# limix/CellRegMap

Measured on AMD Instinct MI355X. Metric: variant-tests/sec (interaction test), higher is better.
Workload: dtype f64

## Files before the change

### cellregmap_amd/_lib.py

```python
import ctypes
import os

import numpy as np

_HERE = os.path.dirname(os.path.abspath(__file__))
LIB_PATH = os.path.join(_HERE, "libcrm_hip.so")

c_double_p = ctypes.POINTER(ctypes.c_double)
c_int_p = ctypes.POINTER(ctypes.c_int)
c_long_p = ctypes.POINTER(ctypes.c_long)
vp = ctypes.c_void_p

SIGNATURES = {
    "crm_last_error": (ctypes.c_char_p, []),
    "crm_version": (ctypes.c_char_p, []),
    "crm_ctx_create": (ctypes.c_int, [ctypes.c_int, ctypes.POINTER(vp)]),
    "crm_ctx_destroy": (None, [vp]),
    "crm_ctx_synchronize": (ctypes.c_int, [vp]),
    "crm_ctx_trim": (ctypes.c_int, [vp]),
    "crm_background_create_qs": (ctypes.c_int, [vp, ctypes.c_long, ctypes.c_int, vp, vp, vp, vp,
                                                ctypes.POINTER(vp)]),
    "crm_background_create": (ctypes.c_int, [vp, ctypes.c_long, vp, ctypes.c_int, vp, ctypes.c_long,
                                             ctypes.c_int, vp, ctypes.c_double, ctypes.POINTER(vp)]),
    "crm_background_create_hadamard": (ctypes.c_int, [vp, ctypes.c_long, vp, ctypes.c_int, vp, ctypes.c_int, vp,
                                                      ctypes.c_int, ctypes.c_int, vp, ctypes.c_double,
                                                      ctypes.POINTER(vp)]),
    "crm_background_set_kinship_groups": (ctypes.c_int, [vp, vp, ctypes.c_long, vp, ctypes.c_long, vp, ctypes.c_int]),
    "crm_background_kinship_groups": (ctypes.c_int, [vp]),
    "crm_background_kinship_folded": (ctypes.c_long, [vp]),
    "crm_background_begin": (ctypes.c_int, [vp, ctypes.c_long, vp, ctypes.c_int, vp, ctypes.c_long, vp, ctypes.c_int, vp,
                                            ctypes.c_int, ctypes.c_int, vp, vp, ctypes.c_double, ctypes.POINTER(vp)]),
    "crm_background_complete": (ctypes.c_int, [vp, vp]),
    "crm_background_layout": (ctypes.c_int, [vp, c_long_p, c_long_p, c_long_p, c_int_p]),
    "crm_background_export": (ctypes.c_int, [vp, ctypes.c_int, ctypes.c_int, vp]),
    "crm_background_import": (ctypes.c_int, [vp, ctypes.c_int, ctypes.c_int, vp]),
    "crm_background_seal": (ctypes.c_int, [vp]),
    "crm_background_destroy": (None, [vp]),
    "crm_background_rank": (ctypes.c_int, [vp, ctypes.c_int]),
    "crm_background_read": (ctypes.c_int, [vp, ctypes.c_int, vp, vp]),
    "crm_gene_create": (ctypes.c_int, [vp, vp, vp, ctypes.c_int, vp, ctypes.c_int, ctypes.POINTER(vp)]),
    "crm_gene_create_like": (ctypes.c_int, [vp, vp, ctypes.POINTER(vp)]),
    "crm_gene_create_batch": (ctypes.c_int, [vp, vp, ctypes.c_long, ctypes.c_int, ctypes.POINTER(vp)]),
    "crm_gene_destroy": (None, [vp]),
    "crm_panel_create": (ctypes.c_int, [vp, ctypes.c_long, vp, ctypes.c_long, ctypes.c_long,
                                        ctypes.POINTER(vp)]),
    "crm_panel_create_grouped": (ctypes.c_int, [vp, ctypes.c_long, vp, ctypes.c_long, vp, ctypes.c_long,
                                                ctypes.c_long, ctypes.POINTER(vp)]),
    "crm_panel_create_grouped_i8": (ctypes.c_int, [vp, ctypes.c_long, vp, ctypes.c_long, vp, ctypes.c_long, ctypes.c_long,
                                                   ctypes.c_int, ctypes.POINTER(vp)]),
    "crm_panel_create_auto": (ctypes.c_int, [vp, ctypes.c_long, vp, ctypes.c_long, ctypes.c_long, vp, ctypes.c_long,
                                             vp, ctypes.POINTER(vp), c_int_p]),
    "crm_set_donor_collapse": (ctypes.c_int, [vp, ctypes.c_int]),
    "crm_panel_destroy": (None, [vp]),
    "crm_scan_interaction": (ctypes.c_int, [vp, vp, ctypes.c_long, ctypes.c_long] + [vp] * 13),
    "crm_scan_interaction_info": (ctypes.c_int, [vp, vp, ctypes.c_long, ctypes.c_long] + [vp] * 6),
    "crm_scan_interaction_bounds": (ctypes.c_int, [vp, vp, ctypes.c_long, ctypes.c_long] + [vp] * 8),
    "crm_scan_interaction_permuted": (ctypes.c_int, [vp, vp, ctypes.c_long, ctypes.c_long, ctypes.c_int] + [vp] * 8),
    "crm_scan_interaction_multi": (ctypes.c_int, [vp, ctypes.c_int, vp, ctypes.c_long, ctypes.c_long] + [vp] * 8),
    "crm_scan_interaction_tail": (ctypes.c_int, [vp, vp, ctypes.c_long, ctypes.c_long] + [vp] * 15),
    "crm_scan_interaction_permuted_tail": (ctypes.c_int, [vp, vp, ctypes.c_long, ctypes.c_long, ctypes.c_int] + [vp] * 10),
    "crm_scan_interaction_multi_tail": (ctypes.c_int, [vp, ctypes.c_int, vp, ctypes.c_long, ctypes.c_long] + [vp] * 10),
    "crm_scan_association": (ctypes.c_int, [vp, vp, ctypes.c_long, ctypes.c_long, ctypes.c_int, vp, vp, vp]),
    "crm_association_null_multi": (ctypes.c_int, [vp, ctypes.c_int, vp]),
    "crm_scan_association_multi": (ctypes.c_int, [vp, ctypes.c_int, vp, ctypes.c_long, ctypes.c_long, ctypes.c_int, vp, vp,
                                                  vp]),
    "crm_lmm_fit": (ctypes.c_int, [vp, ctypes.c_int, vp, vp]),
    "crm_cov_solve": (ctypes.c_int, [vp, ctypes.c_int, ctypes.c_double, ctypes.c_double, vp, ctypes.c_int, vp]),
    "crm_effects_multi": (ctypes.c_int, [vp, vp, ctypes.c_long, vp, ctypes.c_int, vp, ctypes.c_int, vp, ctypes.c_int, vp,
                                         ctypes.c_int, vp, ctypes.c_int, ctypes.c_int, vp, vp, vp, vp]),
    "crm_set_block_variants": (ctypes.c_int, [vp, ctypes.c_int]),
    "crm_set_null_fit_polish": (ctypes.c_int, [vp, ctypes.c_int]),
    "crm_set_progress_callback": (ctypes.c_int, [vp, vp, vp]),
    "crm_set_fast_rotation": (ctypes.c_int, [vp, ctypes.c_int]),
    "crm_kernel_timer_reset": (ctypes.c_int, [vp]),
    "crm_kernel_timer_read": (ctypes.c_int, [vp, c_double_p, c_long_p, c_double_p, c_double_p]),
    "crm_kernel_timer_stop": (ctypes.c_int, [vp]),
    "crm_test_set_form": (ctypes.c_int, [ctypes.c_char_p, ctypes.c_int, ctypes.c_int]),
    "crm_test_set_contraction": (ctypes.c_int, [vp, ctypes.c_int, ctypes.c_int]),
    "crm_test_set_shared_h": (ctypes.c_int, [vp, ctypes.c_int]),
    "crm_test_tail_launches": (ctypes.c_long, [vp]),
    "crm_test_spectrum_tail_launches": (ctypes.c_long, [vp]),
    "crm_test_dense_repeats": (ctypes.c_long, [vp]),
    "crm_test_donor_pair_blocks": (ctypes.c_long, [vp]),
    "crm_test_unrelated_donor_blocks": (ctypes.c_int, [vp, ctypes.POINTER(ctypes.c_long)]),
    "crm_test_gram_dma_launches": (ctypes.c_int, [vp, ctypes.POINTER(ctypes.c_long)]),
    "crm_test_rho0_position_blocks": (ctypes.c_int, [vp, ctypes.POINTER(ctypes.c_long)]),
    "crm_test_rotation_tail_launches": (ctypes.c_int, [vp, ctypes.POINTER(ctypes.c_long)]),
    "crm_test_tests_without_pair": (ctypes.c_long, [vp]),
    "crm_test_set_contraction_sync": (ctypes.c_int, [vp, ctypes.c_int]),
    "crm_test_sync_fallbacks": (ctypes.c_long, [vp]),
    "crm_test_overruns": (ctypes.c_long, []),
    "crm_test_live_device_bytes": (ctypes.c_long, []),
    "crm_test_set_kinship_route": (ctypes.c_int, [vp, ctypes.c_int]),
    "crm_test_check_context": (ctypes.c_int, [vp]),
    "crm_test_overrun_selftest": (ctypes.c_int, [vp]),
    "crm_test_null_fit_probe": (ctypes.c_int, [vp, ctypes.c_int, ctypes.c_double]),
    "crm_test_null_fit_probe_read": (ctypes.c_int, [vp, vp, ctypes.c_long]),
    "crm_test_contract": (ctypes.c_int, [vp, ctypes.c_long, ctypes.c_int, ctypes.c_int, vp, vp, vp,
                                         ctypes.c_int]),
    "crm_test_contract_kr": (ctypes.c_int, [vp, ctypes.c_long, ctypes.c_int, ctypes.c_int, ctypes.c_int,
                                            vp, vp, vp, vp]),
    "crm_test_contract_kr_t": (ctypes.c_int, [vp, ctypes.c_long, ctypes.c_int, ctypes.c_int, ctypes.c_int,
                                              vp, vp, vp, vp]),
    "crm_test_eigh": (ctypes.c_int, [vp, ctypes.c_int, ctypes.c_int, vp, vp, vp, ctypes.c_int, vp, vp]),
    "crm_test_eigh2": (ctypes.c_int, [vp, ctypes.c_int, ctypes.c_int, vp, vp, vp, vp, vp, ctypes.c_int, vp, vp, vp]),
    "crm_test_back_tasks": (ctypes.c_int, [ctypes.c_int, ctypes.c_long, ctypes.c_int, vp, ctypes.c_int, c_int_p]),
    "crm_test_dc_plan": (ctypes.c_int, [vp, vp, ctypes.c_int, ctypes.c_int, ctypes.c_double, c_int_p, c_double_p, vp, vp, vp,
                                        c_int_p, vp]),
    "crm_test_eigvalsh": (ctypes.c_int, [vp, ctypes.c_int, ctypes.c_int, vp, vp]),
    "crm_test_davies": (ctypes.c_int, [vp, ctypes.c_int, ctypes.c_int, vp, vp, vp, vp, vp]),
    "crm_test_davies_trace": (ctypes.c_int, [vp, ctypes.c_int, ctypes.c_int, vp, vp, vp, vp, vp, vp]),
    "crm_test_tail_pvalue": (ctypes.c_int, [vp, ctypes.c_int, ctypes.c_int, vp, vp, vp, vp, vp]),
}

_lib = None


class CrmError(RuntimeError):
    pass


def load():
    global _lib
    if _lib is not None:
        return _lib
    if not os.path.exists(LIB_PATH):
        raise CrmError(
            f"{LIB_PATH} is missing: build it with `python -m cellregmap_amd.build` "
            "(there is no CPU fallback for this path)")
    lib = ctypes.CDLL(LIB_PATH)
    for name, (res, args) in SIGNATURES.items():
        fn = getattr(lib, name)
        fn.restype = res
        fn.argtypes = args
    _lib = lib
    return lib


def check(rc):
    if rc != 0:
        msg = load().crm_last_error()
        raise CrmError(f"libcrm_hip error {rc}: {msg.decode() if msg else ''}")


def f64(a):
    return np.ascontiguousarray(a, dtype=np.float64)


def ptr(a):
    return None if a is None else a.ctypes.data_as(vp)
```

### cellregmap_amd/csrc/api_core.hip

```cpp
#include <dlfcn.h>

#include <algorithm>
#include <atomic>
#include <cstdarg>
#include <mutex>

#include <map>

#include "crm_internal.h"
#include "eigh.h"

namespace crm {

static thread_local std::string g_error;

void set_error(const char* fmt, ...) {
    char buf[1024];
    va_list ap;
    va_start(ap, fmt);
    vsnprintf(buf, sizeof buf, fmt, ap);
    va_end(ap);
    g_error = buf;
}

const char* last_error_text() { return g_error.c_str(); }

namespace {
struct Roctx {
    int (*push)(const char*) = nullptr;
    int (*pop)() = nullptr;
    Roctx() {
        void* h = dlopen("librocprofiler-sdk-roctx.so", RTLD_LAZY | RTLD_GLOBAL);
        if (!h) h = dlopen("librocprofiler-sdk-roctx.so.1", RTLD_LAZY | RTLD_GLOBAL);
        if (!h) return;
        push = reinterpret_cast<int (*)(const char*)>(dlsym(h, "roctxRangePushA"));
        pop = reinterpret_cast<int (*)()>(dlsym(h, "roctxRangePop"));
        if (!push || !pop) push = nullptr, pop = nullptr;
    }
};
const Roctx& roctx() {
    static Roctx r;
    return r;
}
bool ranges_on() {
    static const bool on = getenv("CRM_ROCTX") || getenv("ROCP_TOOL_LIBRARIES") || getenv("ROCPROFILER_LIBRARY_CTOR");
    return on;
}
}

void trace_push(const char* name) {
    if (ranges_on() && roctx().push) roctx().push(name);
}
void trace_pop() {
    if (ranges_on() && roctx().pop) roctx().pop();
}

static bool poison_mode() {
    static const bool on = getenv("CRM_POISON") && atoi(getenv("CRM_POISON")) != 0;
    return on;
}
static constexpr size_t REDZONE = 4096;
static std::atomic<long> g_overruns{0};
long overruns_detected() { return g_overruns.load(); }
static std::atomic<long> g_live_bytes{0};
long live_device_bytes() { return g_live_bytes.load(); }

static void check_redzone(const void* ptr, size_t bytes) {
    if (!ptr || !poison_mode()) return;
    std::vector<unsigned char> rz(REDZONE);
    if (hipMemcpy(rz.data(), static_cast<const char*>(ptr) + bytes, REDZONE, hipMemcpyDeviceToHost) != hipSuccess) return;
    for (size_t i = 0; i < REDZONE; i++) {
        if (rz[i] != 0xFF) {
            g_overruns++;
            fprintf(stderr, "[crm] CRM_POISON: write past the end of a %zu-byte device buffer (first touched byte at +%zu)\n",
                    bytes, i);
            break;
        }
    }
}

static hipStream_t fill_stream() {
    static std::mutex mu;
    static std::map<int, hipStream_t> streams;
    int dev = 0;
    if (hipGetDevice(&dev) != hipSuccess) return nullptr;
    std::lock_guard<std::mutex> lock(mu);
    auto it = streams.find(dev);
    if (it != streams.end()) return it->second;
    hipStream_t st = nullptr;
    if (hipStreamCreateWithFlags(&st, hipStreamNonBlocking) != hipSuccess) st = nullptr;
    streams[dev] = st;
    return st;
}

int DevBuf::ensure(size_t need) {
    if (need <= bytes) return CRM_OK;
    if (ptr) {
        check_redzone(ptr, bytes);
        CRM_HIP(hipFree(ptr));
        g_live_bytes -= (long)bytes;
        ptr = nullptr;
        bytes = 0;
    }
    const size_t total = need + REDZONE;
    hipError_t e = hipMalloc(&ptr, total);
    if (e == hipErrorOutOfMemory && trim_idle_workspaces() > 0) {
        (void)hipGetLastError();
        e = hipMalloc(&ptr, total);
    }
    if (e != hipSuccess) {
        ptr = nullptr;
        (void)hipGetLastError();
        set_error("device allocation of %zu bytes failed: %s", need, hipGetErrorString(e));
        return CRM_ERR_HIP;
    }
    bytes = need;
    g_live_bytes += (long)need;
    hipStream_t fs = fill_stream();
    CRM_HIP(hipMemsetAsync(ptr, poison_mode() ? 0xFF : 0, total, fs));
    CRM_HIP(hipStreamSynchronize(fs));
    return CRM_OK;
}

static std::mutex g_ctx_mutex;
static std::vector<crm_ctx*> g_contexts;

static size_t trim_context(crm_ctx* c) {
    if (!c->eigh_ws || c->eigh_ws_busy) return 0;
    size_t freed = 0;
    for (const DevBuf* b : {&c->eigh_ws->A, &c->eigh_ws->Vt, &c->eigh_ws->Vc, &c->eigh_ws->QA, &c->eigh_ws->QB}) freed += b->bytes;
    *c->eigh_ws = EighWork();
    return freed;
}

EighWork* acquire_eigh_workspace(crm_ctx* c) {
    std::lock_guard<std::mutex> lock(g_ctx_mutex);
    if (!c->eigh_ws) c->eigh_ws = new EighWork();
    c->eigh_ws_busy = true;
    return c->eigh_ws;
}

void release_eigh_workspace(crm_ctx* c) {
    std::lock_guard<std::mutex> lock(g_ctx_mutex);
    c->eigh_ws_busy = false;
}

size_t trim_idle_workspaces() {
    std::lock_guard<std::mutex> lock(g_ctx_mutex);
    size_t freed = 0;
    for (crm_ctx* c : g_contexts) freed += trim_context(c);
    return freed;
}
void DevBuf::release() {
    if (ptr) check_redzone(ptr, bytes);
    if (ptr) (void)hipFree(ptr);
    g_live_bytes -= (long)bytes;
    ptr = nullptr;
    bytes = 0;
}

int upload_padded(hipStream_t st, double* dst, long ld_dst, long rows_pad, const double* src,
                  long ld_src, long rows, long cols) {
    CRM_HIP(hipMemsetAsync(dst, 0, sizeof(double) * rows_pad * ld_dst, st));
    if (rows > 0 && cols > 0)
        CRM_HIP(hipMemcpy2DAsync(dst, ld_dst * sizeof(double), src, ld_src * sizeof(double),
                                 cols * sizeof(double), rows, hipMemcpyHostToDevice, st));
    return CRM_OK;
}

}

using namespace crm;

extern "C" {

const char* crm_last_error(void) { return last_error_text(); }
const char* crm_version(void) { return "0.6.0"; }

int crm_ctx_create(int device, crm_ctx** out) {
    return crm::guarded("crm_ctx_create", [&]() -> int {
    if (!out) return CRM_ERR_ARG;
    *out = nullptr;
    int count = 0;
    CRM_HIP(hipGetDeviceCount(&count));
    if (device < 0 || device >= count) {
        set_error("crm_ctx_create: device %d not present (%d visible)", device, count);
        return CRM_ERR_ARG;
    }
    CRM_HIP(hipSetDevice(device));
    crm_ctx* c = new crm_ctx();
    c->device = device;
    if (const char* e = getenv("CRM_KIN_ROUTE")) c->kin_route = std::max(0, std::min(2, atoi(e)));
    CRM_HIP(hipStreamCreateWithFlags(&c->stream, hipStreamNonBlocking));
    CRM_HIP(hipStreamCreateWithFlags(&c->upload_stream, hipStreamNonBlocking));
    CRM_HIP(hipEventCreate(&c->ev0));
    CRM_HIP(hipEventCreate(&c->ev1));
    {
        std::lock_guard<std::mutex> lock(g_ctx_mutex);
        g_contexts.push_back(c);
    }
    *out = c;
    return CRM_OK;
    });
}

int crm_ctx_trim(crm_ctx* c) {
    return crm::guarded_on("crm_ctx_trim", c, [&]() -> int {
    if (!c) return CRM_ERR_ARG;
    CRM_HIP(hipSetDevice(c->device));
    CRM_HIP(hipStreamSynchronize(c->stream));
    std::lock_guard<std::mutex> lock(g_ctx_mutex);
    (void)trim_context(c);
    return CRM_OK;
    });
}

void crm_ctx_destroy(crm_ctx* c) {
    try {
    if (!c) return;
    (void)hipSetDevice(c->device);
    (void)hipStreamSynchronize(c->stream);
    {
        std::lock_guard<std::mutex> lock(g_ctx_mutex);
        g_contexts.erase(std::remove(g_contexts.begin(), g_contexts.end(), c), g_contexts.end());
        delete c->eigh_ws;
        c->eigh_ws = nullptr;
    }
    c->replay_clear();
    for (auto* b : c->all_bufs()) b->release();
    for (auto& e : c->timed) {
        (void)hipEventDestroy(e.first);
        (void)hipEventDestroy(e.second);
    }
    (void)hipEventDestroy(c->ev0);
    (void)hipEventDestroy(c->ev1);
    (void)hipStreamDestroy(c->stream);
    if (c->upload_stream) (void)hipStreamDestroy(c->upload_stream);
    if (c->sync_timeouts_host) (void)hipHostFree(c->sync_timeouts_host);
    delete c;
    } catch (...) {
    }
}

int crm_ctx_synchronize(crm_ctx* c) {
    return crm::guarded_on("crm_ctx_synchronize", c, [&]() -> int {
    if (!c) return CRM_ERR_ARG;
    CRM_HIP(hipSetDevice(c->device));
    CRM_HIP(hipStreamSynchronize(c->stream));
    return CRM_OK;
    });
}

int crm_set_block_variants(crm_ctx* c, int variants) {
    return crm::guarded_on("crm_set_block_variants", c, [&]() -> int {
    if (!c || variants < 0) return CRM_ERR_ARG;
    c->block_variants = variants == 0 ? 0 : (int)round_up(variants, 128);
    return CRM_OK;
    });
}

int crm_set_null_fit_polish(crm_ctx* c, int on) {
    return crm::guarded_on("crm_set_null_fit_polish", c, [&]() -> int {
    if (!c) return CRM_ERR_ARG;
    c->polish = on != 0;
    return CRM_OK;
    });
}

int crm_set_progress_callback(crm_ctx* c, void (*callback)(long, long, void*), void* user) {
    return crm::guarded_on("crm_set_progress_callback", c, [&]() -> int {
    if (!c) return CRM_ERR_ARG;
    if (callback) c->progress[std::this_thread::get_id()] = crm_ctx::Progress{callback, user};
    else c->progress.erase(std::this_thread::get_id());
    return CRM_OK;
    });
}

int crm_set_fast_rotation(crm_ctx* c, int on) {
    return crm::guarded_on("crm_set_fast_rotation", c, [&]() -> int {
    if (!c) return CRM_ERR_ARG;
    c->fast_T = on != 0;
    return CRM_OK;
    });
}

extern "C++" {
namespace crm {
namespace {
struct FormSlot { const char* name; int value; bool set; };
FormSlot g_forms[] = {{"gram_staged", 0, false}, {"kr_no_tail", 0, false}, {"nullfit_per_wave", 0, false}, {"kin_fold", 0, false},
                      {"eigh_one_stage", 0, false}, {"nullfit_exact", 0, false}, {"donor_pairs", 0, false},
                      {"pairs_without_kinship_term", 0, false}, {"flat_kappa_milli", 0, false}, {"chase_abort", 0, false}, {"nullfit_one_per_wave", 0, false},
                      {"kin_diag", 0, false}, {"donor_pairs_rotate", 0, false}, {"rho0_positions", 0, false},
                      {"rotation_tails", 0, false}, {"woodbury_ytY", 0, false},
                      {"wb_block_order", 0, false}};
std::mutex g_forms_mu;
}
int form(const char* name, int otherwise) {
    std::lock_guard<std::mutex> lock(g_forms_mu);
    for (const FormSlot& f : g_forms)
        if (strcmp(f.name, name) == 0) return f.set ? f.value : otherwise;
    return otherwise;
}
}
}

int crm_test_set_form(const char* name, int value, int reset) {
    return crm::guarded("crm_test_set_form", [&]() -> int {
    if (!name) return CRM_ERR_ARG;
    std::lock_guard<std::mutex> lock(crm::g_forms_mu);
    for (crm::FormSlot& f : crm::g_forms)
        if (strcmp(f.name, name) == 0) {
            f.value = value;
            f.set = reset == 0;
            return CRM_OK;
        }
    crm::set_error("crm_test_set_form: no kernel form is called '%s'", name);
    return CRM_ERR_ARG;
    });
}

long crm_test_tail_launches(const crm_ctx* ctx) { return ctx ? ctx->tail_launches : -1; }

long crm_test_spectrum_tail_launches(const crm_ctx* ctx) { return ctx ? ctx->spectrum_tail_launches : -1; }

long crm_test_dense_repeats(const crm_ctx* ctx) { return ctx ? ctx->dense_repeats : -1; }

long crm_test_donor_pair_blocks(const crm_ctx* ctx) { return ctx ? ctx->donor_pair_blocks : -1; }

int crm_test_gram_dma_launches(const crm_ctx* ctx, long* launches) {
    return crm::guarded("crm_test_gram_dma_launches", [&]() -> int {
    if (!ctx || !launches) return CRM_ERR_ARG;
    *launches = ctx->gram_dma_launches;
    return CRM_OK;
    });
}
int crm_test_unrelated_donor_blocks(const crm_ctx* ctx, long* blocks) {
    return crm::guarded("crm_test_unrelated_donor_blocks", [&]() -> int {
    if (!ctx || !blocks) return CRM_ERR_ARG;
    *blocks = ctx->unrelated_donor_blocks;
    return CRM_OK;
    });
}

int crm_test_rho0_position_blocks(const crm_ctx* ctx, long* blocks) {
    return crm::guarded("crm_test_rho0_position_blocks", [&]() -> int {
    if (!ctx || !blocks) return CRM_ERR_ARG;
    *blocks = ctx->rho0_position_blocks;
    return CRM_OK;
    });
}
int crm_test_rotation_tail_launches(const crm_ctx* ctx, long* launches) {
    return crm::guarded("crm_test_rotation_tail_launches", [&]() -> int {
    if (!ctx || !launches) return CRM_ERR_ARG;
    *launches = ctx->rotation_tail_launches;
    return CRM_OK;
    });
}

long crm_test_tests_without_pair(const crm_ctx* ctx) { return ctx ? ctx->tests_without_pair : -1; }

int crm_test_set_shared_h(crm_ctx* ctx, int mode) {
    return crm::guarded_on("crm_test_set_shared_h", ctx, [&]() -> int {
    if (!ctx) return CRM_ERR_ARG;
    ctx->tune.shared_h = mode < 0 ? -1 : (mode > 0 ? 1 : 0);
    return CRM_OK;
    });
}

int crm_kernel_timer_reset(crm_ctx* c) {
    return crm::guarded_on("crm_kernel_timer_reset", c, [&]() -> int {
    if (!c) return CRM_ERR_ARG;
    CRM_HIP(hipSetDevice(c->device));
    CRM_HIP(hipStreamSynchronize(c->stream));
    c->timed_used = 0;
    c->kr_flops = 0.0;
    c->timing = true;
    return CRM_OK;
    });
}

int crm_kernel_timer_stop(crm_ctx* c) {
    return crm::guarded_on("crm_kernel_timer_stop", c, [&]() -> int {
    if (!c) return CRM_ERR_ARG;
    c->timing = false;
    return CRM_OK;
    });
}

int crm_kernel_timer_read(crm_ctx* c, double* kr_ms, long* kr_launches, double* kr_flops,
                          double* total_ms) {
    return crm::guarded_on("crm_kernel_timer_read", c, [&]() -> int {
    if (!c) return CRM_ERR_ARG;
    CRM_HIP(hipSetDevice(c->device));
    CRM_HIP(hipStreamSynchronize(c->stream));
    double ms = 0.0;
    for (size_t i = 0; i < c->timed_used; i++) {
        float t = 0.f;
        CRM_HIP(hipEventElapsedTime(&t, c->timed[i].first, c->timed[i].second));
        ms += t;
    }
    if (kr_ms) *kr_ms = ms;
    if (kr_launches) *kr_launches = (long)c->timed_used;
    if (kr_flops) *kr_flops = c->kr_flops;
    if (total_ms) *total_ms = 0.0;
    return CRM_OK;
    });
}

int crm_test_set_contraction(crm_ctx* c, int tile_width, int lds_dma) {
    return crm::guarded_on("crm_test_set_contraction", c, [&]() -> int {
    if (!c || (tile_width != 0 && tile_width != 64 && tile_width != 128 && tile_width != 160)) return CRM_ERR_ARG;
    c->tune.bn = tile_width;
    c->tune.glds = lds_dma ? 1 : 0;
    return CRM_OK;
    });
}

long crm_test_sync_fallbacks(const crm_ctx* c) { return c ? c->sync_fallbacks : -1; }
long crm_test_overruns(void) { return crm::overruns_detected(); }
long crm_test_live_device_bytes(void) { return crm::live_device_bytes(); }

int crm_test_set_kinship_route(crm_ctx* c, int on) {
    return crm::guarded_on("crm_test_set_kinship_route", c, [&]() -> int {
    if (!c) return CRM_ERR_ARG;
    c->kin_route = on < 0 ? 0 : (on > 2 ? 2 : on);
    return CRM_OK;
    });
}

int crm_test_overrun_selftest(crm_ctx* c) {
    return crm::guarded_on("crm_test_overrun_selftest", c, [&]() -> int {
    if (!c) return CRM_ERR_ARG;
    CRM_HIP(hipSetDevice(c->device));
    const long before = overruns_detected();
    {
        DevBuf b;
        CRM_TRY(b.ensure(1000));
        if (poison_mode()) CRM_HIP(hipMemset(static_cast<char*>(b.ptr) + 1000, 0, 8));
        CRM_HIP(hipDeviceSynchronize());
    }
    return (int)(overruns_detected() - before);
    });
}

int crm_test_check_context(crm_ctx* c) {
    return crm::guarded_on("crm_test_check_context", c, [&]() -> int {
    if (!c) return CRM_ERR_ARG;
    CRM_HIP(hipSetDevice(c->device));
    CRM_HIP(hipStreamSynchronize(c->stream));
    for (const DevBuf* b : c->all_bufs()) check_redzone(b->ptr, b->bytes);
    if (c->eigh_ws)
        for (const DevBuf* b : {&c->eigh_ws->A, &c->eigh_ws->Vt, &c->eigh_ws->Vc, &c->eigh_ws->QA, &c->eigh_ws->QB, &c->eigh_ws->d,
                                &c->eigh_ws->e, &c->eigh_ws->tau, &c->eigh_ws->lam, &c->eigh_ws->small})
            check_redzone(b->ptr, b->bytes);
    return CRM_OK;
    });
}

int crm_test_null_fit_probe(crm_ctx* c, int on, double x) {
    return crm::guarded_on("crm_test_null_fit_probe", c, [&]() -> int {
    if (!c) return CRM_ERR_ARG;
    if (on < 0 || on > 2) return CRM_ERR_ARG;
    c->probe_on = on != 0;
    c->probe_mode = on;
    c->probe_x = x;
    return CRM_OK;
    });
}

int crm_test_null_fit_probe_read(crm_ctx* c, double* out, long capacity) {
    return crm::guarded_on("crm_test_null_fit_probe_read", c, [&]() -> int {
    if (!c || !out || capacity < (long)c->probe_out.size()) return CRM_ERR_ARG;
    std::copy(c->probe_out.begin(), c->probe_out.end(), out);
    return (int)c->probe_out.size();
    });
}

int crm_test_set_contraction_sync(crm_ctx* c, int every) {
    return crm::guarded_on("crm_test_set_contraction_sync", c, [&]() -> int {
    if (!c || every < 0) return CRM_ERR_ARG;
    c->tune.sync = every;
    return CRM_OK;
    });
}

int crm_test_contract(crm_ctx* c, long cells, int M, int N, const double* X, const double* Y,
                      double* C, int ksplit) {
    return crm::guarded_on("crm_test_contract", c, [&]() -> int {
    if (!c || cells <= 0 || M <= 0 || N <= 0 || !X || !Y || !C || ksplit < 1) return CRM_ERR_ARG;
    CRM_HIP(hipSetDevice(c->device));
    const long cp = round_up(cells, GEMM_BK * (long)ksplit);
    const long ldx = round_up(M, 128), ldy = round_up(N, 128);
// ... 170 lines not shown
```

### cellregmap_amd/csrc/blockops.hip

```cpp
#include "nullfit.h"

namespace crm {

namespace {

constexpr int STAT_SPLITS = 64;

__device__ __forceinline__ void row_and_chunk(int chunks, long& row, int& chunk) {
    row = blockIdx.x / (unsigned)chunks;
    chunk = (int)(blockIdx.x - (unsigned)row * (unsigned)chunks);
}
inline dim3 row_chunk_grid(long rows, int chunks) { return dim3((unsigned)(rows * chunks)); }

template <int C>
__global__ __launch_bounds__(256) void variant_stats_kernel(const double* __restrict__ G, long ldg,
                                                           long cells, int variants,
                                                           const double* __restrict__ y,
                                                           const double* __restrict__ W, long ldw,
                                                           double* __restrict__ partial) {
    __shared__ double red[4][C + 2][64];
    const int tx = threadIdx.x & 63, ty = threadIdx.x >> 6;
    const int b = blockIdx.x * 64 + tx;
    const long per = (cells + STAT_SPLITS - 1) / STAT_SPLITS;
    const long i0 = (long)blockIdx.y * per;
// ... 213 lines not shown
    if (q >= dst_cols) return;
    double v = 0.0;
    const int p = q / k0;
    if (p < npairs) v = src[h * ld_src + (long)ord[p] * k0 + (q - p * k0)];
    dst[h * ld_dst + q] = v;
}

int launch_gather_slabs(hipStream_t st, const double* src, long ld_src, long rows, const int* ord, int npairs,
                        int k0, double* dst, long ld_dst, int dst_cols) {
    if (rows <= 0 || dst_cols <= 0) return CRM_OK;
    dim3 grid((unsigned)rows, (dst_cols + 255) / 256);
    hipLaunchKernelGGL(gather_slabs_kernel, grid, dim3(256), 0, st, src, ld_src, ord, npairs, k0, dst, ld_dst,
                       dst_cols);
    CRM_HIP(hipGetLastError());
    return CRM_OK;
}

__global__ void gather_rows_kernel(const double* __restrict__ src, long ld_src, const int* __restrict__ map, int cols,
                                   double* __restrict__ dst, long ld_dst, int chunks) {
    long k;
    int chunk;
    row_and_chunk(chunks, k, chunk);
    const int j = chunk * blockDim.x + threadIdx.x;
    if (j >= cols) return;
    const int c = map[k];
    dst[k * ld_dst + j] = c >= 0 ? src[(long)c * ld_src + j] : 0.0;
}

int launch_gather_rows(hipStream_t st, const double* src, long ld_src, const int* map, long rows, int cols, double* dst,
                       long ld_dst) {
    if (rows <= 0 || cols <= 0) return CRM_OK;
    const int chunks = (cols + 255) / 256;
    hipLaunchKernelGGL(gather_rows_kernel, row_chunk_grid(rows, chunks), dim3(256), 0, st, src, ld_src, map, cols, dst, ld_dst,
                       chunks);
    CRM_HIP(hipGetLastError());
    return CRM_OK;
}

__global__ void kin_operand_kernel(const double* __restrict__ U, int k2, const double* __restrict__ H, long ldh, int k1,
                                   const int* __restrict__ map, double* __restrict__ Y, long ldy) {
    const long k = blockIdx.x;
    const int j = threadIdx.x;
    if (j >= ldy) return;
    const int c = map[k];
    double v = 0.0;
    if (c >= 0) {
        if (j < k2) v = U[(long)c * k2 + j];
        else if (j < k2 + k1) v = H[(long)c * ldh + (j - k2)];
    }
    Y[k * ldy + j] = v;
}

int launch_kin_operand(hipStream_t st, const double* U, int k2, const double* H, long ldh, int k1, const int* map, long rows,
                       double* Y, long ldy) {
    if (rows <= 0) return CRM_OK;
    hipLaunchKernelGGL(kin_operand_kernel, dim3((unsigned)rows), dim3((unsigned)ldy), 0, st, U, k2, H, ldh, k1, map, Y, ldy);
    CRM_HIP(hipGetLastError());
    return CRM_OK;
}

__global__ void kin_verify_kernel(const double* __restrict__ H, long ldh, int k1, const double* __restrict__ U, int k2,
                                  const int* __restrict__ group, const double* __restrict__ hKd, long ldk, long m,
                                  unsigned long long* __restrict__ out) {
    const long c = blockIdx.x;
    const long g = group[c];
    double dmax = 0.0, hmax = 0.0;
    for (long e = threadIdx.x; e < (long)k2 * m; e += blockDim.x) {
        const long j = e / m, d = e - j * m;
        const double h = H[c * ldh + k1 + e];
        const double want = U[c * k2 + j] * hKd[g * ldk + d];
        const double diff = fabs(h - want);
        dmax = diff > dmax || diff != diff ? diff : dmax;
        hmax = fmax(hmax, fabs(h));
    }
    for (int off = 32; off > 0; off >>= 1) {
        const double o = __shfl_xor(dmax, off);
        dmax = o > dmax || o != o ? o : dmax;
        hmax = fmax(hmax, __shfl_xor(hmax, off));
    }
    if ((threadIdx.x & 63) == 0) {
        if (dmax != dmax) dmax = INFINITY;
        atomicMax(&out[0], (unsigned long long)__double_as_longlong(dmax));
        atomicMax(&out[1], (unsigned long long)__double_as_longlong(hmax));
    }
}

int launch_kin_verify(hipStream_t st, const double* H, long ldh, int k1, const double* U, int k2, const int* group,
                      const double* hKd, long ldk, long m, long n, unsigned long long* out) {
    if (n <= 0) return CRM_OK;
    hipLaunchKernelGGL(kin_verify_kernel, dim3((unsigned)n), dim3(256), 0, st, H, ldh, k1, U, k2, group, hKd, ldk, m, out);
    CRM_HIP(hipGetLastError());
    return CRM_OK;
}

__global__ void kin_sum_e1_kernel(const double* __restrict__ S, long ld_s, int KT, int k2, int groups, long cols,
                                  double* __restrict__ AH, long ld_ah) {
    const int a = blockIdx.y;
    const long c = (long)blockIdx.x * blockDim.x + threadIdx.x;
    if (c >= cols) return;
    double acc = 0.0;
    for (int d = 0; d < groups; d++) acc += S[((long)d * KT + k2 + a) * ld_s + c];
    AH[(long)a * ld_ah + c] = acc;
}

int launch_kin_sum_e1(hipStream_t st, const double* S, long ld_s, int KT, int k2, int k1, int groups, long cols, double* AH,
                      long ld_ah) {
    if (k1 <= 0 || cols <= 0) return CRM_OK;
    dim3 grid((unsigned)((cols + 255) / 256), (unsigned)k1);
    hipLaunchKernelGGL(kin_sum_e1_kernel, grid, dim3(256), 0, st, S, ld_s, KT, k2, groups, cols, AH, ld_ah);
    CRM_HIP(hipGetLastError());
    return CRM_OK;
}

__global__ void ortho_coef_kernel(const double* __restrict__ gW, long ld_gW, const double* __restrict__ proj, int c,
                                  int variants, int cols, double* __restrict__ coef, long ld_coef,
                                  double* __restrict__ thr) {
    const int b = blockIdx.x * blockDim.x + threadIdx.x;
    if (b >= cols) return;
    constexpr double EPS = 2.220446049250313e-16;
    const double* __restrict__ inv = proj;
    const double* __restrict__ V = proj + (long)c * c;
    const double* __restrict__ d2 = V + (long)c * c;
    const double* __restrict__ h = gW + (long)b * ld_gW;
    double t = 1.0;
    for (int j = 0; j < c; j++) {
        double a = 0.0;
        if (b < variants) {
            double hv = 0.0;
            for (int k = 0; k < c; k++) {
                a = fma(inv[j * c + k], h[k], a);
                hv = fma(V[k * c + j], h[k], hv);
            }
            t += (hv / d2[j]) * (hv / (d2[j] - EPS));
        }
        coef[(long)j * ld_coef + b] = a;
    }
    if (b < variants) thr[b] = EPS * t;
}

__global__ __launch_bounds__(256) void ortho_apply_kernel(const double* __restrict__ G, long ldg,
                                                         const double* __restrict__ W, long ldw, int c,
                                                         const double* __restrict__ coef, long ld_coef, int cols,
                                                         double* __restrict__ Gx, long ldx, int chunks) {
    long i;
    int chunk;
    row_and_chunk(chunks, i, chunk);
    const int b = chunk * blockDim.x + threadIdx.x;
    if (b >= cols) return;
    double v = G[i * ldg + b];
    for (int j = 0; j < c; j++) v = fma(-W[i * ldw + j], coef[(long)j * ld_coef + b], v);
    Gx[i * ldx + b] = v;
}

__global__ void ortho_rank_kernel(const double* __restrict__ gg, const double* __restrict__ thr, int variants,
                                  int* __restrict__ drop) {
    const int b = blockIdx.x * blockDim.x + threadIdx.x;
    if (b < variants) drop[b] = gg[b] < thr[b] ? 1 : 0;
}

__global__ void collinear_flag_kernel(const double* __restrict__ gg, const double* __restrict__ gW, long ld_gW,
                                      const double* __restrict__ proj, int c, int variants, double tau,
                                      int* __restrict__ near) {
    const int b = blockIdx.x * blockDim.x + threadIdx.x;
    if (b >= variants) return;
    const double* __restrict__ h = gW + (long)b * ld_gW;
    double rest = gg[b];
    for (int j = 0; j < c; j++) {
        double a = 0.0;
        for (int k = 0; k < c; k++) a = fma(proj[j * c + k], h[k], a);
        rest -= h[j] * a;
    }
    near[b] = rest > tau * gg[b] ? 0 : 1;
}

int launch_ortho_block(hipStream_t st, const double* G, long ldg, long cells_pad, int variants, int cols,
                       const double* W, long ldw, int c, const double* proj, const double* gW, long ld_gW,
                       double* coef, long ld_coef, double* thr, double* Gx, long ldx) {
    if (cols <= 0) return CRM_OK;
    hipLaunchKernelGGL(ortho_coef_kernel, dim3((cols + 255) / 256), dim3(256), 0, st, gW, ld_gW, proj, c, variants, cols,
                       coef, ld_coef, thr);
    CRM_HIP(hipGetLastError());
    const int chunks = (cols + 255) / 256;
    hipLaunchKernelGGL(ortho_apply_kernel, row_chunk_grid(cells_pad, chunks), dim3(256), 0, st, G, ldg, W,
                       ldw, c, coef, ld_coef, cols, Gx, ldx, chunks);
    CRM_HIP(hipGetLastError());
    return CRM_OK;
}

int launch_ortho_rank(hipStream_t st, const double* gg, const double* thr, int variants, int* drop) {
    if (variants <= 0) return CRM_OK;
    hipLaunchKernelGGL(ortho_rank_kernel, dim3((variants + 255) / 256), dim3(256), 0, st, gg, thr, variants, drop);
    CRM_HIP(hipGetLastError());
    return CRM_OK;
}

int launch_collinear_flag(hipStream_t st, const double* gg, const double* gW, long ld_gW, const double* proj, int c,
                          int variants, double tau, int* near) {
    if (variants <= 0) return CRM_OK;
    hipLaunchKernelGGL(collinear_flag_kernel, dim3((variants + 255) / 256), dim3(256), 0, st, gg, gW, ld_gW, proj, c,
                       variants, tau, near);
    CRM_HIP(hipGetLastError());
    return CRM_OK;
}

__global__ void pair_features_kernel(const double* __restrict__ H, long ldh, int k1, const double* __restrict__ Ep,
                                     long ld_ep, int k0, double* __restrict__ P, long ldp) {
    const long c = blockIdx.x;
    for (int q = threadIdx.x; q < ldp; q += blockDim.x) {
        const int a = q / k0, i = q - a * k0;
        P[c * ldp + q] = a < k1 ? H[c * ldh + a] * Ep[c * ld_ep + i] : 0.0;
    }
}

int launch_pair_features(hipStream_t st, const double* H, long ldh, int k1, const double* Ep, long ld_ep, int k0,
                         long cells_pad, double* P, long ldp) {
    if (cells_pad <= 0) return CRM_OK;
    hipLaunchKernelGGL(pair_features_kernel, dim3((unsigned)cells_pad), dim3(256), 0, st, H, ldh, k1, Ep, ld_ep, k0, P, ldp);
    CRM_HIP(hipGetLastError());
    return CRM_OK;
}

__global__ void same_columns_kernel(const double* __restrict__ H, long ldh, const double* __restrict__ Ep, long ld_ep,
                                    long cells, int k, int* __restrict__ flag) {
    const long c = blockIdx.x;
    if (c >= cells) return;
    bool diff = false;
    for (int a = threadIdx.x; a < k; a += blockDim.x)
        diff |= __double_as_longlong(H[c * ldh + a]) != __double_as_longlong(Ep[c * ld_ep + a]);
    if (diff) atomicOr(flag, 1);
}

int launch_same_columns(hipStream_t st, const double* H, long ldh, const double* Ep, long ld_ep, long cells, int k, int* flag) {
    if (cells <= 0 || k <= 0) return CRM_OK;
    hipLaunchKernelGGL(same_columns_kernel, dim3((unsigned)cells), dim3(64), 0, st, H, ldh, Ep, ld_ep, cells, k, flag);
    CRM_HIP(hipGetLastError());
    return CRM_OK;
}

__global__ void pair_rows_sym_kernel(const double* __restrict__ C, long ldc, int variants, int k0, double* __restrict__ S,
                                     long lds) {
    const int a = blockIdx.y;
    const long e = (long)blockIdx.x * blockDim.x + threadIdx.x;
    if (e >= (long)variants * k0) return;
    const long b = e / k0;
    const int i = (int)(e - b * k0);
    const int lo = a < i ? a : i, hi = a < i ? i : a;
    const long pidx = (long)lo * k0 - (long)lo * (lo - 1) / 2 + (hi - lo);
    S[(long)a * lds + e] = C[b * ldc + pidx];
}

int launch_pair_rows_sym(hipStream_t st, const double* C, long ldc, int variants, int k0, double* S, long lds) {
    if (variants <= 0 || k0 <= 0) return CRM_OK;
    dim3 grid((unsigned)(((long)variants * k0 + 255) / 256), (unsigned)k0);
    hipLaunchKernelGGL(pair_rows_sym_kernel, grid, dim3(256), 0, st, C, ldc, variants, k0, S, lds);
    CRM_HIP(hipGetLastError());
    return CRM_OK;
}

constexpr int DP_VARIANTS = 4, DP_MAX_SLOTS = 32;

template <int DP_SLOTS>
__global__ __launch_bounds__(256) void donor_pairs_expand_kernel(const double* __restrict__ P, long p_slab, long ldp, int donors,
                                                                  int variants, int k0, int k1, double* __restrict__ S, long lds,
                                                                  double* __restrict__ Psum, long psum_slab, long row_d, long row_j) {
    extern __shared__ double tile[];
    const int npair = k0 * (k0 + 1) / 2, total = DP_VARIANTS * npair;
    const int v0 = blockIdx.x * DP_VARIANTS, tid = threadIdx.x;
    const int per = (donors + gridDim.y - 1) / gridDim.y;
    const int d0 = blockIdx.y * per, d1 = min(donors, d0 + per);
    if (d0 >= d1) return;
    double acc[DP_SLOTS], x[DP_SLOTS];
    int src[DP_SLOTS];
#pragma unroll
    for (int q = 0; q < DP_SLOTS; q++) {
        const int e = tid + 256 * q, v = e / npair, pr = e - v * npair;
        acc[q] = 0.0;
        src[q] = e < total && v0 + v < variants ? (int)((long)(v0 + v) * ldp + pr) : -1;
    }
    auto fetch = [&](int d) {
        const double* __restrict__ Pd = P + (size_t)d * p_slab;
#pragma unroll
        for (int q = 0; q < DP_SLOTS; q++)
            if (tid + 256 * q < total) x[q] = src[q] >= 0 ? Pd[src[q]] : 0.0;
    };
    const int row_len = DP_VARIANTS * k0;
    const int vw = tid / k0, iw = tid - vw * k0;
    const bool writer = tid < row_len && v0 + vw < variants;
    const int base_i = iw * k0 - iw * (iw - 1) / 2 - iw;
    const double* __restrict__ mine = tile + vw * npair;
    fetch(d0);
    for (int d = d0; d < d1; d++) {
#pragma unroll
        for (int q = 0; q < DP_SLOTS; q++)
            if (tid + 256 * q < total) { acc[q] += x[q]; tile[tid + 256 * q] = x[q]; }
        __syncthreads();
        if (d + 1 < d1) fetch(d + 1);
        if (writer) {
            double* __restrict__ Sd = S + (size_t)(k1 + (long)d * row_d) * lds + (long)v0 * k0 + tid;
            for (int j = 0; j < k0; j++) {
                const int pidx = j <= iw ? j * k0 - j * (j - 1) / 2 + (iw - j) : base_i + j;
                Sd[(long)j * row_j * lds] = mine[pidx];
            }
        }
        __syncthreads();
    }
    double* __restrict__ out = Psum + (size_t)blockIdx.y * psum_slab;
#pragma unroll
    for (int q = 0; q < DP_SLOTS; q++)
        if (tid + 256 * q < total && src[q] >= 0) out[src[q]] = acc[q];
}

bool donor_pairs_serves(int k0) { return k0 >= 2 && DP_VARIANTS * (k0 * (k0 + 1) / 2) <= 256 * DP_MAX_SLOTS && DP_VARIANTS * k0 <= 256; }

int launch_donor_pairs_expand(hipStream_t st, const double* P, long p_slab, long ldp, int donors, int variants, int k0, int k1,
                              double* S, long lds, double* Psum, long psum_slab, int splits, long row_d, long row_j) {
    if (row_d <= 0) { row_d = k0; row_j = 1; }
    if (variants <= 0 || donors <= 0) return CRM_OK;
    if (!donor_pairs_serves(k0) || splits < 1) {
        set_error("donor pairs: k0=%d outside the supported range", k0);
        return CRM_ERR_UNSUPPORTED;
    }
    const size_t lds_bytes = sizeof(double) * DP_VARIANTS * (size_t)(k0 * (k0 + 1) / 2);
    dim3 grid((unsigned)((variants + DP_VARIANTS - 1) / DP_VARIANTS), (unsigned)splits);
    const int slots = (DP_VARIANTS * (k0 * (k0 + 1) / 2) + 255) / 256;
#define CRM_DP_LAUNCH(SL)                                                                                                        \
    hipLaunchKernelGGL(donor_pairs_expand_kernel<SL>, grid, dim3(256), lds_bytes, st, P, p_slab, ldp, donors, variants, k0, k1, \
                       S, lds, Psum, psum_slab, row_d, row_j)
    if (slots <= 4) CRM_DP_LAUNCH(4);
    else if (slots <= 8) CRM_DP_LAUNCH(8);
    else if (slots <= 16) CRM_DP_LAUNCH(16);
    else if (slots <= 24) CRM_DP_LAUNCH(24);
    else CRM_DP_LAUNCH(32);
#undef CRM_DP_LAUNCH
    CRM_HIP(hipGetLastError());
    return CRM_OK;
}

// ... 247 lines not shown
```

### cellregmap_amd/csrc/crm_internal.h

```cpp
#pragma once
#include <map>
#include <mutex>
#include <thread>
#include <type_traits>
#include <utility>

#include "crm_common.h"

namespace crm {

constexpr int CRM_DEFAULT_BLOCK = 1024;
constexpr int CRM_MAX_AUTO_BLOCK = 4096;
constexpr int CRM_MAX_RHO = 16;
constexpr int CRM_MAX_COV = 8;
constexpr int CRM_MAX_COV_WIDE = 62;
constexpr int CRM_MAX_COV_XWIDE = 128;
constexpr int CRM_MAX_K0 = 256;
constexpr int CRM_MAX_GRAM_ROWS = 288;
constexpr int DT_SUMS_LD = 136;
constexpr int BLOCK_SLACK_MAX = 4096;

struct DevBuf {
    void* ptr = nullptr;
    size_t bytes = 0;
    DevBuf() = default;
    DevBuf(const DevBuf&) = delete;
    DevBuf& operator=(const DevBuf&) = delete;
    DevBuf(DevBuf&& o) noexcept : ptr(o.ptr), bytes(o.bytes) { o.ptr = nullptr; o.bytes = 0; }
    DevBuf& operator=(DevBuf&& o) noexcept {
        if (this != &o) {
            release();
            ptr = o.ptr; bytes = o.bytes;
            o.ptr = nullptr; o.bytes = 0;
        }
        return *this;
    }
    ~DevBuf() { release(); }
    int ensure(size_t need);
    void release();
    template <class T>
    T* as() const { return static_cast<T*>(ptr); }
};
static_assert(!std::is_copy_constructible<DevBuf>::value, "DevBuf owns its allocation");

int upload_padded(hipStream_t st, double* dst, long ld_dst, long rows_pad, const double* src,
                  long ld_src, long rows, long cols);

struct EighWork;
size_t trim_idle_workspaces();
long overruns_detected();
long live_device_bytes();
}
struct crm_ctx;
namespace crm {
EighWork* acquire_eigh_workspace(crm_ctx* ctx);
void release_eigh_workspace(crm_ctx* ctx);

}

struct crm_ctx {
    std::recursive_mutex mu;
    int device = 0;
    hipStream_t stream = nullptr;
    hipStream_t upload_stream = nullptr;
    hipEvent_t ev0 = nullptr, ev1 = nullptr;
    int block_variants = 0;
    bool fast_T = true;
    int kin_route = 1;
    bool fast_gene_rot = true;
    bool collapse = true;
    struct Progress { void (*fn)(long done, long total, void* user) = nullptr; void* user = nullptr; };
    std::map<std::thread::id, Progress> progress;
    bool progress_muted = false;
    void report(long done, long total) {
        if (progress_muted) return;
        auto it = progress.find(std::this_thread::get_id());
        if (it != progress.end() && it->second.fn) it->second.fn(done, total, it->second.user);
    }
    bool in_scan = false;
    bool polish = false;
    bool probe_on = false;
    int probe_mode = 0;
    double probe_x = 0.0;
    std::vector<double> probe_out;
    bool nullfit_exact = false;
    crm::GemmTune tune;
    crm::DevBuf sync_counters;
    unsigned* sync_timeouts_host = nullptr;
    long sync_fallbacks = 0;
    long dense_repeats = 0;
    long tail_launches = 0;
    long spectrum_tail_launches = 0;
    long donor_pair_blocks = 0;
    long rotation_tail_launches = 0;
    long rho0_position_blocks = 0;
    long unrelated_donor_blocks = 0;
    long gram_dma_launches = 0;
    long tests_without_pair = 0;
    struct ReplayBlock {
        long col0 = 0;
        int nb = 0;
        bool collapsed = false;
        std::vector<char> fit;
        crm::DevBuf T;
    };
    int replay_mode = 0;
    size_t replay_cursor = 0;
    std::vector<ReplayBlock*> replay_blocks;
    void replay_clear() {
        for (ReplayBlock* b : replay_blocks) delete b;
        replay_blocks.clear();
        replay_cursor = 0;
        replay_mode = 0;
    }
    crm::EighWork* eigh_ws = nullptr;
    bool eigh_ws_busy = false;
    bool timing = false;
    std::vector<std::pair<hipEvent_t, hipEvent_t>> timed;
    size_t timed_used = 0;
    double kr_flops = 0.0;
    crm::DevBuf ws_T, ws_A, ws_Gb, ws_Gx, ws_Gs, ws_G2, ws_GG, ws_Gt, ws_Z, ws_small, ws_probs, ws_F, ws_Gext, ws_TH, ws_AH, ws_XG;
    crm::DevBuf ws_xwide;
    crm::DevBuf ws_Tcut;
    crm::DevBuf ws_Gk, ws_S, ws_S2;
    crm::DevBuf ws_WB;
    crm::DevBuf ws_Pd;
    crm::DevBuf ws_Anone;
    std::vector<crm::DevBuf*> all_bufs() {
        return {&sync_counters, &ws_xwide, &ws_Tcut, &ws_S, &ws_S2, &ws_Gk, &ws_Pd, &ws_WB, &ws_Anone, &ws_AH, &ws_XG, &ws_TH, &ws_T, &ws_A, &ws_Gb, &ws_Gx, &ws_Gs, &ws_G2, &ws_GG, &ws_Gt, &ws_Z, &ws_small, &ws_probs, &ws_F, &ws_Gext};
    }
};

namespace crm {
template <class Body>
inline int guarded_on(const char* entry, crm_ctx* ctx, Body&& body) noexcept {
    try {
        if (!ctx) return guarded(entry, body);
        std::lock_guard<std::recursive_mutex> lock(ctx->mu);
        return guarded(entry, body);
    } catch (...) {
        set_error("%s: could not take the context's lock", entry);
        return CRM_ERR_INTERNAL;
    }
}
}
```

### cellregmap_amd/csrc/kinship.hip

```cpp
#include <algorithm>
#include <atomic>

#include "nullfit.h"
#include "objects.h"

using namespace crm;

namespace crm {

void jacobi_rotate(int k, double* A, double* V, int p, int q, double cs, double sn) {
    for (int r = 0; r < k; r++) {
        const double arp = A[(size_t)r * k + p], arq = A[(size_t)r * k + q];
        A[(size_t)r * k + p] = cs * arp - sn * arq;
        A[(size_t)r * k + q] = sn * arp + cs * arq;
    }
    for (int r = 0; r < k; r++) {
        const double apr = A[(size_t)p * k + r], aqr = A[(size_t)q * k + r];
        A[(size_t)p * k + r] = cs * apr - sn * aqr;
        A[(size_t)q * k + r] = sn * apr + cs * aqr;
    }
    for (int r = 0; r < k; r++) {
        const double vrp = V[(size_t)r * k + p], vrq = V[(size_t)r * k + q];
        V[(size_t)r * k + p] = cs * vrp - sn * vrq;
        V[(size_t)r * k + q] = sn * vrp + cs * vrq;
    }
}

static void jacobi_eigh(int k, std::vector<double>& A, std::vector<double>& V, std::vector<double>& w) {
    V.assign((size_t)k * k, 0.0);
    for (int i = 0; i < k; i++) V[(size_t)i * k + i] = 1.0;
    for (int sweep = 0; sweep < 60; sweep++) {
        bool rotated = false;
        for (int p = 0; p < k - 1; p++)
            for (int q = p + 1; q < k; q++) {
                const double apq = A[(size_t)p * k + q], app = A[(size_t)p * k + p], aqq = A[(size_t)q * k + q];
                if (!(std::fabs(apq) > 2.220446049250313e-16 * std::sqrt(std::fabs(app * aqq))) || apq == 0.0) continue;
                rotated = true;
                const double theta = (aqq - app) / (2.0 * apq);
                const double t = (theta >= 0.0 ? 1.0 : -1.0) / (std::fabs(theta) + std::sqrt(theta * theta + 1.0));
                const double cs = 1.0 / std::sqrt(t * t + 1.0), sn = t * cs;
                jacobi_rotate(k, A.data(), V.data(), p, q, cs, sn);
                A[(size_t)p * k + q] = A[(size_t)q * k + p] = 0.0;
            }
        if (!rotated) break;
    }
    w.resize(k);
    for (int i = 0; i < k; i++) w[i] = A[(size_t)i * k + i];
}

static int seal_unrelated_donors(crm_background* bg, const double* hKd, long m) {
    bg->kin_wb = false;
    const long groups = bg->kin_groups;
    const int k1 = bg->kin_k1, k2 = bg->kin_k2, KK = k1 + k2;
    if (form("kin_diag", 1) == 0 || k2 > 128 || k1 > 64 || (double)groups * groups * m > 4e9) return CRM_OK;
    std::vector<double> kappa(groups, 0.0);
    for (long d = 0; d < groups; d++)
        for (long q = 0; q < m; q++) kappa[d] += hKd[d * m + q] * hKd[d * m + q];
    const double tol = 8.0 * (double)m * 2.220446049250313e-16;
    for (long d = 0; d < groups; d++)
        for (long e = d + 1; e < groups; e++) {
            double s = 0.0;
            for (long q = 0; q < m; q++) s += hKd[d * m + q] * hKd[e * m + q];
            if (!(std::fabs(s) <= tol * std::sqrt(kappa[d] * kappa[e]))) return CRM_OK;
        }
    crm_ctx* ctx = bg->ctx;
    hipStream_t st = ctx->stream;
    const long ldc = round_up(KK, 128);
    if (sizeof(double) * (double)groups * KK * ldc > (double)(1ull << 30)) return CRM_OK;
    DevBuf dC, probs_dev;
    CRM_TRY(dC.ensure(sizeof(double) * (size_t)groups * KK * ldc));
    std::vector<GemmProblem> pr((size_t)groups);
    long maxlen = GEMM_BK;
    for (long d = 0; d < groups; d++) {
        GemmProblem p{};
        p.X = bg->kin_Y.as<double>() + bg->kin_row0[d] * bg->kin_ldy; p.ldx = bg->kin_ldy;
        p.Y = p.X; p.ldy = bg->kin_ldy;
        p.C = dC.as<double>() + (size_t)d * KK * ldc; p.ldc = ldc;
        p.M = KK; p.N = KK; p.cells = bg->kin_len[d];
        maxlen = std::max(maxlen, bg->kin_len[d]);
        pr[d] = p;
    }
    CRM_TRY(probs_dev.ensure(sizeof(GemmProblem) * pr.size()));
    CRM_HIP(hipMemcpyAsync(probs_dev.ptr, pr.data(), sizeof(GemmProblem) * pr.size(), hipMemcpyHostToDevice, st));
    CRM_TRY(launch_gemm_tn(ctx, probs_dev.as<GemmProblem>(), (int)groups, KK, KK, maxlen, false, 0, 1, 0));
    std::vector<double> C((size_t)groups * KK * ldc);
    CRM_HIP(hipMemcpyAsync(C.data(), dC.ptr, sizeof(double) * C.size(), hipMemcpyDeviceToHost, st));
    CRM_HIP(hipStreamSynchronize(st));
    const int k2pad = (int)round_up(k2, GEMM_BK);
    const long P = groups * k2, ldp = round_up(P, 128);
    std::vector<double> hU((size_t)groups * k2pad * 128, 0.0), hR((size_t)k1 * ldp, 0.0), hEE((size_t)k1 * k1, 0.0),
        lam((size_t)P, 0.0);
    std::vector<double> A((size_t)k2 * k2), V, w;
    long kept = 0;
    for (long d = 0; d < groups; d++) {
        const double* Cd = C.data() + (size_t)d * KK * ldc;
        for (int i = 0; i < k2; i++)
            for (int j = 0; j < k2; j++) A[(size_t)i * k2 + j] = 0.5 * (Cd[i * ldc + j] + Cd[j * ldc + i]);
        jacobi_eigh(k2, A, V, w);
        double wmax = 0.0;
        for (int j = 0; j < k2; j++) wmax = std::max(wmax, w[j]);
        double* Ud = hU.data() + (size_t)d * k2pad * 128;
        for (int j = 0; j < k2; j++) {
            if (!(w[j] > (double)k2 * 2.220446049250313e-16 * wmax)) continue;
            const double sc = 1.0 / std::sqrt(w[j]);
            lam[d * k2 + j] = w[j];
            kept++;
            for (int q = 0; q < k2; q++) Ud[(size_t)q * 128 + j] = V[(size_t)q * k2 + j] * sc;
            for (int a = 0; a < k1; a++) {
                double s = 0.0;
                for (int q = 0; q < k2; q++) s += Ud[(size_t)q * 128 + j] * Cd[q * ldc + k2 + a];
                hR[(size_t)a * ldp + d * k2 + j] = s;
            }
        }
        for (int a = 0; a < k1; a++)
            for (int e = 0; e < k1; e++) hEE[(size_t)a * k1 + e] += Cd[(k2 + a) * ldc + k2 + e];
    }
    CRM_TRY(bg->wb_U.ensure(sizeof(double) * hU.size()));
    CRM_TRY(bg->wb_R.ensure(sizeof(double) * hR.size()));
    CRM_TRY(bg->wb_EE.ensure(sizeof(double) * hEE.size()));
    CRM_HIP(hipMemcpyAsync(bg->wb_U.ptr, hU.data(), sizeof(double) * hU.size(), hipMemcpyHostToDevice, st));
    CRM_HIP(hipMemcpyAsync(bg->wb_R.ptr, hR.data(), sizeof(double) * hR.size(), hipMemcpyHostToDevice, st));
    CRM_HIP(hipMemcpyAsync(bg->wb_EE.ptr, hEE.data(), sizeof(double) * hEE.size(), hipMemcpyHostToDevice, st));
    std::vector<std::vector<double>> s0(bg->nrho, std::vector<double>((size_t)ldp, 0.0));
    for (int i = 0; i < bg->nrho; i++) {
        for (long p = 0; p < P; p++) s0[i][p] = (1.0 - bg->rho[i]) * kappa[p / k2] * lam[p];
        CRM_TRY(bg->wb_S0[i].ensure(sizeof(double) * (size_t)ldp));
        CRM_HIP(hipMemcpyAsync(bg->wb_S0[i].ptr, s0[i].data(), sizeof(double) * (size_t)ldp, hipMemcpyHostToDevice, st));
    }
    CRM_HIP(hipStreamSynchronize(st));
    bg->wb_P = P;
    bg->wb_kept = kept;
    bg->wb_ldp = ldp;
    bg->wb_k2pad = k2pad;
    static std::atomic<unsigned long> wb_tables_made{0};
    bg->wb_gen = ++wb_tables_made;
    bg->kin_wb = true;
    return CRM_OK;
}

}

extern "C" {

int crm_background_set_kinship_groups(crm_background* bg, const int* group, long groups, const double* hKd, long m,
                                      const double* U, int k2) {
    return crm::guarded_on("crm_background_set_kinship_groups", bg ? bg->ctx : nullptr, [&]() -> int {
    if (!bg || !group || !hKd || !U || groups < 1 || m < 1 || k2 < 1) return CRM_ERR_ARG;
    if (bg->builder) {
        set_error("kinship groups: the background is still under construction");
        return CRM_ERR_ARG;
    }
    const long n = bg->n;
    const int k1 = (int)(bg->cols - (long)k2 * m);
    if (!bg->fast_T || !bg->H.ptr || k1 < 1 || k1 + k2 > 2 * CRM_MAX_K0 || groups > 4096) return CRM_OK;
    for (long i = 0; i < n; i++)
        if (group[i] < 0 || group[i] >= groups) {
            set_error("kinship groups: group index %d at cell %ld outside [0, %ld)", group[i], i, groups);
            return CRM_ERR_ARG;
        }
    crm_ctx* ctx = bg->ctx;
    CRM_HIP(hipSetDevice(ctx->device));
    hipStream_t st = ctx->stream;
    bg->kin = false;
    struct Undo {
        crm_background* b;
        ~Undo() {
            if (b->kin) return;
            b->kin_fold = false;
            b->kin_wb = false;
            for (DevBuf* x : {&b->kin_map, &b->kin_Y, &b->kin_hKd, &b->wb_U, &b->wb_R, &b->wb_EE}) x->release();
            for (int i = 0; i < b->nrho; i++) b->wb_S0[i].release();
            for (int i = 0; i < b->nrho; i++) b->MixK[i].release();
        }
    } undo{bg};
    std::vector<long> count(groups, 0);
    for (long i = 0; i < n; i++) count[group[i]]++;
    bg->kin_row0.assign(groups, 0);
    bg->kin_len.assign(groups, 0);
    long rows = 0;
    for (long d = 0; d < groups; d++) {
        bg->kin_row0[d] = rows;
        bg->kin_len[d] = round_up(std::max<long>(count[d], 1), GEMM_BK);
        rows += bg->kin_len[d];
    }
    std::vector<int> map(rows, -1);
    std::vector<long> fill(groups, 0);
    for (long i = 0; i < n; i++) {
        const long d = group[i];
        map[bg->kin_row0[d] + fill[d]++] = (int)i;
    }
    bg->kin_rows = rows;
    bg->kin_groups = groups;
    bg->kin_groups_pad = round_up(groups, GEMM_BK);
    bg->kin_cols = m;
    bg->kin_k1 = k1;
    bg->kin_k2 = k2;
    bg->kin_ldh = round_up(m, 128);
    bg->kin_ldy = round_up(k1 + k2, 128);
    CRM_TRY(bg->kin_map.ensure(sizeof(int) * rows));
    CRM_TRY(bg->kin_Y.ensure(sizeof(double) * rows * bg->kin_ldy));
    CRM_TRY(bg->kin_hKd.ensure(sizeof(double) * bg->kin_groups_pad * bg->kin_ldh));
    DevBuf dU;
    CRM_TRY(dU.ensure(sizeof(double) * n * k2));
    CRM_HIP(hipMemcpyAsync(bg->kin_map.ptr, map.data(), sizeof(int) * rows, hipMemcpyHostToDevice, st));
    CRM_HIP(hipMemcpyAsync(dU.ptr, U, sizeof(double) * n * k2, hipMemcpyHostToDevice, st));
    CRM_TRY(upload_padded(st, bg->kin_hKd.as<double>(), bg->kin_ldh, bg->kin_groups_pad, hKd, m, groups, m));
    CRM_TRY(launch_kin_operand(st, dU.as<double>(), k2, bg->H.as<double>(), bg->ldh, k1, bg->kin_map.as<int>(), rows,
                               bg->kin_Y.as<double>(), bg->kin_ldy));
    DevBuf dgroup, dcheck;
    CRM_TRY(dgroup.ensure(sizeof(int) * n));
    CRM_TRY(dcheck.ensure(2 * sizeof(unsigned long long)));
    unsigned long long check[2] = {0, 0};
    CRM_HIP(hipMemcpyAsync(dgroup.ptr, group, sizeof(int) * n, hipMemcpyHostToDevice, st));
    CRM_HIP(hipMemsetAsync(dcheck.ptr, 0, sizeof check, st));
    CRM_TRY(launch_kin_verify(st, bg->H.as<double>(), bg->ldh, k1, dU.as<double>(), k2, dgroup.as<int>(),
                              bg->kin_hKd.as<double>(), bg->kin_ldh, m, n, dcheck.as<unsigned long long>()));
    CRM_HIP(hipMemcpyAsync(check, dcheck.ptr, sizeof check, hipMemcpyDeviceToHost, st));
    CRM_HIP(hipStreamSynchronize(st));
    double dmax, hmax;
    memcpy(&dmax, &check[0], sizeof dmax);
    memcpy(&hmax, &check[1], sizeof hmax);
    if (!(dmax <= 1e-12 * hmax)) {
        set_error("kinship groups: the half factor of this background is not U[c, j] * hKd[group(c), d] (largest difference "
                  "%.3g against entries up to %.3g)", dmax, hmax);
        return CRM_ERR_ARG;
    }
    if (m + 1 <= bg->kin_ldh) {
        std::vector<double> ones((size_t)groups, 1.0);
        CRM_HIP(hipMemcpy2DAsync(bg->kin_hKd.as<double>() + m, sizeof(double) * bg->kin_ldh, ones.data(), sizeof(double),
                                 sizeof(double), groups, hipMemcpyHostToDevice, st));
        CRM_HIP(hipStreamSynchronize(st));
    }
    bg->kin_fold = false;
    const long kfold = k1 + groups * (long)k2, m_pad = round_up(m, GEMM_BK);
    const int fold_form = form("kin_fold", 1);
    if ((double)kfold <= 1.25 * (double)bg->cols && bg->cols + (m_pad - m) <= bg->ldh && (k2 >= 32 || k2 == 1 || fold_form > 1) && fold_form != 0) {
        const long kdim = round_up(kfold, GEMM_BK), ldq = bg->ldq, ld_t = round_up(groups, 128);
        DevBuf hKdT, probs_dev;
        CRM_TRY(hKdT.ensure(sizeof(double) * m_pad * ld_t));
        {
            std::vector<double> t((size_t)m_pad * ld_t, 0.0);
            for (long dd = 0; dd < groups; dd++)
                for (long d = 0; d < m; d++) t[(size_t)d * ld_t + dd] = hKd[dd * m + d];
            CRM_HIP(hipMemcpyAsync(hKdT.ptr, t.data(), sizeof(double) * t.size(), hipMemcpyHostToDevice, st));
            CRM_HIP(hipStreamSynchronize(st));
        }
        std::vector<GemmProblem> pr((size_t)bg->nrho * k2);
        for (int i = 0; i < bg->nrho; i++) {
            CRM_TRY(bg->MixK[i].ensure(sizeof(double) * kdim * ldq));
            CRM_HIP(hipMemsetAsync(bg->MixK[i].ptr, 0, sizeof(double) * kdim * ldq, st));
            CRM_HIP(hipMemcpyAsync(bg->MixK[i].ptr, bg->Mix[i].ptr, sizeof(double) * (size_t)k1 * ldq, hipMemcpyDeviceToDevice, st));
            for (int j = 0; j < k2; j++) {
                GemmProblem p{};
                p.X = hKdT.as<double>(); p.ldx = ld_t;
                p.Y = bg->Mix[i].as<double>() + (size_t)(k1 + (long)j * m) * ldq; p.ldy = ldq;
                p.C = bg->MixK[i].as<double>() + (size_t)(k1 + j) * ldq; p.ldc = (long)k2 * ldq;
                p.M = (int)groups; p.N = bg->r[i] > 0 ? bg->r[i] : 1;
                pr[(size_t)i * k2 + j] = p;
            }
        }
        CRM_TRY(probs_dev.ensure(sizeof(GemmProblem) * pr.size()));
        CRM_HIP(hipMemcpyAsync(probs_dev.ptr, pr.data(), sizeof(GemmProblem) * pr.size(), hipMemcpyHostToDevice, st));
        CRM_TRY(launch_gemm_tn(ctx, probs_dev.as<GemmProblem>(), (int)pr.size(), (int)groups, (int)ldq, m_pad, false, 0, 1, 0));
        CRM_HIP(hipStreamSynchronize(st));
        bg->kin_kdim = kdim;
        bg->kin_fold = true;
        CRM_TRY(seal_unrelated_donors(bg, hKd, m));
    }
    bg->kin = true;
    return CRM_OK;
    });
}

int crm_background_kinship_groups(const crm_background* bg) {
    if (!bg) return 0;
    try {
        std::lock_guard<std::recursive_mutex> lock(bg->ctx->mu);
        return bg->kin ? (int)bg->kin_groups : 0;
    } catch (...) {
        return 0;
    }
}

long crm_background_kinship_folded(const crm_background* bg) {
    if (!bg) return 0;
    try {
        std::lock_guard<std::recursive_mutex> lock(bg->ctx->mu);
        return bg->kin && bg->kin_fold ? bg->kin_kdim : 0;
    } catch (...) {
        return 0;
    }
}

}
```

### cellregmap_amd/csrc/nullfit.h

```cpp
#pragma once
#include "crm_internal.h"

namespace crm {

struct NullFitRho {
    const double* T;
    const double* ty;
    const double* tW;
    const double* S0;
    long ldT, ldW;
    int r;
    int pad_;
};

struct NullFitTrial {
    double lml, delta, scale;
    int use_g, nfev;
    double margin;
    double noise;
    double curv;
};

struct NullFitOut {
    int rho_index;
    int use_g;
    double lml, delta, scale, v0, v1;
    double decision, rho_decision;
    double margin, noise, gap, curv;
};

struct NullFitArgs {
    NullFitRho rho[CRM_MAX_RHO];
    int nrho, c, restricted;
    int polish;
    int exact;
    int track;
    int probe;
    double probe_x;
    long n;
    const double* WW;
    const double* Wy;
    double yy;
    const double* gg;
    const double* gy;
    const double* gW;
    long ld_gW;
    const int* g_drop;
    double* xwide;
    NullFitTrial* trial;
    NullFitOut* out;
};
void nullfit_gene_args(NullFitArgs& a, const crm_gene* gene, int restricted);

int launch_nullfit(hipStream_t st, const NullFitArgs& a, int variants, bool force_wide = false, unsigned* queue = nullptr);
int launch_nullfit_wide(hipStream_t st, const NullFitArgs& a, int variants);
int launch_nullfit_xwide(hipStream_t st, const NullFitArgs& a, int variants);
size_t nullfit_xwide_scratch_doubles(int variants, int nrho, int c);

struct AssocArgs {
    const double* T;
    const double* ty;
    const double* tW;
    const double* S0;
    long ldT, ldW;
    int r, c;
    long n;
    double delta0;
    const double* WW; const double* Wy; double yy;
    const double* gg; const double* gy; const double* gW; long ld_gW;
};
size_t fastscan_prep_doubles();
int launch_fastscan_prep(hipStream_t st, const AssocArgs& a, double* prep, double* wts);
int launch_fastscan_prep_batch(hipStream_t st, const AssocArgs* args_dev, int genes, int c, double* prep, long prep_stride,
                               double* wts, long wts_stride);
int launch_fastscan(hipStream_t st, const AssocArgs& a, const double* prep, const double* wts,
                    int variants, double* alt_lml);
int launch_lrt(hipStream_t st, const double* alt_lml, double null_lml, int count, double* pv);
int launch_gather_trial_lml(hipStream_t st, const NullFitTrial* trial, int count, double* out);

int launch_variant_stats(hipStream_t st, const double* G, long ldg, long cells, int variants,
                         const double* y, const double* W, long ldw, int c, double* partial,
                         double* gg, double* gy, double* gW, long ld_gW);
size_t variant_stats_workspace(int variants, int c);
int launch_ortho_block(hipStream_t st, const double* G, long ldg, long cells_pad, int variants, int cols,
                       const double* W, long ldw, int c, const double* proj, const double* gW, long ld_gW,
                       double* coef, long ld_coef, double* thr, double* Gx, long ldx);
int launch_ortho_rank(hipStream_t st, const double* gg, const double* thr, int variants, int* drop);
int launch_collinear_flag(hipStream_t st, const double* gg, const double* gW, long ld_gW, const double* proj, int c,
                          int variants, double tau, int* near);
int launch_gather_block(hipStream_t st, const double* src, long ld_src, long cells_pad, long cells,
                        const int* row_index, const int* col_index, int variants, double* dst,
                        long ld_dst, int dst_cols);
int launch_gather_slabs(hipStream_t st, const double* src, long ld_src, long rows, const int* ord, int npairs,
                        int k0, double* dst, long ld_dst, int dst_cols);
int launch_gather_rows(hipStream_t st, const double* src, long ld_src, const int* map, long rows, int cols, double* dst,
                       long ld_dst);
int launch_kin_operand(hipStream_t st, const double* U, int k2, const double* H, long ldh, int k1, const int* map, long rows,
                       double* Y, long ldy);
int launch_kin_verify(hipStream_t st, const double* H, long ldh, int k1, const double* U, int k2, const int* group,
                      const double* hKd, long ldk, long m, long n, unsigned long long* out);
int launch_kin_sum_e1(hipStream_t st, const double* S, long ld_s, int KT, int k2, int k1, int groups, long cols, double* AH,
                      long ld_ah);
int launch_pair_features(hipStream_t st, const double* H, long ldh, int k1, const double* Ep, long ld_ep, int k0,
                         long cells_pad, double* P, long ldp);
int launch_pair_rows(hipStream_t st, const double* C, long ldc, int variants, int k1, int k0, double* S, long lds);
int launch_same_columns(hipStream_t st, const double* H, long ldh, const double* Ep, long ld_ep, long cells, int k, int* flag);
int launch_pair_rows_sym(hipStream_t st, const double* C, long ldc, int variants, int k0, double* S, long lds);
bool donor_pairs_serves(int k0);
int launch_donor_pairs_expand(hipStream_t st, const double* P, long p_slab, long ldp, int donors, int variants, int k0, int k1,
                              double* S, long lds, double* Psum, long psum_slab, int splits, long row_d = 0, long row_j = 0);
bool donor_pairs_rotate_serves(int k0);
int launch_donor_pairs_rotate(hipStream_t st, const double* P, long p_slab, long ldp, int donors, int variants, int k0,
                              const double* U, long u_slab, long ldu, int k2pad, double* A, long lda, double* Psum, long psum_slab,
                              int splits);
int launch_scale_rows(hipStream_t st, const double* src, long ld_src, const double* scale, long ld_scale, long rows, int cols,
                      double* dst, long ld_dst);
int launch_expand_block(hipStream_t st, const double* Gd, long ld_gd, const int* group, long cells_pad,
                        long cells, const int* row_index, int variants, double* dst, long ld_dst,
                        int dst_cols);
int launch_indicator(hipStream_t st, const int* group, long cells, long cells_pad, int m, double* Z, long ldz);
int launch_donor_stats(hipStream_t st, const double* Gam, long ld_gam, int m, int variants,
                       const double* sums, int c, double* gg, double* gy, double* gW, long ld_gW);
int launch_square_block(hipStream_t st, const double* Gt, const double* G, long ldg, long ldg_t,
                        long cells_pad, int cols, double* G2, double* GG, long ld_out);
int launch_context_features(hipStream_t st, const double* E, long lde, const int* row_index,
                            long cells, long cells_pad, int k0, const double* y, const double* W,
                            long ldw, int c, double* Ep, long ld_ep, double* YE, long ld_ye,
                            double* EE, long ld_ee);

struct AssembleRho {
    const double* ty;
    const double* tW;
    const double* S0;
    const double* T;
    long ldW, ldT;
    int r;
    int pad_;
    double rho;
};

struct AssembleArgs {
    AssembleRho rho[CRM_MAX_RHO];
    const NullFitOut* fit;
    const int* sorted_pos;
    const double* A;
    long ldA;
    const double* A_none;
    int k0, c;
    long n;
    const double* Z1; long ldZ1;
    const double* Z2; long ldZ2;
    const double* Z3; long ldZ3;
    const double* WW; const double* Wy; double yy;
    const double* gg; const double* gy; const double* gW; long ld_gW;
    const double* coef; long ld_coef;
    double* Q;
    double* F;
    int wb_k1;
    const double* wb_R; long wb_ldR;
    const double* wb_E1X; long wb_ldE1X;
    const double* wb_E1yW; long wb_ldE1yW;
    const double* wb_E1g; long wb_ldE1g;
    const double* wb_EE;
    double* wb_Gw;
};

int launch_assemble(hipStream_t st, const AssembleArgs& a, int variants, double* Gext, double* fin_rows = nullptr,
                    long* dma_launches = nullptr);
size_t assemble_rows_scratch_doubles(int variants, int k0, int c);
size_t woodbury_lds_bytes(int KT, int k1);

int launch_eig_davies(hipStream_t st, const double* F, const double* Q, int count, int k,
                      double* lambda, double* pvalue, int* ifault, double* liu, bool do_eig, double* scratch = nullptr,
                      int* trace = nullptr);
size_t eig_scratch_doubles(int count, int k);

int launch_tail_pvalue(hipStream_t st, const double* Q, const double* lambda, int count, int k, double* pvalue,
                       double* logp, int* status);

}
```

### cellregmap_amd/csrc/objects.h

```cpp
#pragma once
#include <cmath>
#include <memory>

#include "crm_internal.h"

namespace crm {
constexpr long CELL_PAD = 128;
}

struct crm_donor_tables {
    unsigned long e0_key = 0, group_key = 0;
    unsigned long stamp = 0;
    crm::DevBuf TZ;
    crm::DevBuf Bd;
    crm::DevBuf Z2;
    crm::DevBuf Z3;
};

struct crm_background_builder;

struct crm_background {
    ~crm_background();
    crm_background_builder* builder = nullptr;
    crm_ctx* ctx = nullptr;
    long n = 0, n_pad = 0;
    int nrho = 0;
    double rho[crm::CRM_MAX_RHO] = {0};
    int r[crm::CRM_MAX_RHO] = {0};
    double ortho_defect[crm::CRM_MAX_RHO] = {0};
    long ldq = 0;
    crm::DevBuf Q0[crm::CRM_MAX_RHO];
    bool q0_ready[crm::CRM_MAX_RHO] = {false};
    crm::DevBuf Ht;
    crm::DevBuf S0[crm::CRM_MAX_RHO];
    std::vector<double> s0_max;
    bool fast_T = false;
    long ldh = 0, cols = 0;
    crm::DevBuf H;
    crm::DevBuf Mix[crm::CRM_MAX_RHO];
    bool kin = false;
    long kin_groups = 0, kin_groups_pad = 0;
    long kin_cols = 0;
    int kin_k1 = 0, kin_k2 = 0;
    long kin_rows = 0;
    std::vector<long> kin_row0, kin_len;
    crm::DevBuf kin_map;
    crm::DevBuf kin_Y;
    long kin_ldy = 128;
    crm::DevBuf kin_hKd;
    long kin_ldh = 0;
    bool kin_fold = false;
    long kin_kdim = 0;
    crm::DevBuf MixK[crm::CRM_MAX_RHO];
    bool kin_wb = false;
    long wb_P = 0, wb_ldp = 0;
    long wb_kept = 0;
    int wb_k2pad = 0;
    crm::DevBuf wb_U;
    crm::DevBuf wb_R;
    crm::DevBuf wb_EE;
    crm::DevBuf wb_S0[crm::CRM_MAX_RHO];
    unsigned long wb_gen = 0;
    static constexpr int DT_CACHE = 2;
    std::vector<crm_donor_tables*> dt_cache;
    unsigned long dt_clock = 0;
};

int crm_background_require_q0(crm_background* bg, int i);

struct crm_gene {
    crm_background* bg = nullptr;
    crm_ctx* ctx = nullptr;
    int c = 0, k0 = 0;
    long ld_yw = 0, ldw = 0, lde = 0;
    std::vector<double> W_host;
    std::vector<double> W_basis;
    crm::DevBuf yW;
    crm::DevBuf E0;
    crm::DevBuf WW, Wy;
    crm::DevBuf Wproj;
    double yy = 0.0;
    crm::DevBuf rot;
    crm::DevBuf Ep, YE, EE, idx;
    crm::DevBuf kinEp;
    crm::DevBuf kinP;
    crm::DevBuf kinUE;
    crm::DevBuf kinEE;
    crm::DevBuf wb_yW;
    unsigned long wb_gen = 0;
    long ld_ep = 0, ld_ye = 0, ld_ee = 0;
    unsigned long e0_key = 0;
    unsigned long w_key = 0;
    unsigned long dt_group = 0;
    crm_donor_tables dt_own;
    crm::DevBuf dt_Z1;
    crm::DevBuf dt_sums;
    crm::DevBuf dt_Zt;
};

struct crm_panel {
    crm_ctx* ctx = nullptr;
    unsigned long uid = 0;
    long n = 0, n_pad = 0, p = 0, ld = 0;
    crm::DevBuf G;
    bool grouped = false;
    long m = 0, m_pad = 0;
    crm::DevBuf Gd;
    crm::DevBuf group;
    unsigned long group_key = 0;
    crm::DevBuf Z;
    long ldz = 0;
};

namespace crm {
template <class T> struct Destroy;
template <> struct Destroy<crm_background> { void operator()(crm_background* p) const { crm_background_destroy(p); } };
template <> struct Destroy<crm_gene> { void operator()(crm_gene* p) const { crm_gene_destroy(p); } };
template <> struct Destroy<crm_panel> { void operator()(crm_panel* p) const { crm_panel_destroy(p); } };
template <class T> using Owned = std::unique_ptr<T, Destroy<T>>;

unsigned long content_key(const void* data, size_t bytes, unsigned long seed);

void jacobi_rotate(int k, double* A, double* V, int p, int q, double cs, double sn);

int build_donor_tables(crm_gene* gene, const crm_panel* panel, crm_donor_tables* shared, const double* d_Ep, const double* d_EE,
                       const double* Zt, bool cross);
int launch_permute_group(hipStream_t st, const int* group, const int* idx, long n, int* out);
int launch_donor_cross(hipStream_t st, int nb, const double* Gam, long ld_gam, int m, const double* C, long ldc, int k0,
                       double* Z2, long ldz2);
}
```

### cellregmap_amd/csrc/scan_block.hip

```cpp
#include "scan_pass.h"

namespace crm {

int ctx_cus(const crm_ctx* ctx) {
    int cus = 256;
    if (hipDeviceGetAttribute(&cus, hipDeviceAttributeMultiprocessorCount, ctx->device) != hipSuccess || cus < 1) cus = 256;
    return cus;
}

__global__ void replay_rows_kernel(double* __restrict__ T, long blk, long ldT, const crm::NullFitOut* __restrict__ fit, int nb,
                                   int cols, double* __restrict__ rows, int restore) {
    const int b = blockIdx.y;
    const int j = blockIdx.x * blockDim.x + threadIdx.x;
    if (b >= nb || j >= cols) return;
    const int ri = fit[b].rho_index;
    if (ri < 0) return;
    double* slab = T + ((size_t)ri * blk + b) * ldT;
    if (restore) slab[j] = rows[(size_t)b * ldT + j];
    else rows[(size_t)b * ldT + j] = slab[j];
}

int ScanPass::copy_block(Block& B) {
    const long ldb = P.ldb;
    const int nb = B.nb;
    B.Gb = B.Gt = B.Gx = ctx->ws_Gb.as<double>();
    if (P.collapsed()) {
        CRM_TRY(launch_gather_block(st, panel->Gd.as<double>() + B.col0, panel->ld, P.mp, panel->m, nullptr, nullptr, nb, B.Gb, ldb, (int)ldb));
    } else if (panel->grouped) {
        CRM_TRY(launch_expand_block(st, panel->Gd.as<double>() + B.col0, panel->ld, panel->group.as<int>(), np, n, nullptr, nb, B.Gb, ldb, (int)ldb));
        if (idx_G) {
            B.Gt = ctx->ws_Gt.as<double>();
            CRM_TRY(launch_expand_block(st, panel->Gd.as<double>() + B.col0, panel->ld, panel->group.as<int>(), np, n, d_idxG, nb, B.Gt, ldb, (int)ldb));
        }
    } else {
        CRM_TRY(launch_gather_block(st, panel->G.as<double>() + B.col0, panel->ld, np, n, nullptr, nullptr, nb, B.Gb, ldb, (int)ldb));
        if (idx_G) {
            B.Gt = ctx->ws_Gt.as<double>();
            CRM_TRY(launch_gather_block(st, panel->G.as<double>() + B.col0, panel->ld, np, n, d_idxG, nullptr, nb, B.Gt, ldb, (int)ldb));
        }
    }
    return CRM_OK;
}

int ScanPass::block_stats(Block& B) {
    const long ldb = P.ldb, ld_gW = P.ld_gW;
    const int nb = B.nb, BLK = P.BLK;
    if (!P.collapsed()) {
        B.Gx = ctx->ws_Gx.as<double>();
        CRM_TRY(launch_variant_stats(st, B.Gb, ldb, np, nb, g0->yW.as<double>(), g0->yW.as<double>() + 1, g0->ld_yw, c, d_part, d_gg, d_gy, d_gW, ld_gW));
        CRM_TRY(launch_ortho_block(st, B.Gb, ldb, np, nb, (int)ldb, g0->yW.as<double>() + 1, g0->ld_yw, c, g0->Wproj.as<double>(),
                                   d_gW, ld_gW, d_coef, ldb, d_thr, B.Gx, ldb));
    }
    for (int gi = 0; gi < ng; gi++) {
        crm_gene* g = genes[gi];
        if (P.collapsed())
            CRM_TRY(launch_donor_stats(st, B.Gb, ldb, (int)panel->m, nb, g->dt_sums.as<double>(), c, d_gg, d_gy + (size_t)gi * BLK, d_gW, ld_gW));
        else
            CRM_TRY(launch_variant_stats(st, B.Gx, ldb, np, nb, g->yW.as<double>(), g->yW.as<double>() + 1, g->ld_yw, c, d_part, d_gg, d_gy + (size_t)gi * BLK, d_gW, ld_gW));
    }
    if (P.collapsed()) {
        if (near_out) CRM_TRY(launch_collinear_flag(st, d_gg, d_gW, ld_gW, g0->Wproj.as<double>(), c, nb, COLLINEAR_TAU, d_near));
    } else
        CRM_TRY(launch_ortho_rank(st, d_gg, d_thr, nb, d_drop));
    return CRM_OK;
}

int ScanPass::fold_TH(const Block& B) {
    const long ldb = P.ldb;
    const int nb = B.nb, k1 = bg->kin_k1, k2 = bg->kin_k2;
    const long groups = bg->kin_groups;
    double* Gk = ctx->ws_Gk.as<double>();
    double* TH = ctx->ws_TH.as<double>();
    CRM_TRY(launch_gather_rows(st, B.Gx, ldb, bg->kin_map.as<int>(), bg->kin_rows, (int)ldb, Gk, ldb));
    std::vector<GemmProblem> kp((size_t)groups + 1);
    GemmProblem p{};
    p.X = bg->kin_Y.as<double>(); p.ldx = bg->kin_ldy; p.Y = Gk; p.ldy = ldb; p.C = TH + (size_t)k1 * ldb; p.ldc = ldb;
    p.M = k2; p.N = nb;
    const long maxlen = donor_run_records(bg, p, (long)k2 * ldb, kp.data());
    GemmProblem& e = kp[groups];
    e.X = bg->H.as<double>(); e.ldx = bg->ldh; e.Y = B.Gx; e.ldy = ldb;
    e.C = ctx->ws_S2.as<double>(); e.ldc = ldb; e.M = k1; e.N = nb;
    const long e1_slab = (long)k1 * ldb;
    return with_records(SLOT_KIN, kp, [&](GemmProblem* d_kp) -> int {
        CRM_TRY(launch_gemm_tn(ctx, d_kp, (int)groups, k2, nb, maxlen, false, 0, 1, 0));
        CRM_TRY(launch_gemm_tn(ctx, d_kp + groups, 1, k1, nb, np, false, 0, P.fold_split3, e1_slab));
        CRM_TRY(launch_reduce_splits(st, ctx->ws_S2.as<double>(), e1_slab, P.fold_split3, e1_slab));
        CRM_HIP(hipMemcpyAsync(TH, ctx->ws_S2.ptr, sizeof(double) * (size_t)e1_slab, hipMemcpyDeviceToDevice, st));
        return CRM_OK;
    });
}

int ScanPass::unfolded_TH(const Block& B) {
    const long ldb = P.ldb, KK = P.KK;
    const int nb = B.nb, k1 = bg->kin_k1, k2 = bg->kin_k2;
    const long groups = bg->kin_groups, mk = bg->kin_cols;
    double* Gk = ctx->ws_Gk.as<double>();
    double* S2 = ctx->ws_S2.as<double>();
    CRM_TRY(launch_gather_rows(st, B.Gx, ldb, bg->kin_map.as<int>(), bg->kin_rows, (int)ldb, Gk, ldb));
    std::vector<GemmProblem> kp((size_t)groups + k2);
    GemmProblem p{};
    p.X = bg->kin_Y.as<double>(); p.ldx = bg->kin_ldy; p.Y = Gk; p.ldy = ldb; p.C = S2; p.ldc = ldb;
    p.M = (int)KK; p.N = nb;
    const long maxlen = donor_run_records(bg, p, KK * ldb, kp.data());
    for (int j = 0; j < k2; j++) {
        GemmProblem& q = kp[groups + j];
        q.X = bg->kin_hKd.as<double>(); q.ldx = bg->kin_ldh; q.Y = S2 + (size_t)j * ldb; q.ldy = KK * ldb;
        q.C = ctx->ws_TH.as<double>() + (size_t)(k1 + (long)j * mk) * ldb; q.ldc = ldb; q.M = (int)mk; q.N = nb;
    }
    return with_records(SLOT_KIN, kp, [&](GemmProblem* d_kp) -> int {
        CRM_TRY(launch_gemm_tn(ctx, d_kp, (int)groups, (int)KK, nb, maxlen, false, 0, 1, 0));
        CRM_TRY(launch_gemm_tn(ctx, d_kp + groups, k2, (int)mk, nb, bg->kin_groups_pad, false, 0, 1, 0));
        return launch_kin_sum_e1(st, S2, ldb, (int)KK, k2, k1, (int)groups, nb, ctx->ws_TH.as<double>(), ldb);
    });
}

int ScanPass::plain_TH(const Block& B) {
    const long ldb = P.ldb;
    GemmProblem p{};
    p.X = bg->H.as<double>(); p.ldx = bg->ldh; p.Y = B.Gx; p.ldy = ldb;
    p.C = ctx->ws_TH.as<double>(); p.ldc = ldb; p.M = (int)bg->cols; p.N = B.nb;
    CRM_TRY(upload(SLOT_ONE, &p, 1));
    CRM_TRY(launch_gemm_tn(ctx, d_probs + SLOT_ONE, 1, (int)bg->cols, B.nb, np, false, 0, P.ks_h, P.th_slab));
    return launch_reduce_splits(st, ctx->ws_TH.as<double>(), (long)bg->cols * ldb, P.ks_h, P.th_slab);
}

bool ScanPass::cut_choice(int nb, int cnt, const int* N, bool* is_cut, long& acc, long& rounds) const {
    const long slots = 2L * ctx_cus(ctx), mtl = (nb + GEMM_BM - 1) / GEMM_BM;
    long tiles[CRM_MAX_RHO], total = 0;
    int order[CRM_MAX_RHO];
    for (int i = 0; i < cnt; i++) { tiles[i] = mtl * ((N[i] + 127) / 128); total += tiles[i]; order[i] = i; }
    std::sort(order, order + cnt, [&](int a, int b) { return tiles[a] < tiles[b]; });
    const long need = total % slots;
    acc = 0;
    int take = 0;
    while (take < cnt - 1 && acc < need) acc += tiles[order[take++]];
    const bool cut = total > slots && need > 0 && acc >= need && acc <= slots / 4;
    rounds = ((cut ? total - acc : total) + slots - 1) / slots;
    for (int q = 0; q < take && cut; q++) is_cut[order[q]] = true;
    return cut;
}
int ScanPass::cut_rotations(const Block& B, int n_list, int& n_main) {
    const int nb = B.nb, BLK = P.BLK;
    n_main = n_list;
    const long slots = 2L * ctx_cus(ctx);
    int widths[CRM_MAX_RHO];
    bool is_cut[CRM_MAX_RHO] = {false};
    long acc = 0, rounds = 0;
    for (int i = 0; i < n_list; i++) widths[i] = probs[i].N;
    if (!cut_choice(nb, n_list, widths, is_cut, acc, rounds)) return CRM_OK;
    int n_cut = 0, cut_ks = 1;
    GemmProblem cut_probs[CRM_MAX_RHO];
    double* cut_dst[CRM_MAX_RHO];
    long cut_doubles = 0;
    while ((long)(cut_ks + 1) * acc <= slots && cut_ks < 16 && P.kdim / GEMM_BK / (cut_ks + 1) >= 8) cut_ks++;
    n_main = 0;
    for (int i = 0; i < n_list; i++) {
        if (!is_cut[i]) { probs[n_main++] = probs[i]; continue; }
        GemmProblem c = probs[i];
        cut_dst[n_cut] = c.C;
        c.ldc = round_up(c.N, 128);
        cut_doubles += (long)BLK * c.ldc;
        cut_probs[n_cut++] = c;
    }
    CRM_TRY(ctx->ws_Tcut.ensure(sizeof(double) * (size_t)cut_doubles * cut_ks));
    long at = 0;
    for (int q = 0; q < n_cut; q++) {
        cut_probs[q].C = ctx->ws_Tcut.as<double>() + at;
        at += (long)BLK * cut_probs[q].ldc;
    }
    const int slot = SLOT_RHO + n_main;
    CRM_TRY(upload(slot, cut_probs, n_cut));
    int cut_maxn = 1;
    for (int q = 0; q < n_cut; q++) cut_maxn = std::max(cut_maxn, cut_probs[q].N);
    CRM_TRY(launch_gemm_tn(ctx, d_probs + slot, n_cut, nb, cut_maxn, P.kdim, false, 0, cut_ks, cut_doubles));
    CRM_TRY(launch_reduce_splits(st, ctx->ws_Tcut.as<double>(), cut_doubles, cut_ks, cut_doubles));
    for (int q = 0; q < n_cut; q++)
        CRM_HIP(hipMemcpy2DAsync(cut_dst[q], sizeof(double) * P.ldT, cut_probs[q].C, sizeof(double) * cut_probs[q].ldc,
                                 sizeof(double) * cut_probs[q].N, nb, hipMemcpyDeviceToDevice, st));
    return CRM_OK;
}

int ScanPass::rotations(const Block& B) {
    const int nb = B.nb;
    if (P.folded()) CRM_TRY(fold_TH(B));
    else if (P.kin()) CRM_TRY(unfolded_TH(B));
    else if (P.fastT) CRM_TRY(plain_TH(B));
    if (P.wb()) CRM_TRY(woodbury_phi(B));
    GemmProblem all[CRM_MAX_RHO];
    for (int i = 0; i < nrho; i++) {
        GemmProblem p{};
        if (P.fastT) {
            p.X = ctx->ws_TH.as<double>(); p.ldx = P.ldb;
            p.Y = P.folded() ? bg->MixK[i].as<double>() : bg->Mix[i].as<double>(); p.ldy = ldq;
        } else {
            p.X = B.Gx; p.ldx = P.ldb;
            p.Y = P.collapsed() ? tab->TZ.as<double>() + (size_t)i * P.mp * ldq : bg->Q0[i].as<double>(); p.ldy = ldq;
        }
        p.C = ctx->ws_T.as<double>() + (size_t)i * P.BLK * P.ldT; p.ldc = P.ldT;
        p.M = nb; p.N = bg->r[i] > 0 ? bg->r[i] : 1;
        all[i] = p;
    }
    const int n_list = plan_rotations(B, all);
    if (n_list == 0) return CRM_OK;
    int n_main = n_list;
    if (P.fastT) CRM_TRY(cut_rotations(B, n_list, n_main));
    CRM_TRY(upload(SLOT_RHO, probs.data(), n_main));
    const bool timing_T = P.wb() && ctx->timing && ctx->timed_used < 65536;
    if (timing_T) CRM_TRY(timer_open(true));
    CRM_TRY(launch_gemm_tn(ctx, d_probs + SLOT_RHO, n_main, nb, (int)ldq, P.fastT ? P.kdim : P.xrows, false, 0, 1, 0));
    if (timing_T) {
        CRM_TRY(timer_close());
        for (int q = 0; q < n_main; q++) ctx->kr_flops += 2.0 * (double)P.kdim * (double)nb * (double)probs[q].N;
    }
    if (!rot_tails.empty()) {
        CRM_TRY(upload(SLOT_RHO + n_list, rot_tails.data(), rot_tails.size()));
        CRM_TRY(launch_skinny_tn(st, d_probs + SLOT_RHO + n_list, (int)rot_tails.size(), nb, P.kdim));
        ctx->rotation_tail_launches++;
    }
    return CRM_OK;
}

int ScanPass::plan_rotations(const Block& B, const GemmProblem* all) {
    const int mode0 = P.fastT && P.wb() ? form("rho0_positions", 1) : 0;
    const int modeT = P.fastT && P.kin() && !form("kr_no_tail", 0) ? form("rotation_tails", 1) : 0;
    bool cand[CRM_MAX_RHO] = {false};
    int rem[CRM_MAX_RHO] = {0}, n_cand = 0, n_rem = 0;
    for (int i = 0; i < nrho; i++) {
        const GemmProblem& p = all[i];
        cand[i] = mode0 > 0 && bg->rho[i] == 0.0 && bg->r[i] > 0 && bg->wb_kept == bg->r[i];
        const int m = p.N % 128;
        if (modeT > 0 && p.N >= 1024 && m > 0 && m <= 16 && p.ldx % 2 == 0 && (reinterpret_cast<uintptr_t>(p.X) & 15) == 0) rem[i] = m;
        n_cand += cand[i] ? 1 : 0;
    }
    for (int i = 0; i < nrho; i++) n_rem += rem[i] > 0 ? 1 : 0;
    auto rounds = [&](bool drop, bool tails) {
        int widths[CRM_MAX_RHO], cnt = 0;
        bool is_cut[CRM_MAX_RHO] = {false};
        long acc = 0, r = 0;
        for (int i = 0; i < nrho; i++)
            if (!(drop && cand[i])) widths[cnt++] = all[i].N - (tails ? rem[i] : 0);
        if (cnt > 0) cut_choice(B.nb, cnt, widths, is_cut, acc, r);
        return r;
    };
    const bool can0 = n_cand > 0, canT = n_rem > 0, force0 = mode0 >= 2 && can0, forceT = modeT >= 2 && canT;
    bool drop = force0, tails = forceT;
    long best = rounds(drop, tails);
    for (int pick = 1; pick < 4; pick++) {
        const bool d = force0 || (can0 && (pick & 1)), t = forceT || (canT && (pick & 2));
        const long r = rounds(d, t);
        if (r < best) { best = r; drop = d; tails = t; }
    }
// ... 147 lines not shown
```

### cellregmap_amd/csrc/scan_pairs.hip

```cpp
#include "scan_pass.h"

namespace crm {

SubRange ScanPass::sub_range(const Block& B, int b0) const {
    SubRange R;
    R.b0 = b0;
    R.nb = B.nb - b0;
    R.done = B.done + b0;
    if (ng > 1) {
        long pairs = 0;
        int take = 0;
        for (; b0 + take < B.nb; take++) {
            unsigned seen = 0;
            for (int gi = 0; gi < ng; gi++) {
                const NullFitOut& f = h_fit[(size_t)gi * P.BLK + b0 + take];
                if (!no_kinship_term(f)) seen |= 1u << f.rho_index;
            }
            const int here = __builtin_popcount(seen);
            if (take > 0 && pairs + here > P.pair_cap) break;
            pairs += here;
        }
        R.nb = take;
    }
    return R;
}

int ScanPass::select_pairs(const Block& B, const SubRange& R, Pairs& Q) {
    const int nb = R.nb, BLK = P.BLK;
    const NullFitOut* fit = h_fit.data() + R.b0;
    std::fill(pair_of.begin(), pair_of.end(), -1);
    long with_pair = 0;
    for (int gi = 0; gi < ng; gi++)
        for (int b = 0; b < nb; b++) {
            const NullFitOut& f = fit[(size_t)gi * BLK + b];
            if (no_kinship_term(f)) continue;
            pair_of[(size_t)f.rho_index * BLK + b] = 0;
            with_pair++;
        }
    ctx->tests_without_pair += (long)ng * nb - with_pair;
    if (with_pair == 0) pair_of[(size_t)fit[0].rho_index * BLK] = 0;
    for (int i = 0; i < nrho; i++) {
        Q.start[i] = Q.npairs;
        for (int b = 0; b < nb; b++) {
            if (pair_of[(size_t)i * BLK + b] == 0) {
                pair_of[(size_t)i * BLK + b] = Q.npairs;
                h_ord[Q.npairs++] = b;
            }
        }
        Q.cnt[i] = Q.npairs - Q.start[i];
    }
    Q.start[nrho] = Q.npairs;
    for (int gi = 0; gi < ng; gi++)
        for (int b = 0; b < nb; b++) {
            const NullFitOut& f = fit[(size_t)gi * BLK + b];
            h_pos[(size_t)gi * BLK + b] = no_kinship_term(f) ? -1 : pair_of[(size_t)f.rho_index * BLK + b];
        }
    if (P.wb_block && ng == 1) {
        for (int b = 0; b < nb; b++)
            if (h_pos[b] >= 0) h_pos[b] = b;
        CRM_HIP(hipMemcpyAsync(d_pos, h_pos.data(), sizeof(int) * (size_t)BLK, hipMemcpyHostToDevice, st));
        return CRM_OK;
    }
    CRM_HIP(hipMemcpyAsync(d_pos, h_pos.data(), sizeof(int) * (size_t)BLK * ng, hipMemcpyHostToDevice, st));
    if (P.wb() && ng > 1) {
        std::vector<int> h_posw((size_t)BLK * ng, -1);
        for (int gi = 0; gi < ng; gi++)
            for (int b = 0; b < nb; b++)
                if (h_pos[(size_t)gi * BLK + b] >= 0) h_posw[(size_t)gi * BLK + b] = b;
        CRM_HIP(hipMemcpyAsync(d_posw, h_posw.data(), sizeof(int) * h_posw.size(), hipMemcpyHostToDevice, st));
        CRM_HIP(hipStreamSynchronize(st));
    }
    CRM_HIP(hipMemcpyAsync(d_ord, h_ord.data(), sizeof(int) * Q.npairs, hipMemcpyHostToDevice, st));
    return launch_gather_block(st, B.Gt + R.b0, P.ldb, P.xrows, P.xrows, nullptr, d_ord, Q.npairs, ctx->ws_Gs.as<double>(),
                               P.ldp, (int)P.ldp);
}

int ScanPass::direct_splits(const Pairs& Q, AGroups& A, bool* tail_of) {
    A.a_slab = (size_t)P.pair_cap * k0 * P.ldA;
    long row_tiles = 0;
    int mn = 1;
    for (int i = 0; i < nrho; i++)
        if (Q.cnt[i] > 0) { row_tiles += ((long)Q.cnt[i] * k0 + GEMM_BM - 1) / GEMM_BM; mn = std::max(mn, bg->r[i]); }
    const int cap = (int)std::min<size_t>(8, ((size_t)16 << 30) / std::max<size_t>(sizeof(double) * A.a_slab, 1));
    A.kr_split = kr_split_for(ctx, row_tiles, mn, 1, np, std::max(cap, 1));
    if (A.kr_split > 1) CRM_TRY(ctx->ws_A.ensure(sizeof(double) * A.a_slab * A.kr_split));
    if (A.kr_split > 1 || !ctx->tune.glds || ctx->tune.bn == 64 || ctx->tune.bn == 160 || form("kr_no_tail", 0)) return CRM_OK;
    long tail_row_tiles = 0, main_tiles = 0;
    for (int i = 0; i < nrho; i++) {
        if (Q.cnt[i] == 0) continue;
        const int N = bg->r[i], rem = N % 128;
        const long rt = ((long)Q.cnt[i] * k0 + GEMM_BM - 1) / GEMM_BM;
        main_tiles += rt * ((N + 127) / 128);
        if (N >= 1024 && rem > 0 && rem <= 32) {
            tail_of[i] = true;
            tail_row_tiles += rt;
            A.tail_maxn = std::max(A.tail_maxn, 128 + rem);
        }
    }
    if (tail_row_tiles == 0 || main_tiles <= 1024) {
        std::fill(tail_of, tail_of + CRM_MAX_RHO, false);
    } else {
        const int saved_bn = ctx->tune.bn;
        ctx->tune.bn = 160;
        A.tail_split = kr_split_for(ctx, tail_row_tiles, A.tail_maxn, 1, np, std::max(cap, 1));
        ctx->tune.bn = saved_bn;
        if (A.tail_split > 1) CRM_TRY(ctx->ws_A.ensure(sizeof(double) * A.a_slab * A.tail_split));
    }
    return CRM_OK;
}

void ScanPass::a_records(const Pairs& Q, bool via_H, const bool* tail_of, AGroups& A) {
    const double kin_rows = P.folded() ? bg->kin_k1 + bg->kin_groups * (long)bg->kin_k2 : bg->cols;
    for (int i = 0; i < nrho; i++) {
        if (Q.cnt[i] == 0 || P.wb()) continue;
        GemmProblem p{};
        p.X = ctx->ws_Gs.as<double>() + Q.start[i]; p.ldx = P.ldp;
        p.C = ctx->ws_A.as<double>() + (size_t)Q.start[i] * k0 * P.ldA;
        if (P.collapsed()) {
            p.Y = tab->Bd.as<double>() + (size_t)i * P.mp * k0 * ldq; p.ldy = (long)k0 * ldq; p.ldc = (long)k0 * P.ldA;
            p.M = Q.cnt[i]; p.N = (int)((long)k0 * ldq);
        } else if (via_H) {
            if (P.kin() && ng == 1) {
                p.X = (P.folded() ? ctx->ws_S.as<double>() : ctx->ws_AH.as<double>()) + (size_t)Q.start[i] * k0; p.ldx = P.ld_ah;
            } else {
                p.X = ctx->ws_XG.as<double>() + (size_t)Q.start[i] * k0; p.ldx = P.ld_xg;
            }
            p.Y = P.folded() ? bg->MixK[i].as<double>() : bg->Mix[i].as<double>(); p.ldy = ldq; p.ldc = P.ldA;
            p.M = Q.cnt[i] * k0; p.N = bg->r[i] > 0 ? bg->r[i] : 1;
            A.kr_flops += 2.0 * kin_rows * (double)bg->r[i] * (double)k0 * (double)Q.cnt[i];
        } else {
            p.E = d_Ep; p.lde = g0->ld_ep; p.k0 = k0; p.Y = bg->Q0[i].as<double>(); p.ldy = ldq; p.ldc = P.ldA;
            p.M = Q.cnt[i] * k0; p.N = bg->r[i] > 0 ? bg->r[i] : 1;
            A.kr_flops += 2.0 * (double)n * (double)bg->r[i] * (double)k0 * (double)Q.cnt[i];
            if (tail_of[i]) {
                GemmProblem t = p;
                const int rem = 128 + p.N % 128;
                p.N -= rem;
                t.Y = p.Y + p.N; t.C = p.C + p.N; t.N = rem;
                A.tails.push_back(t);
            }
        }
        if (P.kin() && p.N >= 1024 && p.N % 128 > 0 && p.N % 128 <= 16 && p.ldx % 2 == 0 &&
            (reinterpret_cast<uintptr_t>(p.X) & 15) == 0 && !form("kr_no_tail", 0)) {
            GemmProblem t = p;
            const int rem = p.N % 128;
            A.kr_flops -= 2.0 * kin_rows * (double)rem * (double)k0 * (double)Q.cnt[i];
            p.N -= rem;
            t.Y = p.Y + p.N; t.C = p.C + p.N; t.N = rem;
            A.spectrum_tails.push_back(t);
        }
        A.max_m = std::max(A.max_m, p.M);
        A.max_n = std::max(A.max_n, p.N);
        probs[A.nz++] = p;
    }
}

int ScanPass::donor_columns(const Block& B, const SubRange& R, const Pairs& Q, DonorCols& D) {
    D.in_pair_order = ng == 1 && !P.wb_block;
    D.G = D.in_pair_order ? ctx->ws_Gs.as<double>() : B.Gt + R.b0;
    D.ldg = D.in_pair_order ? P.ldp : P.ldb;
    D.ncol = D.in_pair_order ? Q.npairs : R.nb;
    const int blk_cols = (int)(P.ldb - R.b0);
    return launch_gather_rows(st, D.G, D.ldg, bg->kin_map.as<int>(), bg->kin_rows, D.in_pair_order ? (int)D.ldg : blk_cols,
                              ctx->ws_Gk.as<double>(), D.ldg);
}
int ScanPass::gather_pairs(const double* src, long rows, const Pairs& Q) {
    const int xg_cols = (int)std::min<long>(P.ld_xg, round_up((long)Q.npairs * k0, 128) + 128);
    return launch_gather_slabs(st, src, P.ld_ah, rows, d_ord, Q.npairs, k0, ctx->ws_XG.as<double>(), P.ld_xg, xg_cols);
}

int ScanPass::folded_S(const Block& B, const SubRange& R, const Pairs& Q) {
    DonorCols D;
    CRM_TRY(donor_columns(B, R, Q, D));
    double* S = ctx->ws_S.as<double>();
    double* Gk = ctx->ws_Gk.as<double>();
    const int k1 = bg->kin_k1, k2 = bg->kin_k2, ncol = D.ncol, npair = P.npair;
    const long groups = bg->kin_groups, ld_ah = P.ld_ah;
    std::vector<GemmProblem> kp((size_t)groups + P.fold_split6);
    GemmProblem p{};
    p.X = Gk; p.ldx = D.ldg;
    if (probed.donor_pairs) {
        p.Y = g0->kinEE.as<double>(); p.ldy = g0->ld_ee; p.C = ctx->ws_Pd.as<double>(); p.ldc = P.ldPd;
        p.M = ncol; p.N = npair;
    } else if (k2 == 1) {
        p.Y = g0->kinUE.as<double>(); p.ldy = g0->ld_ep; p.C = S + (size_t)k1 * ld_ah; p.ldc = k0; p.M = ncol; p.N = k0;
    } else {
        p.E = g0->kinEp.as<double>(); p.lde = g0->ld_ep; p.k0 = k0; p.Y = bg->kin_Y.as<double>(); p.ldy = bg->kin_ldy;
        p.C = S + (size_t)k1 * ld_ah; p.ldc = ld_ah; p.M = ncol * k0; p.N = k2;
    }
    const long maxlen = donor_run_records(bg, p, probed.donor_pairs ? P.pd_slab : (long)k2 * ld_ah, kp.data());
    const long stages_all = np / GEMM_BK, per = (stages_all + P.fold_split6 - 1) / P.fold_split6;
    const long e1_slab = (long)k1 * ld_ah;
    int slices = 0;
    long chunk_max = GEMM_BK;
    if (P.e1_pairs) {
        GemmProblem& e = kp[groups];
        e.X = D.G; e.ldx = D.ldg; e.Y = g0->kinP.as<double>(); e.ldy = P.ldP;
        e.C = ctx->ws_AH.as<double>(); e.ldc = P.ldP; e.M = ncol; e.N = k1 * k0;
        if (probed.e1_sym) { e.Y = d_EE; e.ldy = g0->ld_ee; e.N = npair; }
    }
    for (int sps = 0; sps < P.fold_split6 && !P.e1_pairs; sps++) {
        const long s0 = sps * per, s1 = std::min(stages_all, s0 + per);
        if (s1 <= s0) break;
        GemmProblem& e = kp[groups + slices++];
        e.X = D.G + s0 * GEMM_BK * D.ldg; e.ldx = D.ldg;
        e.E = d_Ep + s0 * GEMM_BK * g0->ld_ep; e.lde = g0->ld_ep; e.k0 = k0;
        e.Y = bg->H.as<double>() + s0 * GEMM_BK * bg->ldh; e.ldy = bg->ldh;
        e.C = ctx->ws_AH.as<double>() + (size_t)sps * e1_slab; e.ldc = ld_ah;
        e.M = ncol * k0; e.N = k1; e.cells = (s1 - s0) * GEMM_BK;
        chunk_max = std::max(chunk_max, e.cells);
    }
    kp.resize((size_t)groups + std::max(slices, 1));
    return with_records(SLOT_KIN, kp, [&](GemmProblem* d_kp) -> int {
        double* AH = ctx->ws_AH.as<double>();
        if (probed.donor_pairs) {
            CRM_TRY(launch_gemm_tn(ctx, d_kp, (int)groups, ncol, npair, maxlen, false, 0, 1, 0));
            if (probed.wb_rotate)
                CRM_TRY(launch_donor_pairs_rotate(st, ctx->ws_Pd.as<double>(), P.pd_slab, P.ldPd, (int)groups, ncol, k0,
                                                  bg->wb_U.as<double>(), (long)bg->wb_k2pad * 128, 128, bg->wb_k2pad,
                                                  ctx->ws_A.as<double>(), P.ldAw, AH, P.pd_slab, P.donor_pair_splits));
            else
                CRM_TRY(launch_donor_pairs_expand(st, ctx->ws_Pd.as<double>(), P.pd_slab, P.ldPd, (int)groups, ncol, k0, k1, S, ld_ah,
                                                  AH, P.pd_slab, P.donor_pair_splits));
            CRM_TRY(launch_reduce_splits(st, AH, (long)ncol * P.ldPd, P.donor_pair_splits, P.pd_slab));
            CRM_TRY(launch_pair_rows_sym(st, AH, P.ldPd, ncol, k0, S, ld_ah));
            ctx->donor_pair_blocks++;
        } else {
            if (k2 == 1) CRM_TRY(launch_gemm_tn(ctx, d_kp, (int)groups, ncol, k0, maxlen, false, 0, 1, 0));
            else CRM_TRY(launch_kr_transposed(ctx, d_kp, (int)groups, ncol * k0, k2, maxlen, k0));
            if (P.e1_pairs) {
                const long p_slab = (long)(std::max<long>(P.BLK, P.pair_cap) + 128) * P.ldP;
                CRM_TRY(launch_gemm_tn(ctx, d_kp + groups, 1, ncol, probed.e1_sym ? npair : k1 * k0, np, false, 0, P.fold_split6, p_slab));
                CRM_TRY(launch_reduce_splits(st, AH, (long)ncol * P.ldP, P.fold_split6, p_slab));
                if (probed.e1_sym) CRM_TRY(launch_pair_rows_sym(st, AH, P.ldP, ncol, k0, S, ld_ah));
                else CRM_TRY(launch_pair_rows(st, AH, P.ldP, ncol, k1, k0, S, ld_ah));
            } else {
                CRM_TRY(launch_kr_transposed(ctx, d_kp + groups, slices, ncol * k0, k1, chunk_max, k0));
                CRM_TRY(launch_reduce_splits(st, AH, e1_slab, slices, e1_slab));
                CRM_HIP(hipMemcpyAsync(S, AH, sizeof(double) * (size_t)e1_slab, hipMemcpyDeviceToDevice, st));
            }
        }
        if (!D.in_pair_order && !P.wb()) CRM_TRY(gather_pairs(S, P.kdim, Q));
        return CRM_OK;
    });
}

int ScanPass::unfolded_AH(const Block& B, const SubRange& R, const Pairs& Q) {
    DonorCols D;
    CRM_TRY(donor_columns(B, R, Q, D));
    double* S = ctx->ws_S.as<double>();
    double* AH = ctx->ws_AH.as<double>();
    const int k1 = bg->kin_k1, k2 = bg->kin_k2, ncol = D.ncol, npair = P.npair;
    const long groups = bg->kin_groups, mk = bg->kin_cols, KK = P.KK, ld_ah = P.ld_ah;
    GemmProblem p{};
    p.X = ctx->ws_Gk.as<double>(); p.ldx = D.ldg;
    if (probed.pairs_unfolded) {
        double* Pd = ctx->ws_Pd.as<double>();
        double* Z = S;
        std::vector<GemmProblem> kp((size_t)groups + 1);
        p.Y = g0->kinEE.as<double>(); p.ldy = g0->ld_ee; p.C = Pd; p.ldc = P.ldPd; p.M = ncol; p.N = npair;
        const long maxlen = donor_run_records(bg, p, P.pd_slab, kp.data());
        GemmProblem& z = kp[groups];
        z.X = bg->kin_hKd.as<double>(); z.ldx = bg->kin_ldh;
        z.Y = Pd; z.ldy = P.pd_slab; z.C = Z; z.ldc = P.pd_slab; z.M = (int)mk + 1; z.N = (int)((long)ncol * P.ldPd);
        return with_records(SLOT_KIN, kp, [&](GemmProblem* d_kp) -> int {
            CRM_TRY(launch_gemm_tn(ctx, d_kp, (int)groups, ncol, npair, maxlen, false, 0, 1, 0));
            CRM_TRY(launch_gemm_tn(ctx, d_kp + groups, 1, (int)mk + 1, (int)((long)ncol * P.ldPd), bg->kin_groups_pad, false, 0, 1, 0));
            CRM_TRY(launch_donor_pairs_expand(st, Z, P.pd_slab, P.ldPd, (int)mk, ncol, k0, k1, AH, ld_ah, Pd, P.pd_slab, 1, 1, mk));
            CRM_TRY(launch_pair_rows_sym(st, Z + (size_t)mk * P.pd_slab, P.ldPd, ncol, k0, AH, ld_ah));
            ctx->donor_pair_blocks++;
            if (!D.in_pair_order) CRM_TRY(gather_pairs(AH, bg->ldh, Q));
            return CRM_OK;
        });
    }
    std::vector<GemmProblem> kp((size_t)groups + k2);
    p.E = g0->kinEp.as<double>(); p.lde = g0->ld_ep; p.k0 = k0; p.Y = bg->kin_Y.as<double>(); p.ldy = bg->kin_ldy;
    p.C = S; p.ldc = ld_ah; p.M = ncol * k0; p.N = (int)KK;
    const long maxlen = donor_run_records(bg, p, KK * ld_ah, kp.data());
    for (int j = 0; j < k2; j++) {
        GemmProblem& q = kp[groups + j];
        q.X = bg->kin_hKd.as<double>(); q.ldx = bg->kin_ldh; q.Y = S + (size_t)j * ld_ah; q.ldy = KK * ld_ah;
        q.C = AH + (size_t)(k1 + (long)j * mk) * ld_ah; q.ldc = ld_ah; q.M = (int)mk; q.N = ncol * k0;
    }
    return with_records(SLOT_KIN, kp, [&](GemmProblem* d_kp) -> int {
        CRM_TRY(launch_kr_transposed(ctx, d_kp, (int)groups, ncol * k0, (int)KK, maxlen, k0));
        CRM_TRY(launch_gemm_tn(ctx, d_kp + groups, k2, (int)mk, ncol * k0, bg->kin_groups_pad, false, 0, 1, 0));
        CRM_TRY(launch_kin_sum_e1(st, S, ld_ah, (int)KK, k2, k1, (int)groups, (long)ncol * k0, AH, ld_ah));
        if (!D.in_pair_order) CRM_TRY(gather_pairs(AH, bg->ldh, Q));
        return CRM_OK;
    });
}

int ScanPass::direct_AH(const Block& B, const SubRange& R, const Pairs& Q, AGroups& A) {
    GemmProblem p{};
    p.X = B.Gt + R.b0; p.ldx = P.ldb; p.E = d_Ep; p.lde = g0->ld_ep; p.k0 = k0; p.Y = bg->H.as<double>(); p.ldy = bg->ldh;
    p.C = ctx->ws_AH.as<double>(); p.ldc = P.ld_ah; p.M = R.nb * k0; p.N = (int)bg->cols;
    CRM_TRY(upload(SLOT_ONE, &p, 1));
    CRM_TRY(launch_kr_transposed(ctx, d_probs + SLOT_ONE, 1, p.M, p.N, np, k0));
    A.kr_flops += 2.0 * (double)n * (double)bg->cols * (double)k0 * (double)R.nb;
    return gather_pairs(ctx->ws_AH.as<double>(), bg->ldh, Q);
}

int ScanPass::woodbury_S(const SubRange& R, const Pairs& Q) {
    const long groups = bg->kin_groups;
    const int ncol = P.wb_block ? R.nb : Q.npairs;
    std::vector<GemmProblem> kp((size_t)groups);
    GemmProblem p{};
    p.X = ctx->ws_S.as<double>() + (size_t)bg->kin_k1 * P.ld_ah; p.ldx = P.ld_ah;
    p.C = ctx->ws_A.as<double>(); p.ldc = P.ldAw; p.M = ncol * k0;
    woodbury_records(bg, p, (long)bg->kin_k2 * P.ld_ah, kp.data());
    return with_records(SLOT_KIN, kp, [&](GemmProblem* d_kp) {
        return launch_gemm_tn(ctx, d_kp, (int)groups, ncol * k0, bg->kin_k2, bg->wb_k2pad, false, 0, 1, 0);
    });
}

int ScanPass::form_A(const Block& B, const SubRange& R, const Pairs& Q) {
    bool via_H = P.kin();
    if (P.fastT && ng > 1 && !P.kin()) {
        double direct = 0.0, via = (double)R.nb * (double)bg->cols * (double)n;
        for (int i = 0; i < nrho; i++) {
            direct += (double)Q.cnt[i] * bg->r[i] * (double)n;
            via += (double)Q.cnt[i] * bg->r[i] * (double)bg->ldh;
        }
        via_H = ctx->tune.shared_h < 0 ? via < 0.9 * direct : ctx->tune.shared_h > 0;
    }
    const bool direct = !P.collapsed() && !via_H;
    if (direct)
        for (int i = 0; i < nrho; i++)
            if (Q.cnt[i] > 0) CRM_TRY(crm_background_require_q0(bg, i));
    AGroups A;
    bool tail_of[CRM_MAX_RHO] = {false};
    if (direct) CRM_TRY(direct_splits(Q, A, tail_of));
    a_records(Q, via_H, tail_of, A);
    const bool timing = !P.wb() && ctx->timing && ctx->timed_used < 65536;
    if (timing) CRM_TRY(timer_open(!P.kin()));
    if (P.folded()) CRM_TRY(folded_S(B, R, Q));
    else if (P.kin()) CRM_TRY(unfolded_AH(B, R, Q));
    else if (via_H) CRM_TRY(direct_AH(B, R, Q, A));
    CRM_TRY(upload(SLOT_ONE, probs.data(), A.nz));
    GemmProblem* d_A = d_probs + SLOT_ONE;
    if (P.collapsed()) {
        CRM_TRY(launch_gemm_tn(ctx, d_A, A.nz, A.max_m, (int)((long)k0 * ldq), P.mp, false, 0, 1, 0));
    } else if (P.wb()) {
        if (!probed.wb_rotate) CRM_TRY(woodbury_S(R, Q));
    } else if (P.kin()) {
        if (timing) CRM_HIP(hipEventRecord(ctx->timed[ctx->timed_used].first, st));
        struct Restore { crm_ctx* c; ~Restore() { c->tune.tag = 0; } } restore{ctx};
        ctx->tune.tag = 1;
        CRM_TRY(launch_gemm_tn(ctx, d_A, A.nz, A.max_m, A.max_n, P.kdim, false, 0, 1, 0));
    } else if (via_H) {
        CRM_TRY(launch_gemm_tn(ctx, d_A, A.nz, A.max_m, A.max_n, P.kdim, false, 0, 1, 0));
    } else {
        CRM_TRY(launch_gemm_tn(ctx, d_A, A.nz, A.max_m, A.max_n, np, true, k0, A.kr_split, (long)A.a_slab));
        CRM_TRY(launch_reduce_splits(st, ctx->ws_A.as<double>(), (long)Q.npairs * k0 * P.ldA, A.kr_split, (long)A.a_slab));
        if (!A.tails.empty()) {
            const int saved_bn = ctx->tune.bn;
            ctx->tune.bn = 160;
            struct Restore { crm_ctx* c; int bn; ~Restore() { c->tune.bn = bn; } } restore{ctx, saved_bn};
            CRM_TRY(upload(A.nz, A.tails.data(), A.tails.size()));
            CRM_TRY(launch_gemm_tn(ctx, d_probs + A.nz, (int)A.tails.size(), A.max_m, A.tail_maxn, np, true, k0, A.tail_split, (long)A.a_slab));
            ctx->tail_launches++;
            for (const GemmProblem& t : A.tails)
                CRM_TRY(launch_reduce_splits_band(st, t.C, (long)t.M, t.ldc, 0, t.N, A.tail_split, (long)A.a_slab));
        }
    }
    if (timing) {
        CRM_TRY(timer_close());
        ctx->kr_flops += A.kr_flops;
    }
    if (!A.spectrum_tails.empty()) {
        CRM_TRY(upload(A.nz, A.spectrum_tails.data(), A.spectrum_tails.size()));
        CRM_TRY(launch_skinny_tn(st, d_probs + A.nz, (int)A.spectrum_tails.size(), A.max_m, P.kdim));
        ctx->spectrum_tail_launches++;
        CRM_HIP(hipStreamSynchronize(st));
    }
    return CRM_OK;
}

int ScanPass::side_contractions(const Block& B, const SubRange& R) {
    const long ldb = P.ldb;
    const int nb = R.nb;
    double* const Gt = B.Gt + R.b0;
    double* G2 = ctx->ws_G2.as<double>();
    double* GG = !P.collapsed() ? ctx->ws_GG.as<double>() : nullptr;
    CRM_TRY(launch_square_block(st, Gt, B.Gx + R.b0, ldb, ldb, P.xrows, (int)(ldb - R.b0), G2, GG, ldb));
    if (!GG) GG = G2;
    const int s2 = P.collapsed() ? 1 : P.ks2, s3 = P.collapsed() ? 1 : P.ks3;
    GemmProblem p{};
    p.ldx = ldb; p.M = nb;
    p.X = GG; p.Y = P.collapsed() ? tab->Z2.as<double>() : d_Ep; p.ldy = g0->ld_ep; p.C = dZ2; p.ldc = P.ldZ2; p.N = k0;
    probs[1] = p;
    p.X = G2; p.Y = P.collapsed() ? tab->Z3.as<double>() : d_EE; p.ldy = g0->ld_ee; p.C = dZ3; p.ldc = P.ldZ3; p.N = P.npair;
    probs[2] = p;
    CRM_TRY(upload(SLOT_RHO, probs.data() + 1, 2));
    if (P.cross) {
        CRM_TRY(launch_donor_cross(st, nb, B.Gb + R.b0, ldb, (int)panel->m, tab->Z2.as<double>(), P.ldZ2, k0, dZ2, P.ldZ2));
    } else {
        CRM_TRY(launch_gemm_tn(ctx, d_probs + SLOT_RHO, 1, nb, k0, P.xrows, false, 0, s2, z2_sz));
        CRM_TRY(launch_reduce_splits(st, dZ2, z2_sz, s2, z2_sz));
    }
    CRM_TRY(launch_gemm_tn(ctx, d_probs + SLOT_RHO + 1, 1, nb, P.npair, P.xrows, false, 0, s3, z3_sz));
    return launch_reduce_splits(st, dZ3, z3_sz, s3, z3_sz);
}

int ScanPass::z1_products(const Block& B, const SubRange& R) {
    const int s1 = P.collapsed() ? 1 : P.ks1;
    std::vector<GemmProblem> zp((size_t)ng);
    for (int gi = 0; gi < ng; gi++) {
        crm_gene* g = genes[gi];
        GemmProblem& p = zp[(size_t)gi];
        p.X = B.Gt + R.b0; p.ldx = P.ldb; p.Y = P.collapsed() ? g->dt_Z1.as<double>() : g->YE.as<double>(); p.ldy = g->ld_ye;
        p.C = dZ1 + (size_t)gi * z1_sz * P.ks1; p.ldc = P.ldZ1; p.M = R.nb; p.N = k0 * (1 + c);
    }
    CRM_TRY(upload(P.z1_slot(), zp.data(), zp.size()));
    CRM_TRY(launch_gemm_tn(ctx, d_probs + P.z1_slot(), ng, R.nb, k0 * (1 + c), P.xrows, false, 0, s1, z1_sz));
    for (int gi = 0; gi < ng; gi++)
        CRM_TRY(launch_reduce_splits(st, dZ1 + (size_t)gi * z1_sz * P.ks1, z1_sz, s1, z1_sz));
    return CRM_OK;
}

}
```

### cellregmap_amd/csrc/scan_pass.h

```cpp
#pragma once
#include <algorithm>
#include <vector>

#include "nullfit.h"
#include "objects.h"

namespace crm {

int ctx_cus(const crm_ctx* ctx);

constexpr double COLLINEAR_TAU = 1e-2;

constexpr double STOP_SHIFT_C = 2.5e-13;
constexpr double FLAT_KAPPA = 1.0;
constexpr double RHO_KAPPA = 1.0;
constexpr int FLAT_REC = 10;

struct ScanOut {
    double *pv, *rho1, *e2, *g2, *eps2, *Q, *lml, *delta, *scale, *lambda, *F;
    int* ifault = nullptr;
    double* liu = nullptr;
    int* flags = nullptr;
    double* bound_Q = nullptr;
    double* bound_p = nullptr;
    bool exact = false;
    double* logp = nullptr;
    int* status = nullptr;
};

enum class Route {
    collapsed,
    direct,
    kin_unfolded,
    kin_folded,
    unrelated,
};

constexpr int SLOT_ONE = 0, SLOT_RHO = 1, SLOT_KIN = 2 * CRM_MAX_RHO + 4;

struct ScanPlan {
    Route route = Route::direct;
    bool fastT = false, slow_forms = false, skip_pairs = true, cross = false;
    bool e1_pairs = false, e1_sym = false, donor_pairs = false, wb_rotate = false, pairs_unfolded = false;
    bool wb_block = false;
    int ng = 1, BLK = 0, pair_cap = 0;
    long ldb = 0, ldp = 0, ldA = 0, ldAw = 0, ldT = 0, ldZ1 = 0, ldZ2 = 0, ldZ3 = 0, ld_ah = 0, ld_xg = 0, ldP = 0, ldPd = 0,
         pd_slab = 0, ldwb = 0, ld_gW = 0, th_slab = 0, s_rows = 0;
    size_t s_bytes = 0;
    int ks1 = 1, ks2 = 1, ks3 = 1, ks_h = 1, fold_split6 = 1, fold_split3 = 1, donor_pair_splits = 1;
    int npair = 0, KT = 0, KK = 0, kin_probs = 0;
    long kdim = 0, mp = 0, xrows = 0;
    bool collapsed() const { return route == Route::collapsed; }
    bool kin() const { return route == Route::kin_unfolded || route == Route::kin_folded || route == Route::unrelated; }
    bool folded() const { return route == Route::kin_folded || route == Route::unrelated; }
    bool wb() const { return route == Route::unrelated; }
    bool through_H() const { return fastT && (ng > 1 || kin()); }
    int z1_slot() const { return SLOT_KIN + kin_probs; }
};

int scan_block_variants(const crm_ctx* ctx, const crm_gene* g0, long count);
ScanPlan plan_scan(const std::vector<crm_gene*>& genes, const crm_panel* panel, const int* idx_G, bool allow_collapse,
                   long count);

long donor_run_records(const crm_background* bg, const GemmProblem& p, long c_step, GemmProblem* out);
void woodbury_records(const crm_background* bg, const GemmProblem& p, long x_step, GemmProblem* out);
struct SameColumns { const double* A; long lda; const double* B; long ldb; long rows; };
int same_columns(hipStream_t st, int* d_flag, int k, std::initializer_list<SameColumns> pairs, bool& same);

struct Block {
    long done = 0, col0 = 0;
    int nb = 0;
    double* Gb = nullptr;
    double* Gt = nullptr;
    double* Gx = nullptr;
    std::vector<double> flat_obj;
};
struct SubRange {
    int b0 = 0, nb = 0;
    long done = 0;
};
struct Pairs {
    int cnt[CRM_MAX_RHO] = {0}, start[CRM_MAX_RHO + 1] = {0}, npairs = 0;
};
struct AGroups {
    int nz = 0, max_m = 0, max_n = 1, kr_split = 1, tail_split = 1, tail_maxn = 0;
    double kr_flops = 0.0;
    size_t a_slab = 0;
    std::vector<GemmProblem> tails, spectrum_tails;
};
struct DonorCols { bool in_pair_order; const double* G; long ldg; int ncol; };

struct ScanPass {
    const std::vector<crm_gene*>& genes;
    crm_panel* panel;
    const long first, count;
    const int *idx_E, *idx_G;
    const std::vector<ScanOut>& outs;
    std::vector<long>* near_out;
    const int ng;
    crm_gene* const g0;
    crm_background* const bg;
    crm_ctx* const ctx;
    const hipStream_t st;
    const long n, np, ldq, slab;
    const int nrho, c, k0;
    const ScanPlan P;
    struct Probed { bool e1_sym, donor_pairs, pairs_unfolded, wb_rotate; } probed{P.e1_sym, P.donor_pairs, P.pairs_unfolded, P.wb_rotate};
    int *d_idxE = nullptr, *d_idxG = nullptr;
    const double *d_Ep = nullptr, *d_EE = nullptr;
    crm_donor_tables* tab = nullptr;
    GemmProblem* d_probs = nullptr;
    double *dZ1 = nullptr, *dZ2 = nullptr, *dZ3 = nullptr;
    long z1_sz = 0, z2_sz = 0, z3_sz = 0;
    double *d_gg, *d_gy, *d_gW, *d_Q, *d_pv, *d_lam, *d_liu, *d_part, *d_coef, *d_thr, *d_tp, *d_tlp;
    int *d_pos, *d_ord, *d_if, *d_drop, *d_near, *d_posw, *d_tst;
    NullFitTrial* d_trial;
    NullFitOut* d_fit;
    unsigned* d_queue;
    double *wb_yW = nullptr, *wb_E1yW = nullptr, *wb_g = nullptr, *wb_Gw = nullptr, *wb_tmp = nullptr;
    std::vector<NullFitOut> h_fit = std::vector<NullFitOut>((size_t)P.BLK * ng);
    std::vector<int> h_pos = std::vector<int>((size_t)P.BLK * ng), h_ord = std::vector<int>(P.pair_cap);
    std::vector<GemmProblem> probs = std::vector<GemmProblem>(CRM_MAX_RHO + 4);
    std::vector<int> pair_of = std::vector<int>((size_t)nrho * P.BLK), h_near = std::vector<int>(P.BLK);
    bool rho0_pos[CRM_MAX_RHO] = {false};
    std::vector<GemmProblem> rot_tails;
    std::vector<GemmProblem> phi_recs;

    ScanPass(const std::vector<crm_gene*>& genes_, crm_panel* panel_, long first_, long count_, const int* idx_E_,
             const int* idx_G_, const std::vector<ScanOut>& outs_, bool allow_collapse, std::vector<long>* near_out_)
        : genes(genes_), panel(panel_), first(first_), count(count_), idx_E(idx_E_), idx_G(idx_G_), outs(outs_),
          near_out(near_out_), ng((int)genes_.size()), g0(genes_[0]), bg(g0->bg), ctx(bg->ctx), st(ctx->stream), n(bg->n),
          np(bg->n_pad), ldq(bg->ldq), slab((long)(1 + g0->c) * bg->ldq), nrho(bg->nrho), c(g0->c), k0(g0->k0),
          P(plan_scan(genes_, panel_, idx_G_, allow_collapse, count_)) {}

    int upload(int slot, const GemmProblem* p, size_t k) {
        CRM_HIP(hipMemcpyAsync(d_probs + slot, p, sizeof(GemmProblem) * k, hipMemcpyHostToDevice, st));
        return CRM_OK;
    }
    template <class F>
    int with_records(int slot, const std::vector<GemmProblem>& kp, F&& launches) {
        CRM_TRY(upload(slot, kp.data(), kp.size()));
        CRM_TRY(launches(d_probs + slot));
        CRM_HIP(hipStreamSynchronize(st));
        return CRM_OK;
    }
    int timer_open(bool record_start) {
        if (ctx->timed_used == ctx->timed.size()) {
            hipEvent_t a, b;
            CRM_HIP(hipEventCreate(&a));
            CRM_HIP(hipEventCreate(&b));
            ctx->timed.emplace_back(a, b);
        }
        if (record_start) CRM_HIP(hipEventRecord(ctx->timed[ctx->timed_used].first, st));
        return CRM_OK;
    }
    int timer_close() {
        CRM_HIP(hipEventRecord(ctx->timed[ctx->timed_used].second, st));
        ctx->timed_used++;
        return CRM_OK;
    }
    bool no_kinship_term(const NullFitOut& f) const {
        return P.skip_pairs && f.v1 > 0.0 && f.v0 >= 0.0 && f.v0 * bg->s0_max[f.rho_index] <= 1e-10 * f.v1;
    }

    int workspaces();
    int context_features(bool shared_too);
    int prepare_contexts();
    int prepare_kinship();
    int prepare_woodbury();
    int copy_block(Block& B);
    int block_stats(Block& B);
    int fold_TH(const Block& B);
    int unfolded_TH(const Block& B);
    int plain_TH(const Block& B);
    bool cut_choice(int nb, int cnt, const int* N, bool* is_cut, long& acc, long& rounds) const;
    int cut_rotations(const Block& B, int n_list, int& n_main);
    int rotations(const Block& B);
    int plan_rotations(const Block& B, const GemmProblem* all);
    int null_fits(const Block& B);
    int replay_block(const Block& B);
    int woodbury_phi(const Block& B);
    int collect_fits(Block& B);
    SubRange sub_range(const Block& B, int b0) const;
    int select_pairs(const Block& B, const SubRange& R, Pairs& Q);
    int direct_splits(const Pairs& Q, AGroups& A, bool* tail_of);
    void a_records(const Pairs& Q, bool via_H, const bool* tail_of, AGroups& A);
    int donor_columns(const Block& B, const SubRange& R, const Pairs& Q, DonorCols& D);
    int gather_pairs(const double* src, long rows, const Pairs& Q);
    int folded_S(const Block& B, const SubRange& R, const Pairs& Q);
    int unfolded_AH(const Block& B, const SubRange& R, const Pairs& Q);
    int direct_AH(const Block& B, const SubRange& R, const Pairs& Q, AGroups& A);
    int woodbury_S(const SubRange& R, const Pairs& Q);
    int form_A(const Block& B, const SubRange& R, const Pairs& Q);
    int side_contractions(const Block& B, const SubRange& R);
    int z1_products(const Block& B, const SubRange& R);
    int flat_probes(const Block& B, const SubRange& R, int gi, const AssembleArgs& aa, double* slow_ws, std::vector<char>& flat,
                    std::vector<double>& probe_rec);
    int gene_results(const Block& B, const SubRange& R, int gi);
};

}
```

### cellregmap_amd/csrc/scan_prepare.hip

```cpp
#include "scan_pass.h"

namespace crm {

long donor_run_records(const crm_background* bg, const GemmProblem& p, long c_step, GemmProblem* out) {
    long maxlen = GEMM_BK;
    for (long d = 0; d < bg->kin_groups; d++) {
        const long r0 = bg->kin_row0[d];
        GemmProblem q = p;
        q.X = p.X + r0 * p.ldx;
        if (p.E) q.E = p.E + r0 * p.lde;
        q.Y = p.Y + r0 * p.ldy; q.C = p.C + d * c_step; q.cells = bg->kin_len[d];
        maxlen = std::max(maxlen, bg->kin_len[d]);
        out[d] = q;
    }
    return maxlen;
}

void woodbury_records(const crm_background* bg, const GemmProblem& p, long x_step, GemmProblem* out) {
    for (long d = 0; d < bg->kin_groups; d++) {
        GemmProblem q = p;
        q.X = p.X + d * x_step; q.Y = bg->wb_U.as<double>() + (size_t)d * bg->wb_k2pad * 128; q.ldy = 128;
        q.C = p.C + d * bg->kin_k2; q.N = bg->kin_k2; q.cells = bg->wb_k2pad;
        out[d] = q;
    }
}

int same_columns(hipStream_t st, int* d_flag, int k, std::initializer_list<SameColumns> pairs, bool& same) {
    int h_flag = 0;
    CRM_HIP(hipMemsetAsync(d_flag, 0, sizeof(int), st));
    for (const SameColumns& q : pairs) CRM_TRY(launch_same_columns(st, q.A, q.lda, q.B, q.ldb, q.rows, k, d_flag));
    CRM_HIP(hipMemcpyAsync(&h_flag, d_flag, sizeof(int), hipMemcpyDeviceToHost, st));
    CRM_HIP(hipStreamSynchronize(st));
    same = h_flag == 0;
    return CRM_OK;
}

int ScanPass::workspaces() {
    const int BLK = P.BLK, max_pairs = P.pair_cap;
    const long ldb = P.ldb;
    CRM_TRY(ctx->ws_T.ensure(sizeof(double) * (size_t)nrho * BLK * P.ldT));
    CRM_TRY(ctx->ws_A.ensure(sizeof(double) * (size_t)(P.wb() ? std::max(max_pairs, BLK) : max_pairs) * k0 * P.ldAw));
    CRM_TRY(ctx->ws_Anone.ensure(sizeof(double) * (size_t)P.ldAw));
    CRM_HIP(hipMemsetAsync(ctx->ws_Anone.ptr, 0, sizeof(double) * (size_t)P.ldAw, st));
    CRM_TRY(ctx->ws_Gb.ensure(sizeof(double) * (size_t)np * ldb));
    CRM_TRY(ctx->ws_Gs.ensure(sizeof(double) * (size_t)np * P.ldp));
    CRM_TRY(ctx->ws_G2.ensure(sizeof(double) * (size_t)np * ldb));
    if (idx_G)
        CRM_TRY(ctx->ws_Gt.ensure(sizeof(double) * (size_t)np * ldb));
    z1_sz = (long)BLK * P.ldZ1, z2_sz = (long)BLK * P.ldZ2, z3_sz = (long)BLK * P.ldZ3;
    const long z1_all = z1_sz * P.ks1 * ng;
    CRM_TRY(ctx->ws_Z.ensure(sizeof(double) * (size_t)(z1_all + z2_sz * P.ks2 + z3_sz * P.ks3)));
    dZ1 = ctx->ws_Z.as<double>();
    dZ2 = dZ1 + z1_all;
    dZ3 = dZ2 + z2_sz * P.ks2;
    if (bg->fast_T) {
        CRM_TRY(ctx->ws_TH.ensure(sizeof(double) * (size_t)P.th_slab * P.ks_h));
        CRM_HIP(hipMemsetAsync(ctx->ws_TH.ptr, 0, sizeof(double) * (size_t)P.th_slab, st));
    }
    CRM_TRY(ctx->ws_F.ensure(sizeof(double) * (size_t)BLK * k0 * k0));
    CRM_TRY(ctx->ws_Gext.ensure(sizeof(double) * (size_t)BLK * P.KT * P.KT));
    if (c > CRM_MAX_COV_WIDE || P.slow_forms) {
        size_t xw = c > CRM_MAX_COV_WIDE ? nullfit_xwide_scratch_doubles(BLK, nrho, c) : 0;
        if (P.slow_forms) xw = std::max(xw, std::max(assemble_rows_scratch_doubles(BLK, k0, c), eig_scratch_doubles(BLK, k0)));
        CRM_TRY(ctx->ws_xwide.ensure(sizeof(double) * xw));
    }
    const size_t stats_ws = variant_stats_workspace(BLK, std::min(c, CRM_MAX_COV));
    auto carve_small = [&](char* base) {
        size_t off = 0;
        auto carve = [&](auto*& ptr, size_t bytes) {
            ptr = base ? reinterpret_cast<std::remove_reference_t<decltype(ptr)>>(base + off) : nullptr;
            off += (bytes + 255) / 256 * 256;
        };
        carve(d_gg, sizeof(double) * BLK), carve(d_gy, sizeof(double) * BLK * ng);
        carve(d_gW, sizeof(double) * BLK * P.ld_gW), carve(d_trial, sizeof(NullFitTrial) * BLK * nrho);
        carve(d_fit, sizeof(NullFitOut) * BLK * ng), carve(d_pos, sizeof(int) * BLK * ng), carve(d_ord, sizeof(int) * max_pairs);
        carve(d_Q, sizeof(double) * BLK), carve(d_pv, sizeof(double) * BLK), carve(d_lam, sizeof(double) * BLK * k0);
        carve(d_if, sizeof(int) * BLK), carve(d_liu, sizeof(double) * BLK), carve(d_part, stats_ws);
        carve(d_queue, sizeof(unsigned) * CRM_MAX_RHO);
        carve(d_coef, sizeof(double) * (size_t)c * ldb);
        carve(d_thr, sizeof(double) * BLK);
        carve(d_drop, sizeof(int) * BLK);
        carve(d_near, sizeof(int) * BLK);
        carve(d_posw, sizeof(int) * BLK * ng);
        carve(d_tp, sizeof(double) * BLK), carve(d_tlp, sizeof(double) * BLK), carve(d_tst, sizeof(int) * BLK);
        return off;
    };
    CRM_TRY(ctx->ws_small.ensure(carve_small(nullptr)));
    carve_small(ctx->ws_small.as<char>());
    CRM_TRY(ctx->ws_probs.ensure(sizeof(GemmProblem) * (P.z1_slot() + ng)));
    d_probs = ctx->ws_probs.as<GemmProblem>();
    if (!P.collapsed()) {
        CRM_TRY(ctx->ws_Gx.ensure(sizeof(double) * (size_t)np * ldb));
        CRM_TRY(ctx->ws_GG.ensure(sizeof(double) * (size_t)np * ldb));
    }
    if (P.through_H()) {
        if (P.folded()) {
            CRM_TRY(ctx->ws_AH.ensure(sizeof(double) * (size_t)P.fold_split6 *
                                      (P.e1_pairs ? (size_t)(std::max<long>(BLK, max_pairs) + 128) * P.ldP : (size_t)bg->kin_k1 * P.ld_ah)));
        } else {
            CRM_TRY(ctx->ws_AH.ensure(sizeof(double) * (size_t)bg->ldh * P.ld_ah));
        }
        if (ng > 1) CRM_TRY(ctx->ws_XG.ensure(sizeof(double) * (size_t)P.kdim * P.ld_xg));
    }
    const long KK = P.KK;
    if (P.folded()) {
        CRM_TRY(ctx->ws_S.ensure(P.s_bytes));
        CRM_TRY(ctx->ws_Gk.ensure(sizeof(double) * (size_t)bg->kin_rows * std::max(ldb, P.ldp)));
        CRM_TRY(ctx->ws_S2.ensure(sizeof(double) * (size_t)P.fold_split3 * bg->kin_k1 * ldb));
        const long used = bg->kin_k1 + bg->kin_groups * (long)bg->kin_k2;
        if (P.s_rows > used)
            CRM_HIP(hipMemsetAsync(ctx->ws_S.as<double>() + (size_t)used * P.ld_ah, 0, sizeof(double) * (size_t)(P.s_rows - used) * P.ld_ah, st));
    } else if (P.kin()) {
        CRM_TRY(ctx->ws_S.ensure(P.s_bytes));
        CRM_TRY(ctx->ws_Gk.ensure(sizeof(double) * (size_t)bg->kin_rows * std::max(ldb, P.ldp)));
        CRM_TRY(ctx->ws_S2.ensure(sizeof(double) * (size_t)bg->kin_groups_pad * KK * ldb));
        if (bg->kin_groups_pad > bg->kin_groups)
            CRM_HIP(hipMemsetAsync(ctx->ws_S2.as<double>() + (size_t)bg->kin_groups * KK * ldb, 0,
                                   sizeof(double) * (size_t)(bg->kin_groups_pad - bg->kin_groups) * KK * ldb, st));
        if (bg->kin_groups_pad > bg->kin_groups)
            CRM_HIP(hipMemsetAsync(ctx->ws_S.as<double>() + (size_t)bg->kin_groups * KK * P.ld_ah, 0,
                                   sizeof(double) * (size_t)(bg->kin_groups_pad - bg->kin_groups) * KK * P.ld_ah, st));
    }
    if (P.wb()) {
        const long brows = bg->kin_groups * bg->kin_k2 + GEMM_BK, kt = P.KT + bg->kin_k1;
        const size_t n_yW = (size_t)ng * (1 + c) * P.ldwb, n_E1 = (size_t)ng * bg->kin_k1 * 128, n_g = (size_t)BLK * P.ldwb,
                     n_Gw = (size_t)BLK * kt * kt, n_tmp = (size_t)(bg->kin_rows + brows) * 128;
        CRM_TRY(ctx->ws_WB.ensure(sizeof(double) * (n_yW + n_E1 + n_g + n_Gw + n_tmp)));
        wb_yW = ctx->ws_WB.as<double>();
        wb_E1yW = wb_yW + n_yW;
        wb_g = wb_E1yW + n_E1;
        wb_Gw = wb_g + n_g;
        wb_tmp = wb_Gw + n_Gw;
    }
    return CRM_OK;
}

int ScanPass::context_features(bool shared_too) {
    for (int gi = 0; gi < ng; gi++) {
        crm_gene* g = genes[gi];
        const bool both = gi == 0 && shared_too;
        CRM_TRY(g->YE.ensure(sizeof(double) * np * g->ld_ye));
        if (both) {
            CRM_TRY(g->Ep.ensure(sizeof(double) * np * g->ld_ep));
            CRM_TRY(g->EE.ensure(sizeof(double) * np * g->ld_ee));
        }
        CRM_TRY(launch_context_features(st, g->E0.as<double>(), g->lde, d_idxE, n, np, k0, g->yW.as<double>(),
                                        g->yW.as<double>() + 1, g->ld_yw, c,
                                        both ? g->Ep.as<double>() : nullptr, g->ld_ep, g->YE.as<double>(),
                                        g->ld_ye, both ? g->EE.as<double>() : nullptr, g->ld_ee));
    }
    if (shared_too) {
        d_Ep = g0->Ep.as<double>();
        d_EE = g0->EE.as<double>();
    }
    return CRM_OK;
}

int ScanPass::prepare_contexts() {
    CRM_TRY(g0->idx.ensure(sizeof(int) * 2 * n));
    if (idx_E) {
        d_idxE = g0->idx.as<int>();
        CRM_HIP(hipMemcpyAsync(d_idxE, idx_E, sizeof(int) * n, hipMemcpyHostToDevice, st));
    }
    if (idx_G) {
        d_idxG = g0->idx.as<int>() + n;
        CRM_HIP(hipMemcpyAsync(d_idxG, idx_G, sizeof(int) * n, hipMemcpyHostToDevice, st));
    }
    for (crm_gene* g : genes) {
        g->ld_ep = round_up(k0, 128);
        g->ld_ye = P.ldZ1;
        g->ld_ee = P.ldZ3;
    }
    if (!P.collapsed()) return context_features(true);
    const double* Zt = panel->Z.as<double>();
    if (P.cross) {
        CRM_TRY(g0->dt_Zt.ensure(sizeof(double) * (size_t)np * panel->ldz + sizeof(int) * n));
        int* gperm = reinterpret_cast<int*>(g0->dt_Zt.as<double>() + (size_t)np * panel->ldz);
        CRM_TRY(launch_permute_group(st, panel->group.as<int>(), d_idxG, n, gperm));
        CRM_TRY(launch_indicator(st, gperm, n, np, (int)panel->m, g0->dt_Zt.as<double>(), panel->ldz));
        Zt = g0->dt_Zt.as<double>();
    }
    const bool reusable = !idx_E && !idx_G;
    bool build_shared = false;
    if (reusable) {
        for (crm_donor_tables* t : bg->dt_cache)
            if (t->e0_key == g0->e0_key && t->group_key == panel->group_key) tab = t;
        if (!tab) {
            if ((int)bg->dt_cache.size() >= crm_background::DT_CACHE) {
                size_t lru = 0;
                for (size_t i = 1; i < bg->dt_cache.size(); i++)
                    if (bg->dt_cache[i]->stamp < bg->dt_cache[lru]->stamp) lru = i;
                tab = bg->dt_cache[lru];
            } else {
                tab = new crm_donor_tables();
                bg->dt_cache.push_back(tab);
            }
            tab->e0_key = 0;
            build_shared = true;
        }
        tab->stamp = ++bg->dt_clock;
    } else {
        tab = &g0->dt_own;
        build_shared = true;
    }
    CRM_TRY(context_features(build_shared));
    for (int gi = 0; gi < ng; gi++) {
        crm_gene* g = genes[gi];
        const bool have = reusable && g->dt_group == panel->group_key && !(gi == 0 && build_shared);
        if (!have) {
            g->dt_group = 0;
            CRM_TRY(build_donor_tables(g, panel, (gi == 0 && build_shared) ? tab : nullptr, d_Ep, d_EE, Zt, P.cross));
            if (reusable) g->dt_group = panel->group_key;
        }
    }
    if (build_shared && reusable) {
        tab->e0_key = g0->e0_key;
        tab->group_key = panel->group_key;
    }
    return CRM_OK;
}

int ScanPass::prepare_kinship() {
    const long ldh = bg->ldh;
    const double* H = bg->H.as<double>();
    if (P.kin()) {
        CRM_TRY(g0->kinEp.ensure(sizeof(double) * (size_t)bg->kin_rows * g0->ld_ep));
        CRM_TRY(launch_gather_rows(st, d_Ep, g0->ld_ep, bg->kin_map.as<int>(), bg->kin_rows, (int)g0->ld_ep,
                                   g0->kinEp.as<double>(), g0->ld_ep));
    }
    if (P.folded() && bg->kin_k2 == 1) {
        CRM_TRY(g0->kinUE.ensure(sizeof(double) * (size_t)bg->kin_rows * g0->ld_ep));
        CRM_TRY(launch_scale_rows(st, g0->kinEp.as<double>(), g0->ld_ep, bg->kin_Y.as<double>(), bg->kin_ldy, bg->kin_rows,
                                  (int)g0->ld_ep, g0->kinUE.as<double>(), g0->ld_ep));
    }
    const SameColumns e1_is_E{H, ldh, d_Ep, g0->ld_ep, n};
    const SameColumns us_is_E{bg->kin_Y.as<double>(), bg->kin_ldy, g0->kinEp.as<double>(), g0->ld_ep, bg->kin_rows};
    if (probed.e1_sym) CRM_TRY(same_columns(st, d_near, k0, {e1_is_E}, probed.e1_sym));
    if (P.e1_pairs && !probed.e1_sym) {
        CRM_TRY(g0->kinP.ensure(sizeof(double) * (size_t)np * P.ldP));
        CRM_TRY(launch_pair_features(st, H, ldh, bg->kin_k1, d_Ep, g0->ld_ep, k0, np, g0->kinP.as<double>(), P.ldP));
    }
    probed.donor_pairs = probed.donor_pairs && probed.e1_sym;
    if (probed.donor_pairs) CRM_TRY(same_columns(st, d_near, k0, {us_is_E}, probed.donor_pairs));
    if (probed.pairs_unfolded) CRM_TRY(same_columns(st, d_near, k0, {e1_is_E, us_is_E}, probed.pairs_unfolded));
    probed.wb_rotate = probed.wb_rotate && probed.donor_pairs;
    if (probed.donor_pairs || probed.pairs_unfolded) {
        CRM_TRY(g0->kinEE.ensure(sizeof(double) * (size_t)bg->kin_rows * g0->ld_ee));
        CRM_TRY(launch_gather_rows(st, d_EE, g0->ld_ee, bg->kin_map.as<int>(), bg->kin_rows, (int)g0->ld_ee, g0->kinEE.as<double>(),
                                   g0->ld_ee));
        CRM_TRY(ctx->ws_Pd.ensure(sizeof(double) * (size_t)(probed.donor_pairs ? bg->kin_groups : bg->kin_groups_pad) * P.pd_slab));
    }
    if (probed.donor_pairs)
        CRM_TRY(ctx->ws_AH.ensure(sizeof(double) * (size_t)std::max<long>(P.donor_pair_splits, P.fold_split6) *
                                  (size_t)std::max<long>(P.pd_slab, (std::max<long>(P.BLK, P.pair_cap) + 128) * P.ldP)));
    if (probed.pairs_unfolded && bg->kin_groups_pad > bg->kin_groups)
        CRM_HIP(hipMemsetAsync(ctx->ws_Pd.as<double>() + (size_t)bg->kin_groups * P.pd_slab, 0,
                               sizeof(double) * (size_t)(bg->kin_groups_pad - bg->kin_groups) * P.pd_slab, st));
    if (P.through_H() && !P.folded()) {
        if (probed.pairs_unfolded && ldh > bg->cols)
            CRM_HIP(hipMemsetAsync(ctx->ws_AH.as<double>() + (size_t)bg->cols * P.ld_ah, 0, sizeof(double) * (size_t)(ldh - bg->cols) * P.ld_ah, st));
        else if (!probed.pairs_unfolded)
            CRM_HIP(hipMemsetAsync(ctx->ws_AH.ptr, 0, sizeof(double) * (size_t)ldh * P.ld_ah, st));
    }
    return CRM_OK;
}

int ScanPass::prepare_woodbury() {
    if (!P.wb()) return CRM_OK;
    const int k2 = bg->kin_k2, k1 = bg->kin_k1;
    const long groups = bg->kin_groups, brows = groups * k2 + GEMM_BK;
    const size_t n_yW1 = (size_t)(1 + c) * P.ldwb, n_E11 = (size_t)k1 * 128;
    double* yWk = wb_tmp;
    double* Bk = yWk + (size_t)bg->kin_rows * 128;
    for (int gi = 0; gi < ng; gi++) {
        crm_gene* g = genes[gi];
        if (g->wb_gen != bg->wb_gen) {
            CRM_TRY(g->wb_yW.ensure(sizeof(double) * (n_yW1 + n_E11)));
            CRM_HIP(hipMemsetAsync(g->wb_yW.ptr, 0, sizeof(double) * (n_yW1 + n_E11), st));
            CRM_HIP(hipMemsetAsync(Bk, 0, sizeof(double) * (size_t)brows * 128, st));
            CRM_TRY(launch_gather_rows(st, g->yW.as<double>(), g->ld_yw, bg->kin_map.as<int>(), bg->kin_rows, 1 + c, yWk, 128));
            std::vector<GemmProblem> kp((size_t)2 * groups);
            GemmProblem p{};
            p.X = bg->kin_Y.as<double>(); p.ldx = bg->kin_ldy; p.Y = yWk; p.ldy = 128; p.C = Bk; p.ldc = 128;
            p.M = k2; p.N = 1 + c;
            const long maxlen = donor_run_records(bg, p, (long)k2 * 128, kp.data());
            GemmProblem q{};
            q.X = Bk; q.ldx = 128; q.C = g->wb_yW.as<double>(); q.ldc = P.ldwb; q.M = 1 + c;
            woodbury_records(bg, q, (long)k2 * 128, kp.data() + groups);
            GemmProblem e{};
            e.X = bg->H.as<double>(); e.ldx = bg->ldh; e.Y = g->yW.as<double>(); e.ldy = g->ld_yw;
            e.C = g->wb_yW.as<double>() + n_yW1; e.ldc = 128; e.M = k1; e.N = 1 + c;
            CRM_TRY(with_records(SLOT_KIN, kp, [&](GemmProblem* d_kp) -> int {
                CRM_TRY(launch_gemm_tn(ctx, d_kp, (int)groups, k2, 1 + c, maxlen, false, 0, 1, 0));
                CRM_TRY(launch_gemm_tn(ctx, d_kp + groups, (int)groups, 1 + c, k2, bg->wb_k2pad, false, 0, 1, 0));
                CRM_TRY(upload(SLOT_ONE, &e, 1));
                return launch_gemm_tn(ctx, d_probs + SLOT_ONE, 1, k1, 1 + c, np, false, 0, 1, 0);
            }));
            g->wb_gen = bg->wb_gen;
        }
        CRM_HIP(hipMemcpyAsync(wb_yW + (size_t)gi * n_yW1, g->wb_yW.as<double>(), sizeof(double) * n_yW1, hipMemcpyDeviceToDevice, st));
        CRM_HIP(hipMemcpyAsync(wb_E1yW + (size_t)gi * n_E11, g->wb_yW.as<double>() + n_yW1, sizeof(double) * n_E11,
                               hipMemcpyDeviceToDevice, st));
    }
    return CRM_OK;
}

}
```

Baseline: 75250.

## Fuse per-block copy, orthogonalize, square and kinship gather; cache per-gene tables

Blocks that are aligned in the panel now read genotypes in place, with no copy into a workspace. A single block_pass kernel computes the orthogonalized Gx, G², G·Gx and the kinship-gathered rows, replacing separate gather, square and ortho launches. Per-gene context tables (YE, Ep, kinEp, kinEE, pair features, same-columns probes) and the TH zeroing are now cached across calls under generation-stamp keys, so repeat scans skip rebuilding them. This adds complexity and a risk of stale caches if a key misses an input that changed.

```diff
diff --git a/cellregmap_amd/_lib.py b/cellregmap_amd/_lib.py
--- a/cellregmap_amd/_lib.py
+++ b/cellregmap_amd/_lib.py
@@ -84,6 +84,7 @@
     "crm_test_donor_pair_blocks": (ctypes.c_long, [vp]),
     "crm_test_unrelated_donor_blocks": (ctypes.c_int, [vp, ctypes.POINTER(ctypes.c_long)]),
     "crm_test_gram_dma_launches": (ctypes.c_int, [vp, ctypes.POINTER(ctypes.c_long)]),
+    "crm_test_fused_blocks": (ctypes.c_int, [vp, ctypes.POINTER(ctypes.c_long)]),
     "crm_test_rho0_position_blocks": (ctypes.c_int, [vp, ctypes.POINTER(ctypes.c_long)]),
     "crm_test_rotation_tail_launches": (ctypes.c_int, [vp, ctypes.POINTER(ctypes.c_long)]),
     "crm_test_tests_without_pair": (ctypes.c_long, [vp]),
diff --git a/cellregmap_amd/csrc/api_core.hip b/cellregmap_amd/csrc/api_core.hip
--- a/cellregmap_amd/csrc/api_core.hip
+++ b/cellregmap_amd/csrc/api_core.hip
@@ -115,6 +115,8 @@
         return CRM_ERR_HIP;
     }
     bytes = need;
+    static std::atomic<unsigned long> allocations{0};
+    serial = ++allocations;
     g_live_bytes += (long)need;
     hipStream_t fs = fill_stream();
     CRM_HIP(hipMemsetAsync(ptr, poison_mode() ? 0xFF : 0, total, fs));
@@ -157,6 +159,7 @@
     g_live_bytes -= (long)bytes;
     ptr = nullptr;
     bytes = 0;
+    serial = 0;
 }
 
 int upload_padded(hipStream_t st, double* dst, long ld_dst, long rows_pad, const double* src,
@@ -293,7 +296,7 @@
                       {"pairs_without_kinship_term", 0, false}, {"flat_kappa_milli", 0, false}, {"chase_abort", 0, false}, {"nullfit_one_per_wave", 0, false},
                       {"kin_diag", 0, false}, {"donor_pairs_rotate", 0, false}, {"rho0_positions", 0, false},
                       {"rotation_tails", 0, false}, {"woodbury_ytY", 0, false},
-                      {"wb_block_order", 0, false}};
+                      {"wb_block_order", 0, false}, {"block_fused", 0, false}};
 std::mutex g_forms_mu;
 }
 int form(const char* name, int otherwise) {
@@ -339,6 +342,14 @@
     return crm::guarded("crm_test_unrelated_donor_blocks", [&]() -> int {
     if (!ctx || !blocks) return CRM_ERR_ARG;
     *blocks = ctx->unrelated_donor_blocks;
+    return CRM_OK;
+    });
+}
+
+int crm_test_fused_blocks(const crm_ctx* ctx, long* blocks) {
+    return crm::guarded("crm_test_fused_blocks", [&]() -> int {
+    if (!ctx || !blocks) return CRM_ERR_ARG;
+    *blocks = ctx->fused_blocks;
     return CRM_OK;
     });
 }
diff --git a/cellregmap_amd/csrc/blockops.hip b/cellregmap_amd/csrc/blockops.hip
--- a/cellregmap_amd/csrc/blockops.hip
+++ b/cellregmap_amd/csrc/blockops.hip
@@ -389,6 +389,38 @@
     Gx[i * ldx + b] = v;
 }
 
+__global__ __launch_bounds__(256) void block_pass_kernel(const double* __restrict__ G, long ldg, long cells, long cells_pad,
+                                                        int variants, const double* __restrict__ W, long ldw, int c,
+                                                        const double* __restrict__ coef, long ld_coef, int cols,
+                                                        double* __restrict__ Gx, double* __restrict__ G2, double* __restrict__ GG,
+                                                        long ld_out, const int* __restrict__ inv, const int* __restrict__ pad_rows,
+                                                        double* __restrict__ Gkx, double* __restrict__ Gkt, int chunks) {
+    long i;
+    int chunk;
+    row_and_chunk(chunks, i, chunk);
+    const int b = chunk * blockDim.x + threadIdx.x;
+    if (b >= cols) return;
+    if (i >= cells_pad) {
+        const long k = pad_rows[i - cells_pad];
+        Gkx[k * ld_out + b] = 0.0;
+        if (Gkt) Gkt[k * ld_out + b] = 0.0;
+        return;
+    }
+    const double g = i < cells && b < variants ? G[i * ldg + b] : 0.0;
+    double v = g;
+    for (int j = 0; j < c; j++) v = fma(-W[i * ldw + j], coef[(long)j * ld_coef + b], v);
+    Gx[i * ld_out + b] = v;
+    G2[i * ld_out + b] = g * g;
+    GG[i * ld_out + b] = g * v;
+    if (inv) {
+        const long k = inv[i];
+        if (k >= 0) {
+            Gkx[k * ld_out + b] = v;
+            if (Gkt) Gkt[k * ld_out + b] = g;
+        }
+    }
+}
+
 __global__ void ortho_rank_kernel(const double* __restrict__ gg, const double* __restrict__ thr, int variants,
                                   int* __restrict__ drop) {
     const int b = blockIdx.x * blockDim.x + threadIdx.x;
@@ -420,6 +452,21 @@
     const int chunks = (cols + 255) / 256;
     hipLaunchKernelGGL(ortho_apply_kernel, row_chunk_grid(cells_pad, chunks), dim3(256), 0, st, G, ldg, W,
                        ldw, c, coef, ld_coef, cols, Gx, ldx, chunks);
+    CRM_HIP(hipGetLastError());
+    return CRM_OK;
+}
+
+int launch_block_pass(hipStream_t st, const double* G, long ldg, long cells, long cells_pad, int variants, int cols,
+                      const double* W, long ldw, int c, const double* proj, const double* gW, long ld_gW, double* coef,
+                      long ld_coef, double* thr, double* Gx, double* G2, double* GG, long ld_out, const int* inv,
+                      const int* pad_rows, long pads, double* Gkx, double* Gkt) {
+    if (cols <= 0) return CRM_OK;
+    hipLaunchKernelGGL(ortho_coef_kernel, dim3((cols + 255) / 256), dim3(256), 0, st, gW, ld_gW, proj, c, variants, cols,
+                       coef, ld_coef, thr);
+    CRM_HIP(hipGetLastError());
+    const int chunks = (cols + 255) / 256;
+    hipLaunchKernelGGL(block_pass_kernel, row_chunk_grid(cells_pad + (inv ? pads : 0), chunks), dim3(256), 0, st, G, ldg, cells,
+                       cells_pad, variants, W, ldw, c, coef, ld_coef, cols, Gx, G2, GG, ld_out, inv, pad_rows, Gkx, Gkt, chunks);
     CRM_HIP(hipGetLastError());
     return CRM_OK;
 }
diff --git a/cellregmap_amd/csrc/crm_internal.h b/cellregmap_amd/csrc/crm_internal.h
--- a/cellregmap_amd/csrc/crm_internal.h
+++ b/cellregmap_amd/csrc/crm_internal.h
@@ -23,15 +23,16 @@
 struct DevBuf {
     void* ptr = nullptr;
     size_t bytes = 0;
+    unsigned long serial = 0;
     DevBuf() = default;
     DevBuf(const DevBuf&) = delete;
     DevBuf& operator=(const DevBuf&) = delete;
-    DevBuf(DevBuf&& o) noexcept : ptr(o.ptr), bytes(o.bytes) { o.ptr = nullptr; o.bytes = 0; }
+    DevBuf(DevBuf&& o) noexcept : ptr(o.ptr), bytes(o.bytes), serial(o.serial) { o.ptr = nullptr; o.bytes = 0; o.serial = 0; }
     DevBuf& operator=(DevBuf&& o) noexcept {
         if (this != &o) {
             release();
-            ptr = o.ptr; bytes = o.bytes;
-            o.ptr = nullptr; o.bytes = 0;
+            ptr = o.ptr; bytes = o.bytes; serial = o.serial;
+            o.ptr = nullptr; o.bytes = 0; o.serial = 0;
         }
         return *this;
     }
@@ -94,6 +95,7 @@
     long donor_pair_blocks = 0;
     long rotation_tail_launches = 0;
     long rho0_position_blocks = 0;
+    long fused_blocks = 0;
     long unrelated_donor_blocks = 0;
     long gram_dma_launches = 0;
     long tests_without_pair = 0;
@@ -123,11 +125,20 @@
     crm::DevBuf ws_xwide;
     crm::DevBuf ws_Tcut;
     crm::DevBuf ws_Gk, ws_S, ws_S2;
+    struct ThKey {
+        unsigned long serial = 0, stamp = 0;
+        int route = -1, ks_h = 0;
+        long ldb = 0, th_slab = 0;
+        bool operator==(const ThKey& o) const {
+            return serial == o.serial && stamp == o.stamp && route == o.route && ks_h == o.ks_h && ldb == o.ldb && th_slab == o.th_slab;
+        }
+    } th_key;
+    crm::DevBuf ws_Gkt;
     crm::DevBuf ws_WB;
     crm::DevBuf ws_Pd;
     crm::DevBuf ws_Anone;
     std::vector<crm::DevBuf*> all_bufs() {
-        return {&sync_counters, &ws_xwide, &ws_Tcut, &ws_S, &ws_S2, &ws_Gk, &ws_Pd, &ws_WB, &ws_Anone, &ws_AH, &ws_XG, &ws_TH, &ws_T, &ws_A, &ws_Gb, &ws_Gx, &ws_Gs, &ws_G2, &ws_GG, &ws_Gt, &ws_Z, &ws_small, &ws_probs, &ws_F, &ws_Gext};
+        return {&sync_counters, &ws_xwide, &ws_Tcut, &ws_S, &ws_S2, &ws_Gk, &ws_Gkt, &ws_Pd, &ws_WB, &ws_Anone, &ws_AH, &ws_XG, &ws_TH, &ws_T, &ws_A, &ws_Gb, &ws_Gx, &ws_Gs, &ws_G2, &ws_GG, &ws_Gt, &ws_Z, &ws_small, &ws_probs, &ws_F, &ws_Gext};
     }
 };
 
diff --git a/cellregmap_amd/csrc/kinship.hip b/cellregmap_amd/csrc/kinship.hip
--- a/cellregmap_amd/csrc/kinship.hip
+++ b/cellregmap_amd/csrc/kinship.hip
@@ -161,6 +161,7 @@
     crm_ctx* ctx = bg->ctx;
     CRM_HIP(hipSetDevice(ctx->device));
     hipStream_t st = ctx->stream;
+    bg->kin_gen = next_stamp();
     bg->kin = false;
     struct Undo {
         crm_background* b;
@@ -168,7 +169,7 @@
             if (b->kin) return;
             b->kin_fold = false;
             b->kin_wb = false;
-            for (DevBuf* x : {&b->kin_map, &b->kin_Y, &b->kin_hKd, &b->wb_U, &b->wb_R, &b->wb_EE}) x->release();
+            for (DevBuf* x : {&b->kin_map, &b->kin_inv, &b->kin_Y, &b->kin_hKd, &b->wb_U, &b->wb_R, &b->wb_EE}) x->release();
             for (int i = 0; i < b->nrho; i++) b->wb_S0[i].release();
             for (int i = 0; i < b->nrho; i++) b->MixK[i].release();
         }
@@ -189,6 +190,12 @@
         const long d = group[i];
         map[bg->kin_row0[d] + fill[d]++] = (int)i;
     }
+    std::vector<int> inv((size_t)bg->n_pad + (size_t)(rows - n), -1);
+    for (long k = 0, pads = 0; k < rows; k++) {
+        if (map[k] >= 0) inv[map[k]] = (int)k;
+        else inv[(size_t)bg->n_pad + pads++] = (int)k;
+    }
+    bg->kin_pads = rows - n;
     bg->kin_rows = rows;
     bg->kin_groups = groups;
     bg->kin_groups_pad = round_up(groups, GEMM_BK);
@@ -202,7 +209,9 @@
     CRM_TRY(bg->kin_hKd.ensure(sizeof(double) * bg->kin_groups_pad * bg->kin_ldh));
     DevBuf dU;
     CRM_TRY(dU.ensure(sizeof(double) * n * k2));
+    CRM_TRY(bg->kin_inv.ensure(sizeof(int) * inv.size()));
     CRM_HIP(hipMemcpyAsync(bg->kin_map.ptr, map.data(), sizeof(int) * rows, hipMemcpyHostToDevice, st));
+    CRM_HIP(hipMemcpyAsync(bg->kin_inv.ptr, inv.data(), sizeof(int) * inv.size(), hipMemcpyHostToDevice, st));
     CRM_HIP(hipMemcpyAsync(dU.ptr, U, sizeof(double) * n * k2, hipMemcpyHostToDevice, st));
     CRM_TRY(upload_padded(st, bg->kin_hKd.as<double>(), bg->kin_ldh, bg->kin_groups_pad, hKd, m, groups, m));
     CRM_TRY(launch_kin_operand(st, dU.as<double>(), k2, bg->H.as<double>(), bg->ldh, k1, bg->kin_map.as<int>(), rows,
diff --git a/cellregmap_amd/csrc/nullfit.h b/cellregmap_amd/csrc/nullfit.h
--- a/cellregmap_amd/csrc/nullfit.h
+++ b/cellregmap_amd/csrc/nullfit.h
@@ -85,6 +85,10 @@
 int launch_ortho_block(hipStream_t st, const double* G, long ldg, long cells_pad, int variants, int cols,
                        const double* W, long ldw, int c, const double* proj, const double* gW, long ld_gW,
                        double* coef, long ld_coef, double* thr, double* Gx, long ldx);
+int launch_block_pass(hipStream_t st, const double* G, long ldg, long cells, long cells_pad, int variants, int cols,
+                      const double* W, long ldw, int c, const double* proj, const double* gW, long ld_gW, double* coef,
+                      long ld_coef, double* thr, double* Gx, double* G2, double* GG, long ld_out, const int* inv,
+                      const int* pad_rows, long pads, double* Gkx, double* Gkt);
 int launch_ortho_rank(hipStream_t st, const double* gg, const double* thr, int variants, int* drop);
 int launch_collinear_flag(hipStream_t st, const double* gg, const double* gW, long ld_gW, const double* proj, int c,
                           int variants, double tau, int* near);
diff --git a/cellregmap_amd/csrc/objects.h b/cellregmap_amd/csrc/objects.h
--- a/cellregmap_amd/csrc/objects.h
+++ b/cellregmap_amd/csrc/objects.h
@@ -1,4 +1,5 @@
 #pragma once
+#include <atomic>
 #include <cmath>
 #include <memory>
 
@@ -6,6 +7,10 @@
 
 namespace crm {
 constexpr long CELL_PAD = 128;
+inline unsigned long next_stamp() {
+    static std::atomic<unsigned long> made{0};
+    return ++made;
+}
 }
 
 struct crm_donor_tables {
@@ -45,6 +50,9 @@
     long kin_rows = 0;
     std::vector<long> kin_row0, kin_len;
     crm::DevBuf kin_map;
+    crm::DevBuf kin_inv;
+    long kin_pads = 0;
+    unsigned long kin_gen = crm::next_stamp();
     crm::DevBuf kin_Y;
     long kin_ldy = 128;
     crm::DevBuf kin_hKd;
@@ -89,6 +97,16 @@
     crm::DevBuf wb_yW;
     unsigned long wb_gen = 0;
     long ld_ep = 0, ld_ye = 0, ld_ee = 0;
+    struct TableKey {
+        unsigned long stamp = 0;
+        int k0 = 0;
+        long ld_ep = 0, ld_ye = 0, ld_ee = 0;
+        bool operator==(const TableKey& o) const {
+            return stamp == o.stamp && k0 == o.k0 && ld_ep == o.ld_ep && ld_ye == o.ld_ye && ld_ee == o.ld_ee;
+        }
+    } tab_key;
+    bool tab_YE = false, tab_E = false, tab_kinEp = false, tab_kinUE = false, tab_kinP = false, tab_kinEE = false;
+    int tab_e1_is_E = -1, tab_us_is_E = -1;
     unsigned long e0_key = 0;
     unsigned long w_key = 0;
     unsigned long dt_group = 0;
diff --git a/cellregmap_amd/csrc/scan_block.hip b/cellregmap_amd/csrc/scan_block.hip
--- a/cellregmap_amd/csrc/scan_block.hip
+++ b/cellregmap_amd/csrc/scan_block.hip
@@ -20,9 +20,26 @@
     else rows[(size_t)b * ldT + j] = slab[j];
 }
 
+bool ScanPass::fused_pass() const {
+    const bool sub_ranges = ng > 1 && P.pair_cap < (long)std::min(nrho, ng) * P.BLK;
+    return form("block_fused", 1) != 0 && !P.collapsed() && !panel->grouped && !idx_G && panel->n_pad == np && !sub_ranges;
+}
+bool ScanPass::fused_block(long col0, int nb) const {
+    const bool kr_reads_Gt = (P.route == Route::direct && ng > 1) || (P.folded() && !P.e1_pairs);
+    return fused_pass() && col0 % 128 == 0 && col0 + round_up(nb, 128) + (kr_reads_Gt ? 128 : 0) <= panel->ld;
+}
+
 int ScanPass::copy_block(Block& B) {
     const long ldb = P.ldb;
     const int nb = B.nb;
+    B.ldt = ldb;
+    if (fused_block(B.col0, nb)) {
+        B.Gb = B.Gt = panel->G.as<double>() + B.col0;
+        B.ldt = panel->ld;
+        B.fused = true;
+        ctx->fused_blocks++;
+        return CRM_OK;
+    }
     B.Gb = B.Gt = B.Gx = ctx->ws_Gb.as<double>();
     if (P.collapsed()) {
         CRM_TRY(launch_gather_block(st, panel->Gd.as<double>() + B.col0, panel->ld, P.mp, panel->m, nullptr, nullptr, nb, B.Gb, ldb, (int)ldb));
@@ -47,9 +64,17 @@
     const int nb = B.nb, BLK = P.BLK;
     if (!P.collapsed()) {
         B.Gx = ctx->ws_Gx.as<double>();
-        CRM_TRY(launch_variant_stats(st, B.Gb, ldb, np, nb, g0->yW.as<double>(), g0->yW.as<double>() + 1, g0->ld_yw, c, d_part, d_gg, d_gy, d_gW, ld_gW));
-        CRM_TRY(launch_ortho_block(st, B.Gb, ldb, np, nb, (int)ldb, g0->yW.as<double>() + 1, g0->ld_yw, c, g0->Wproj.as<double>(),
-                                   d_gW, ld_gW, d_coef, ldb, d_thr, B.Gx, ldb));
+        CRM_TRY(launch_variant_stats(st, B.Gb, B.ldt, np, nb, g0->yW.as<double>(), g0->yW.as<double>() + 1, g0->ld_yw, c, d_part, d_gg, d_gy, d_gW, ld_gW));
+        if (B.fused) {
+            const bool kin_t = P.kin() && (ng > 1 || P.wb_block);
+            CRM_TRY(launch_block_pass(st, B.Gb, B.ldt, n, np, nb, (int)ldb, g0->yW.as<double>() + 1, g0->ld_yw, c,
+                                      g0->Wproj.as<double>(), d_gW, ld_gW, d_coef, ldb, d_thr, B.Gx, ctx->ws_G2.as<double>(),
+                                      ctx->ws_GG.as<double>(), ldb, P.kin() ? bg->kin_inv.as<int>() : nullptr,
+                                      P.kin() ? bg->kin_inv.as<int>() + np : nullptr, P.kin() ? bg->kin_pads : 0,
+                                      P.kin() ? ctx->ws_Gk.as<double>() : nullptr, kin_t ? ctx->ws_Gkt.as<double>() : nullptr));
+        } else
+            CRM_TRY(launch_ortho_block(st, B.Gb, ldb, np, nb, (int)ldb, g0->yW.as<double>() + 1, g0->ld_yw, c, g0->Wproj.as<double>(),
+                                       d_gW, ld_gW, d_coef, ldb, d_thr, B.Gx, ldb));
     }
     for (int gi = 0; gi < ng; gi++) {
         crm_gene* g = genes[gi];
@@ -71,7 +96,7 @@
     const long groups = bg->kin_groups;
     double* Gk = ctx->ws_Gk.as<double>();
     double* TH = ctx->ws_TH.as<double>();
-    CRM_TRY(launch_gather_rows(st, B.Gx, ldb, bg->kin_map.as<int>(), bg->kin_rows, (int)ldb, Gk, ldb));
+    if (!B.fused) CRM_TRY(launch_gather_rows(st, B.Gx, ldb, bg->kin_map.as<int>(), bg->kin_rows, (int)ldb, Gk, ldb));
     std::vector<GemmProblem> kp((size_t)groups + 1);
     GemmProblem p{};
     p.X = bg->kin_Y.as<double>(); p.ldx = bg->kin_ldy; p.Y = Gk; p.ldy = ldb; p.C = TH + (size_t)k1 * ldb; p.ldc = ldb;
@@ -96,7 +121,7 @@
     const long groups = bg->kin_groups, mk = bg->kin_cols;
     double* Gk = ctx->ws_Gk.as<double>();
     double* S2 = ctx->ws_S2.as<double>();
-    CRM_TRY(launch_gather_rows(st, B.Gx, ldb, bg->kin_map.as<int>(), bg->kin_rows, (int)ldb, Gk, ldb));
+    if (!B.fused) CRM_TRY(launch_gather_rows(st, B.Gx, ldb, bg->kin_map.as<int>(), bg->kin_rows, (int)ldb, Gk, ldb));
     std::vector<GemmProblem> kp((size_t)groups + k2);
     GemmProblem p{};
     p.X = bg->kin_Y.as<double>(); p.ldx = bg->kin_ldy; p.Y = Gk; p.ldy = ldb; p.C = S2; p.ldc = ldb;
diff --git a/cellregmap_amd/csrc/scan_pairs.hip b/cellregmap_amd/csrc/scan_pairs.hip
--- a/cellregmap_amd/csrc/scan_pairs.hip
+++ b/cellregmap_amd/csrc/scan_pairs.hip
@@ -71,7 +71,7 @@
         CRM_HIP(hipStreamSynchronize(st));
     }
     CRM_HIP(hipMemcpyAsync(d_ord, h_ord.data(), sizeof(int) * Q.npairs, hipMemcpyHostToDevice, st));
-    return launch_gather_block(st, B.Gt + R.b0, P.ldb, P.xrows, P.xrows, nullptr, d_ord, Q.npairs, ctx->ws_Gs.as<double>(),
+    return launch_gather_block(st, B.Gt + R.b0, B.ldt, P.xrows, P.xrows, nullptr, d_ord, Q.npairs, ctx->ws_Gs.as<double>(),
                                P.ldp, (int)P.ldp);
 }
 
@@ -158,11 +158,17 @@
 int ScanPass::donor_columns(const Block& B, const SubRange& R, const Pairs& Q, DonorCols& D) {
     D.in_pair_order = ng == 1 && !P.wb_block;
     D.G = D.in_pair_order ? ctx->ws_Gs.as<double>() : B.Gt + R.b0;
-    D.ldg = D.in_pair_order ? P.ldp : P.ldb;
+    D.ldg = D.in_pair_order ? P.ldp : B.ldt;
+    D.Gk = ctx->ws_Gk.as<double>();
+    D.ldk = D.in_pair_order ? P.ldp : P.ldb;
     D.ncol = D.in_pair_order ? Q.npairs : R.nb;
+    if (B.fused && !D.in_pair_order) {
+        D.Gk = ctx->ws_Gkt.as<double>();
+        return CRM_OK;
+    }
     const int blk_cols = (int)(P.ldb - R.b0);
     return launch_gather_rows(st, D.G, D.ldg, bg->kin_map.as<int>(), bg->kin_rows, D.in_pair_order ? (int)D.ldg : blk_cols,
-                              ctx->ws_Gk.as<double>(), D.ldg);
+                              ctx->ws_Gk.as<double>(), D.ldk);
 }
 int ScanPass::gather_pairs(const double* src, long rows, const Pairs& Q) {
     const int xg_cols = (int)std::min<long>(P.ld_xg, round_up((long)Q.npairs * k0, 128) + 128);
@@ -173,12 +179,11 @@
     DonorCols D;
     CRM_TRY(donor_columns(B, R, Q, D));
     double* S = ctx->ws_S.as<double>();
-    double* Gk = ctx->ws_Gk.as<double>();
     const int k1 = bg->kin_k1, k2 = bg->kin_k2, ncol = D.ncol, npair = P.npair;
     const long groups = bg->kin_groups, ld_ah = P.ld_ah;
     std::vector<GemmProblem> kp((size_t)groups + P.fold_split6);
     GemmProblem p{};
-    p.X = Gk; p.ldx = D.ldg;
+    p.X = D.Gk; p.ldx = D.ldk;
     if (probed.donor_pairs) {
         p.Y = g0->kinEE.as<double>(); p.ldy = g0->ld_ee; p.C = ctx->ws_Pd.as<double>(); p.ldc = P.ldPd;
         p.M = ncol; p.N = npair;
@@ -253,7 +258,7 @@
     const int k1 = bg->kin_k1, k2 = bg->kin_k2, ncol = D.ncol, npair = P.npair;
     const long groups = bg->kin_groups, mk = bg->kin_cols, KK = P.KK, ld_ah = P.ld_ah;
     GemmProblem p{};
-    p.X = ctx->ws_Gk.as<double>(); p.ldx = D.ldg;
+    p.X = D.Gk; p.ldx = D.ldk;
     if (probed.pairs_unfolded) {
         double* Pd = ctx->ws_Pd.as<double>();
         double* Z = S;
@@ -293,7 +298,7 @@
 
 int ScanPass::direct_AH(const Block& B, const SubRange& R, const Pairs& Q, AGroups& A) {
     GemmProblem p{};
-    p.X = B.Gt + R.b0; p.ldx = P.ldb; p.E = d_Ep; p.lde = g0->ld_ep; p.k0 = k0; p.Y = bg->H.as<double>(); p.ldy = bg->ldh;
+    p.X = B.Gt + R.b0; p.ldx = B.ldt; p.E = d_Ep; p.lde = g0->ld_ep; p.k0 = k0; p.Y = bg->H.as<double>(); p.ldy = bg->ldh;
     p.C = ctx->ws_AH.as<double>(); p.ldc = P.ld_ah; p.M = R.nb * k0; p.N = (int)bg->cols;
     CRM_TRY(upload(SLOT_ONE, &p, 1));
     CRM_TRY(launch_kr_transposed(ctx, d_probs + SLOT_ONE, 1, p.M, p.N, np, k0));
@@ -383,7 +388,7 @@
     double* const Gt = B.Gt + R.b0;
     double* G2 = ctx->ws_G2.as<double>();
     double* GG = !P.collapsed() ? ctx->ws_GG.as<double>() : nullptr;
-    CRM_TRY(launch_square_block(st, Gt, B.Gx + R.b0, ldb, ldb, P.xrows, (int)(ldb - R.b0), G2, GG, ldb));
+    if (!B.fused) CRM_TRY(launch_square_block(st, Gt, B.Gx + R.b0, ldb, ldb, P.xrows, (int)(ldb - R.b0), G2, GG, ldb));
     if (!GG) GG = G2;
     const int s2 = P.collapsed() ? 1 : P.ks2, s3 = P.collapsed() ? 1 : P.ks3;
     GemmProblem p{};
@@ -409,7 +414,7 @@
     for (int gi = 0; gi < ng; gi++) {
         crm_gene* g = genes[gi];
         GemmProblem& p = zp[(size_t)gi];
-        p.X = B.Gt + R.b0; p.ldx = P.ldb; p.Y = P.collapsed() ? g->dt_Z1.as<double>() : g->YE.as<double>(); p.ldy = g->ld_ye;
+        p.X = B.Gt + R.b0; p.ldx = B.ldt; p.Y = P.collapsed() ? g->dt_Z1.as<double>() : g->YE.as<double>(); p.ldy = g->ld_ye;
         p.C = dZ1 + (size_t)gi * z1_sz * P.ks1; p.ldc = P.ldZ1; p.M = R.nb; p.N = k0 * (1 + c);
     }
     CRM_TRY(upload(P.z1_slot(), zp.data(), zp.size()));
diff --git a/cellregmap_amd/csrc/scan_pass.h b/cellregmap_amd/csrc/scan_pass.h
--- a/cellregmap_amd/csrc/scan_pass.h
+++ b/cellregmap_amd/csrc/scan_pass.h
@@ -73,6 +73,8 @@
     double* Gb = nullptr;
     double* Gt = nullptr;
     double* Gx = nullptr;
+    long ldt = 0;
+    bool fused = false;
     std::vector<double> flat_obj;
 };
 struct SubRange {
@@ -88,7 +90,12 @@
     size_t a_slab = 0;
     std::vector<GemmProblem> tails, spectrum_tails;
 };
-struct DonorCols { bool in_pair_order; const double* G; long ldg; int ncol; };
+struct DonorCols {
+    bool in_pair_order;
+    const double* G; long ldg;
+    const double* Gk; long ldk;
+    int ncol;
+};
 
 struct ScanPass {
     const std::vector<crm_gene*>& genes;
@@ -164,10 +171,13 @@
     }
 
     int workspaces();
+    bool keep_tables() const { return !idx_E; }
     int context_features(bool shared_too);
     int prepare_contexts();
     int prepare_kinship();
     int prepare_woodbury();
+    bool fused_pass() const;
+    bool fused_block(long col0, int nb) const;
     int copy_block(Block& B);
     int block_stats(Block& B);
     int fold_TH(const Block& B);
diff --git a/cellregmap_amd/csrc/scan_prepare.hip b/cellregmap_amd/csrc/scan_prepare.hip
--- a/cellregmap_amd/csrc/scan_prepare.hip
+++ b/cellregmap_amd/csrc/scan_prepare.hip
@@ -42,7 +42,12 @@
     CRM_TRY(ctx->ws_A.ensure(sizeof(double) * (size_t)(P.wb() ? std::max(max_pairs, BLK) : max_pairs) * k0 * P.ldAw));
     CRM_TRY(ctx->ws_Anone.ensure(sizeof(double) * (size_t)P.ldAw));
     CRM_HIP(hipMemsetAsync(ctx->ws_Anone.ptr, 0, sizeof(double) * (size_t)P.ldAw, st));
-    CRM_TRY(ctx->ws_Gb.ensure(sizeof(double) * (size_t)np * ldb));
+    bool copies = false, fused = false;
+    for (long done = 0; done < count; done += BLK)
+        (fused_block(first + done, (int)std::min<long>(BLK, count - done)) ? fused : copies) = true;
+    if (copies) CRM_TRY(ctx->ws_Gb.ensure(sizeof(double) * (size_t)np * ldb));
+    if (fused && P.kin() && (ng > 1 || P.wb_block))
+        CRM_TRY(ctx->ws_Gkt.ensure(sizeof(double) * (size_t)bg->kin_rows * ldb));
     CRM_TRY(ctx->ws_Gs.ensure(sizeof(double) * (size_t)np * P.ldp));
     CRM_TRY(ctx->ws_G2.ensure(sizeof(double) * (size_t)np * ldb));
     if (idx_G)
@@ -55,7 +60,11 @@
     dZ3 = dZ2 + z2_sz * P.ks2;
     if (bg->fast_T) {
         CRM_TRY(ctx->ws_TH.ensure(sizeof(double) * (size_t)P.th_slab * P.ks_h));
-        CRM_HIP(hipMemsetAsync(ctx->ws_TH.ptr, 0, sizeof(double) * (size_t)P.th_slab, st));
+        const crm_ctx::ThKey th_key{ctx->ws_TH.serial, bg->kin_gen, (int)P.route, P.ks_h, P.ldb, P.th_slab};
+        if (!(ctx->th_key == th_key)) {
+            CRM_HIP(hipMemsetAsync(ctx->ws_TH.ptr, 0, sizeof(double) * (size_t)P.th_slab, st));
+            ctx->th_key = th_key;
+        }
     }
     CRM_TRY(ctx->ws_F.ensure(sizeof(double) * (size_t)BLK * k0 * k0));
     CRM_TRY(ctx->ws_Gext.ensure(sizeof(double) * (size_t)BLK * P.KT * P.KT));
@@ -139,6 +148,7 @@
     for (int gi = 0; gi < ng; gi++) {
         crm_gene* g = genes[gi];
         const bool both = gi == 0 && shared_too;
+        if (g->tab_YE && (!both || g->tab_E)) continue;
         CRM_TRY(g->YE.ensure(sizeof(double) * np * g->ld_ye));
         if (both) {
             CRM_TRY(g->Ep.ensure(sizeof(double) * np * g->ld_ep));
@@ -148,6 +158,8 @@
                                         g->yW.as<double>() + 1, g->ld_yw, c,
                                         both ? g->Ep.as<double>() : nullptr, g->ld_ep, g->YE.as<double>(),
                                         g->ld_ye, both ? g->EE.as<double>() : nullptr, g->ld_ee));
+        g->tab_YE = keep_tables();
+        if (both) g->tab_E = keep_tables();
     }
     if (shared_too) {
         d_Ep = g0->Ep.as<double>();
@@ -170,6 +182,12 @@
         g->ld_ep = round_up(k0, 128);
         g->ld_ye = P.ldZ1;
         g->ld_ee = P.ldZ3;
+        const crm_gene::TableKey key{bg->kin_gen, k0, g->ld_ep, g->ld_ye, g->ld_ee};
+        if (!keep_tables() || !(g->tab_key == key)) {
+            g->tab_YE = g->tab_E = g->tab_kinEp = g->tab_kinUE = g->tab_kinP = g->tab_kinEE = false;
+            g->tab_e1_is_E = g->tab_us_is_E = -1;
+            g->tab_key = keep_tables() ? key : crm_gene::TableKey{};
+        }
     }
     if (!P.collapsed()) return context_features(true);
     const double* Zt = panel->Z.as<double>();
@@ -223,31 +241,46 @@
 int ScanPass::prepare_kinship() {
     const long ldh = bg->ldh;
     const double* H = bg->H.as<double>();
-    if (P.kin()) {
+    if (P.kin() && !g0->tab_kinEp) {
         CRM_TRY(g0->kinEp.ensure(sizeof(double) * (size_t)bg->kin_rows * g0->ld_ep));
         CRM_TRY(launch_gather_rows(st, d_Ep, g0->ld_ep, bg->kin_map.as<int>(), bg->kin_rows, (int)g0->ld_ep,
                                    g0->kinEp.as<double>(), g0->ld_ep));
-    }
-    if (P.folded() && bg->kin_k2 == 1) {
+        g0->tab_kinEp = keep_tables();
+    }
+    if (P.folded() && bg->kin_k2 == 1 && !g0->tab_kinUE) {
         CRM_TRY(g0->kinUE.ensure(sizeof(double) * (size_t)bg->kin_rows * g0->ld_ep));
         CRM_TRY(launch_scale_rows(st, g0->kinEp.as<double>(), g0->ld_ep, bg->kin_Y.as<double>(), bg->kin_ldy, bg->kin_rows,
                                   (int)g0->ld_ep, g0->kinUE.as<double>(), g0->ld_ep));
+        g0->tab_kinUE = keep_tables();
     }
     const SameColumns e1_is_E{H, ldh, d_Ep, g0->ld_ep, n};
     const SameColumns us_is_E{bg->kin_Y.as<double>(), bg->kin_ldy, g0->kinEp.as<double>(), g0->ld_ep, bg->kin_rows};
-    if (probed.e1_sym) CRM_TRY(same_columns(st, d_near, k0, {e1_is_E}, probed.e1_sym));
-    if (P.e1_pairs && !probed.e1_sym) {
+    auto asked = [&](const SameColumns& pair, int& kept, bool& same) -> int {
+        if (kept < 0) {
+            CRM_TRY(same_columns(st, d_near, k0, {pair}, same));
+            if (keep_tables()) kept = same ? 1 : 0;
+        } else
+            same = kept == 1;
+        return CRM_OK;
+    };
+    if (probed.e1_sym) CRM_TRY(asked(e1_is_E, g0->tab_e1_is_E, probed.e1_sym));
+    if (P.e1_pairs && !probed.e1_sym && !g0->tab_kinP) {
         CRM_TRY(g0->kinP.ensure(sizeof(double) * (size_t)np * P.ldP));
         CRM_TRY(launch_pair_features(st, H, ldh, bg->kin_k1, d_Ep, g0->ld_ep, k0, np, g0->kinP.as<double>(), P.ldP));
+        g0->tab_kinP = keep_tables();
     }
     probed.donor_pairs = probed.donor_pairs && probed.e1_sym;
-    if (probed.donor_pairs) CRM_TRY(same_columns(st, d_near, k0, {us_is_E}, probed.donor_pairs));
-    if (probed.pairs_unfolded) CRM_TRY(same_columns(st, d_near, k0, {e1_is_E, us_is_E}, probed.pairs_unfolded));
+    if (probed.donor_pairs) CRM_TRY(asked(us_is_E, g0->tab_us_is_E, probed.donor_pairs));
+    if (probed.pairs_unfolded) CRM_TRY(asked(e1_is_E, g0->tab_e1_is_E, probed.pairs_unfolded));
+    if (probed.pairs_unfolded) CRM_TRY(asked(us_is_E, g0->tab_us_is_E, probed.pairs_unfolded));
     probed.wb_rotate = probed.wb_rotate && probed.donor_pairs;
     if (probed.donor_pairs || probed.pairs_unfolded) {
-        CRM_TRY(g0->kinEE.ensure(sizeof(double) * (size_t)bg->kin_rows * g0->ld_ee));
-        CRM_TRY(launch_gather_rows(st, d_EE, g0->ld_ee, bg->kin_map.as<int>(), bg->kin_rows, (int)g0->ld_ee, g0->kinEE.as<double>(),
-                                   g0->ld_ee));
+        if (!g0->tab_kinEE) {
+            CRM_TRY(g0->kinEE.ensure(sizeof(double) * (size_t)bg->kin_rows * g0->ld_ee));
+            CRM_TRY(launch_gather_rows(st, d_EE, g0->ld_ee, bg->kin_map.as<int>(), bg->kin_rows, (int)g0->ld_ee,
+                                       g0->kinEE.as<double>(), g0->ld_ee));
+            g0->tab_kinEE = keep_tables();
+        }
         CRM_TRY(ctx->ws_Pd.ensure(sizeof(double) * (size_t)(probed.donor_pairs ? bg->kin_groups : bg->kin_groups_pad) * P.pd_slab));
     }
     if (probed.donor_pairs)
```

After: 76840, median of 6. 2.1% higher.
